# YukeWang96/GNNAdvisor_OSDI21

Measured on AMD Instinct MI355X. Metric: aggregated edges/sec, GCN sum-aggregation SpMM (SAG) hidden=64, higher is better.
Workload: dtype f32; 1 GPU; reddit-like power-law graph, random node order; num_nodes=232965, nnz=114623790, dim=64, partSize=128, num_parts=1008217, parallelism=single GPU, call=GNNA.SAG (pybind module, reference signature, fresh output), decider=auto/mi355x, column_phases=16, build_id=0.6.1+dd9458378fe52dcc

## Files before the change

gnnadvisor_osdi21_amd/_lib.py:

```python
from __future__ import annotations

import ctypes
import math
import os

import torch

_HERE = os.path.dirname(os.path.abspath(__file__))
LIB_PATH = os.environ.get("GNNA_LIB") or os.path.join(_HERE, "csrc", "libgnna.so")

GNNA_OK = 0


class GnnaError(RuntimeError):
    pass


class Tuning(ctypes.Structure):
    _fields_ = [("struct_size", ctypes.c_int), ("groups_per_chunk", ctypes.c_int), ("loads_in_flight", ctypes.c_int),
                ("blocks_per_cu", ctypes.c_int), ("xcd_remap", ctypes.c_int),
                ("trust_canonical", ctypes.c_int), ("column_phases", ctypes.c_int),
                ("avg_degree", ctypes.c_int), ("nonlocal_ids", ctypes.c_int), ("gcn_prescale", ctypes.c_int),
                ("pad_rows", ctypes.c_int), ("zero_fill", ctypes.c_int),
                ("sweep", ctypes.c_int), ("sweep_slack", ctypes.c_int), ("deterministic", ctypes.c_int),
# ... 238 lines not shown
    ci = torch.empty(max(1, s.numel()), dtype=torch.int32)
    nnz = load().gnna_csr_from_edges_i32(s.data_ptr(), d.data_ptr(), s.numel(), int(num_nodes),
                                         rp.data_ptr(), ci.data_ptr())
    if nnz < 0:
        _check(int(nnz))
    return rp, ci[:nnz].clone()


def row_counts(rows, num_nodes: int, counts: torch.Tensor | None = None) -> torch.Tensor:
    r = _host_i32(rows)
    if counts is None:
        counts = torch.zeros(int(num_nodes), dtype=torch.int64)
    assert counts.dtype == torch.int64 and counts.numel() == int(num_nodes) and counts.is_contiguous()
    _check(load().gnna_row_counts_i64(r.data_ptr(), r.numel(), int(num_nodes), counts.data_ptr()))
    return counts


def row_splits(counts: torch.Tensor, world: int, want_row_pointers: bool = False):
    assert counts.dtype == torch.int64 and counts.is_contiguous() and not counts.is_cuda
    n = counts.numel()
    bounds = torch.empty(int(world) + 1, dtype=torch.int64)
    rp = torch.empty(n + 1, dtype=torch.int64) if want_row_pointers else None
    _check(load().gnna_row_splits_i64(counts.data_ptr(), n, int(world), bounds.data_ptr(), _ptr(rp)))
    return (bounds.tolist(), rp) if want_row_pointers else bounds.tolist()


def csr_from_edges_range(src, dst, num_nodes: int, row_lo: int, row_hi: int, capacity: int | None = None):
    s, d = _host_i32(src), _host_i32(dst)
    assert s.numel() == d.numel()
    if capacity is None:
        capacity = int(((s >= row_lo) & (s < row_hi)).sum()) if s.numel() else 0
    rp = torch.empty(int(row_hi - row_lo) + 1, dtype=torch.int32)
    ci = torch.empty(max(1, int(capacity)), dtype=torch.int32)
    nnz = load().gnna_csr_from_edges_range_i32(s.data_ptr(), d.data_ptr(), s.numel(), int(num_nodes), int(row_lo),
                                               int(row_hi), rp.data_ptr(), ci.data_ptr(), int(capacity))
    if nnz < 0:
        _check(int(nnz))
    return rp, ci[:nnz].clone()


def degrees(row_pointers: torch.Tensor) -> torch.Tensor:
    rp = _host_i32(row_pointers)
    out = torch.empty(rp.numel() - 1, dtype=torch.float32)
    _check(load().gnna_degrees_f32(rp.data_ptr(), rp.numel() - 1, out.data_ptr()))
    return out


def edge_span(src, dst) -> float:
    s, d = _host_i32(src), _host_i32(dst)
    v = ctypes.c_double()
    _check(load().gnna_edge_span(s.data_ptr(), d.data_ptr(), s.numel(), ctypes.byref(v)))
    return v.value


def _reorder(entry: str, src, dst, num_nodes: int) -> torch.Tensor:
    s, d = _host_i32(src), _host_i32(dst)
    out = torch.empty(int(num_nodes), dtype=torch.int32)
    _check(getattr(load(), entry)(s.data_ptr(), d.data_ptr(), s.numel(), int(num_nodes), out.data_ptr()))
    return out


def reorder_rcm(src, dst, num_nodes: int) -> torch.Tensor:
    return _reorder("gnna_reorder_rcm_i32", src, dst, num_nodes)


def reorder_community(src, dst, num_nodes: int) -> torch.Tensor:
    return _reorder("gnna_reorder_community_i32", src, dst, num_nodes)


def reorder_community_csr(row_pointers, column_index, num_nodes: int) -> torch.Tensor:
    rp, ci = _host_i32(row_pointers), _host_i32(column_index)
    assert rp.numel() == int(num_nodes) + 1
    out = torch.empty(int(num_nodes), dtype=torch.int32)
    _check(load().gnna_reorder_community_csr_i32(rp.data_ptr(), ci.data_ptr(), int(num_nodes), out.data_ptr()))
    return out


def relabel_edges_(src: torch.Tensor, dst: torch.Tensor, new_id: torch.Tensor, num_nodes: int) -> float:
    for t in (src, dst, new_id):
        assert t.dtype == torch.int32 and t.is_contiguous() and not t.is_cuda
    v = ctypes.c_double()
    _check(load().gnna_relabel_edges_i32(src.data_ptr(), dst.data_ptr(), src.numel(), new_id.data_ptr(), int(num_nodes), ctypes.byref(v)))
    return v.value


def relabel_csr(row_pointers, column_index, new_id, num_nodes: int):
    rp, ci, nid = _host_i32(row_pointers), _host_i32(column_index), _host_i32(new_id)
    out_rp = torch.empty(int(num_nodes) + 1, dtype=torch.int32)
    out_ci = torch.empty(max(1, ci.numel()), dtype=torch.int32)
    _check(load().gnna_relabel_csr_i32(rp.data_ptr(), ci.data_ptr(), int(num_nodes), nid.data_ptr(), out_rp.data_ptr(), out_ci.data_ptr()))
    return out_rp, out_ci[:ci.numel()]


def last_num_phases() -> int:
    return int(load().gnna_last_num_phases())


def last_num_launches() -> int:
    return int(load().gnna_last_num_launches())


def profile_begin(max_calls: int) -> None:
    _check(load().gnna_profile_begin(int(max_calls)))


def profile_end() -> dict:
    a, b, n = ctypes.c_double(), ctypes.c_double(), ctypes.c_int()
    _check(load().gnna_profile_end(ctypes.byref(a), ctypes.byref(b), ctypes.byref(n)))
    return dict(main_ms=a.value, prologue_ms=b.value, calls=n.value)


def count_parts(partSize: int, indptr: torch.Tensor) -> int:
    assert indptr.dtype == torch.int32 and not indptr.is_cuda and indptr.is_contiguous()
    n = load().gnna_count_parts(int(partSize), indptr.data_ptr(), indptr.numel() - 1)
    if n < 0:
        _check(int(n))
    return int(n)


def build_part(partSize: int, indptr: torch.Tensor):
    indptr = indptr.contiguous()
    P = count_parts(partSize, indptr)
    pp = torch.empty(P + 1, dtype=torch.int32)
    p2n = torch.empty(P, dtype=torch.int32)
    _check(load().gnna_build_part_i32(int(partSize), indptr.data_ptr(), indptr.numel() - 1,
                                      pp.data_ptr(), p2n.data_ptr(), P))
    return pp, p2n


def _fresh_output(shape, device, dtype=torch.float32) -> torch.Tensor:
    if os.environ.get("GNNA_DEBUG_POISON", "0") not in ("", "0"):
        return torch.full(tuple(shape), float("nan") if dtype.is_floating_point else -(2 ** 31), dtype=dtype, device=device)
    return torch.empty(tuple(shape), dtype=dtype, device=device)


def _agg(fn_name, X, row_pointers, column_index, extra, part_pointers, part2Node, partSize, dimWorker,
         warpPerBlock, out):
    _need_device(X, "aggregation")
    assert X.dtype == torch.float32 and X.is_contiguous() and X.dim() == 2
    for t in (column_index, part_pointers, part2Node):
        assert t.dtype == torch.int32 and t.is_contiguous() and t.device == X.device
    if out is None:
        out = _fresh_output(X.shape, X.device)
    _call(X.device, fn_name, X.data_ptr(), _ptr(row_pointers), column_index.data_ptr(), extra,
          part_pointers.data_ptr(), part2Node.data_ptr(), out.data_ptr(), X.shape[0], X.shape[1], part2Node.numel(),
          int(partSize), int(dimWorker), int(warpPerBlock))
    return out


def sag(X, row_pointers, column_index, degrees, part_pointers, part2Node, partSize=32, dimWorker=32,
        warpPerBlock=4, out=None):
    return _agg("gnna_sag_f32", X, row_pointers, column_index, _ptr(degrees), part_pointers,
                part2Node, partSize, dimWorker, warpPerBlock, out)


def agg_gcn(X, row_pointers, column_index, degrees, part_pointers, part2Node, partSize=32,
            dimWorker=32, warpPerBlock=4, out=None):
    assert degrees.dtype == torch.float32 and degrees.device == X.device
    return _agg("gnna_agg_gcn_f32", X, row_pointers, column_index, degrees.data_ptr(),
                part_pointers, part2Node, partSize, dimWorker, warpPerBlock, out)


def agg_gin(X, row_pointers, column_index, epsilon, part_pointers, part2Node, partSize=32,
            dimWorker=32, warpPerBlock=4, out=None):
    return _agg("gnna_agg_gin_f32", X, row_pointers, column_index, ctypes.c_float(epsilon),
                part_pointers, part2Node, partSize, dimWorker, warpPerBlock, out)


MODE_SAG, MODE_GCN, MODE_GIN = 0, 1, 2


def agg_rect(mode, X, column_index, part_pointers, part2Node, num_out_rows, partSize=32,
             degrees_out=None, degrees_in=None, epsilon=1.0, out=None, accumulate=False, windows=None):
    _need_device(X, "aggregation")
    assert X.dtype == torch.float32 and X.is_contiguous() and X.dim() == 2
    if out is None:
        assert not accumulate, "accumulate needs an existing `out`"
        out = _fresh_output((num_out_rows, X.shape[1]), X.device)
    args = (int(mode), X.data_ptr(), X.shape[0], column_index.data_ptr(), _ptr(degrees_out), _ptr(degrees_in), float(epsilon),
            part_pointers.data_ptr(), part2Node.data_ptr(), out.data_ptr(), int(num_out_rows), X.shape[1], part2Node.numel(),
            int(partSize), 1 if accumulate else 0)
    if windows is not None:
        K, wb, we = (int(v) for v in windows)
        assert wb == 0 or out is not None
        _call(X.device, "gnna_agg_rect_windows_f32", *args, K, wb, we)
    else:
        _call(X.device, "gnna_agg_rect_f32", *args)
    return out


ACCUMULATE, EPILOGUE_RELU = 1, 2


def _flags(accumulate=False, relu=False) -> int:
    return (ACCUMULATE if accumulate else 0) | (EPILOGUE_RELU if relu else 0)


def _rows_view(t: torch.Tensor, what: str, dtype=torch.float32, unit="floats"):
    assert (dtype is None or t.dtype == dtype) and t.dim() == 2, \
        f"{what} must be a 2-D {'' if dtype is None else str(dtype).replace('torch.', '') + ' '}tensor"
    if t.shape[1] > 1 and t.stride(1) != 1:
        raise GnnaError(f"{what}: the {unit} of a row must be contiguous (stride(1) == 1)")
    ld = t.stride(0) if t.shape[0] > 1 else max(t.shape[1], t.stride(0))
    if ld < t.shape[1]:
        raise GnnaError(f"{what}: rows overlap (stride(0) = {t.stride(0)} < {t.shape[1]})")
    return t.data_ptr(), t.shape[0], t.shape[1], ld


def _rows_view_any(t: torch.Tensor, what: str):
    return _rows_view(t, what, dtype=None, unit="elements")


def _out_rows(out, rows, width, device, accumulate=False):
    if out is None:
        assert not accumulate, "accumulate needs an existing `out`"
        out = _fresh_output((rows, width), device)
    ptr, n, w, ld = _rows_view(out, "out")
    assert n == int(rows) and w == width and out.device == device
    return out, ptr, ld


def agg_ld(mode, X, column_index, part_pointers, part2Node, num_out_rows, partSize=32, degrees_out=None,
           degrees_in=None, epsilon=1.0, out=None, accumulate=False, relu=False):
    _need_device(X, "aggregation")
    xp, n_in, dim, ld_in = _rows_view(X, "X")
    out, yp, ld_out = _out_rows(out, num_out_rows, dim, X.device, accumulate)
    _call(X.device, "gnna_agg_ld_f32", int(mode), xp, ld_in, n_in, column_index.data_ptr(), _ptr(degrees_out), _ptr(degrees_in),
          float(epsilon), part_pointers.data_ptr(), part2Node.data_ptr(), yp, ld_out, int(num_out_rows), dim, part2Node.numel(),
          int(partSize), _flags(accumulate, relu))
    return out


F32, BF16, F16 = 0, 1, 2
_X16_TYPES = {torch.bfloat16: BF16, torch.float16: F16}


def agg_ld_x16(mode, X, column_index, part_pointers, part2Node, num_out_rows, partSize=32, degrees_out=None,
               degrees_in=None, epsilon=1.0, out=None, out_dtype=None, accumulate=False, relu=False):
    _need_device(X, "aggregation")
    if X.dtype not in _X16_TYPES:
        raise GnnaError(f"agg_ld_x16 takes bfloat16 or float16 features (got {X.dtype}); float32 goes through agg_ld")
    xp, n_in, dim, ld_in = _rows_view_any(X, "X")
    if out is None:
        assert not accumulate, "accumulate needs an existing `out`"
        out = _fresh_output((int(num_out_rows), dim), X.device, X.dtype if out_dtype is None else out_dtype)
    elif out_dtype is not None and out.dtype != out_dtype:
        raise GnnaError(f"out is {out.dtype}, out_dtype says {out_dtype}")
    if out.dtype != torch.float32 and out.dtype != X.dtype:
        raise GnnaError(f"the output is float32 or has the input's dtype {X.dtype} (got {out.dtype})")
    out_type = F32 if out.dtype == torch.float32 else _X16_TYPES[out.dtype]
    yp, n_out, dim_o, ld_out = _rows_view_any(out, "out")
    assert n_out == int(num_out_rows) and dim_o == dim and out.device == X.device
    for t in (degrees_out, degrees_in):
        assert t is None or t.dtype == torch.float32, "degrees stay float32"
    _call(X.device, "gnna_agg_ld_x16", int(mode), _X16_TYPES[X.dtype], xp, ld_in, n_in, column_index.data_ptr(), _ptr(degrees_out),
          _ptr(degrees_in), float(epsilon), part_pointers.data_ptr(), part2Node.data_ptr(), yp, out_type, ld_out, int(num_out_rows),
          dim, part2Node.numel(), int(partSize), _flags(accumulate, relu))
    return out


def prepare_x16(num_in_rows: int, num_out_rows: int, dims, device=None) -> None:
    dims = [int(d) for d in dims]
    arr = (ctypes.c_int * max(1, len(dims)))(*dims)
    device = torch.device("cuda", torch.cuda.current_device()) if device is None else torch.device(device)
    _call(device, "gnna_prepare_x16", int(num_in_rows), int(num_out_rows), arr, len(dims))


def preferred_ld(dim: int, num_in_rows: int, num_edges: int) -> int:
    return int(load().gnna_preferred_ld(int(dim), int(num_in_rows), int(num_edges)))


def empty_rows(num_rows: int, dim: int, ld: int, device) -> torch.Tensor:
    if ld == dim:
        return torch.empty(num_rows, dim, dtype=torch.float32, device=device)
    buf = torch.empty(num_rows * ld + ld, dtype=torch.float32, device=device)
    off = (-buf.data_ptr() // 4) % ld
    return buf[off: off + num_rows * ld].view(num_rows, ld)[:, :dim]


def prepare_graph(column_index, part_pointers, part2Node, num_in_rows: int, num_out_rows: int, partSize: int,
                  dims=()) -> dict:
    dims = [int(d) for d in dims]
    arr = (ctypes.c_int * max(1, len(dims)))(*dims)
    out = (ctypes.c_int * max(1, len(dims)))()
    _call(column_index.device, "gnna_prepare_graph", column_index.data_ptr(), part_pointers.data_ptr(), part2Node.data_ptr(),
          part2Node.numel(), int(num_in_rows), int(num_out_rows), int(partSize), arr, len(dims), out)
    _forget_when_freed(column_index)
    return {d: int(out[i]) for i, d in enumerate(dims)}


def release_graph(column_index) -> None:
    ptr = None if column_index is None else column_index.data_ptr()
    _check(load().gnna_release_graph(ptr))
    if column_index is None:
        _registered.clear()
    else:
        _registered.pop(ptr, None)


def runtime_counters() -> dict:
    out = (ctypes.c_int64 * 16)()
    n = load().gnna_runtime_counters_ex(out, 16)
    names = ("plan_builds", "launch_syncs", "launch_frees", "launch_mallocs", "backoff_skips", "sweep_launches",
             "pack_builds", "packed_launches", "full_hashes", "capture_scratch")
    return {name: int(out[i]) for i, name in enumerate(names) if i < n}


def debug_untrusted_copies(column_index) -> int:
    n = load().gnna_debug_untrusted_copies(column_index.data_ptr())
    _check(min(n, 0))
    return n


def set_graph_phases(column_index, dim: int, column_phases: int) -> None:
    _check(load().gnna_set_graph_phases(column_index.data_ptr(), int(dim), int(column_phases)))
    if column_phases > 0:
        _forget_when_freed(column_index)


def xtg(X, G, out=None):
    _need_device(X, "xtg")
    assert X.dtype == torch.float32 and G.dtype == torch.float32 and X.dim() == 2 and G.dim() == 2
    assert X.shape[0] == G.shape[0]
    X, G = X.contiguous(), G.contiguous()
    if out is None:
        out = torch.empty(X.shape[1], G.shape[1], dtype=torch.float32, device=X.device)
    _call(X.device, "gnna_xtg_f32", X.data_ptr(), G.data_ptr(), out.data_ptr(), X.shape[0], X.shape[1], G.shape[1])
    return out


def sddmm(dst_feat, src_feat, column_index, part_pointers, part2Node, partSize=32, out=None):
    _need_device(dst_feat, "sddmm")
    ap, n_out, dim, ld_dst = _rows_view(dst_feat, "dst_feat")
    bp, n_in, dim_b, ld_src = _rows_view(src_feat, "src_feat")
    assert dim == dim_b and dst_feat.device == src_feat.device
    if out is None:
        out = torch.zeros(column_index.numel(), dtype=torch.float32, device=dst_feat.device)
    tail = (column_index.data_ptr(), part_pointers.data_ptr(), part2Node.data_ptr(), out.data_ptr(), n_out, n_in, dim,
            part2Node.numel(), int(partSize))
    if ld_dst == dim and ld_src == dim:
        _call(dst_feat.device, "gnna_sddmm_f32", ap, bp, *tail)
    else:
        _call(dst_feat.device, "gnna_sddmm_ld_f32", ap, ld_dst, bp, ld_src, *tail)
    return out


def agg_edge(X, column_index, edge_weight, part_pointers, part2Node, num_out_rows, partSize=32, out=None,
             accumulate=False, relu=False):
    _need_device(X, "aggregation")
    assert edge_weight.dtype == torch.float32 and edge_weight.is_contiguous() and edge_weight.numel() == column_index.numel(), \
        "edge_weight must be a contiguous float32 tensor indexed like column_index"
    xp, n_in, dim, ld_in = _rows_view(X, "X")
    out, yp, ld_out = _out_rows(out, num_out_rows, dim, X.device, accumulate)
    _call(X.device, "gnna_agg_edge_ld_f32", xp, ld_in, n_in, column_index.data_ptr(), edge_weight.data_ptr(), part_pointers.data_ptr(),
          part2Node.data_ptr(), yp, ld_out, int(num_out_rows), dim, part2Node.numel(), int(partSize), _flags(accumulate, relu))
    return out


def edge_softmax(scores, row_pointers, out=None):
    assert scores.is_cuda and scores.dtype == torch.float32 and scores.is_contiguous() and scores.dim() in (1, 2)
    heads, nnz = (1, scores.numel()) if scores.dim() == 1 else scores.shape
    out = torch.empty_like(scores) if out is None else out
    _call(scores.device, "gnna_edge_softmax_f32", scores.data_ptr(), row_pointers.data_ptr(), row_pointers.numel() - 1, nnz, heads,
          out.data_ptr())
    return out


def edge_softmax_backward(probs, grad_probs, row_pointers, out=None):
    assert probs.is_cuda and probs.dtype == torch.float32 and probs.is_contiguous() and probs.dim() in (1, 2)
    assert grad_probs.shape == probs.shape and grad_probs.dtype == torch.float32 and grad_probs.is_contiguous()
    heads, nnz = (1, probs.numel()) if probs.dim() == 1 else probs.shape
    out = torch.empty_like(probs) if out is None else out
    _call(probs.device, "gnna_edge_softmax_backward_f32", probs.data_ptr(), grad_probs.data_ptr(), row_pointers.data_ptr(),
          row_pointers.numel() - 1, nnz, heads, out.data_ptr())
    return out


def reverse_edges(row_pointers, column_index) -> torch.Tensor:
    rp, ci = _host_i32(row_pointers), _host_i32(column_index)
    rev = torch.empty(ci.numel(), dtype=torch.int32)
    _check(load().gnna_reverse_edges_i32(rp.data_ptr(), ci.data_ptr(), rp.numel() - 1, rev.data_ptr()))
    return rev


REDUCE_MAX, REDUCE_MIN = 0, 1


def _arg_view(t: torch.Tensor, rows: int, dim: int, what: str):
    assert t.dtype == torch.int32 and t.dim() == 2 and tuple(t.shape) == (rows, dim), f"{what} must be int32 [{rows}, {dim}]"
    ptr, _, _, ld = _rows_view(t, what, dtype=torch.int32, unit="elements")
    return ptr, ld


def agg_reduce_ld(op, X, column_index, part_pointers, part2Node, partSize=32, *, num_out_rows=None, out=None, want_arg=True,
                  relu=False, arg=None):
    _need_device(X, "aggregation")
    xp, n_in, dim, ld_in = _rows_view(X, "X")
    n_out = n_in if num_out_rows is None else int(num_out_rows)
    out, yp, ld_out = _out_rows(out, n_out, dim, X.device)
    ap, ld_arg = None, dim
    if arg is not None or want_arg:
        if arg is None:
            arg = _fresh_output((n_out, dim), X.device, torch.int32)
        assert arg.device == X.device
        ap, ld_arg = _arg_view(arg, n_out, dim, "arg")
    _call(X.device, "gnna_agg_reduce_ld_f32", int(op), xp, ld_in, n_in, column_index.data_ptr(), part_pointers.data_ptr(),
          part2Node.data_ptr(), yp, ld_out, ap, ld_arg, n_out, dim, part2Node.numel(), int(partSize), _flags(relu=relu))
    return out, arg


def scatter_arg_ld(grad_out, arg, column_index, num_in_rows, out=None, accumulate=False):
    _need_device(grad_out, "scatter_arg")
    gp, n_out, dim, ld_go = _rows_view(grad_out, "grad_out")
    ap, ld_arg = _arg_view(arg, n_out, dim, "arg")
    out, op_, ld_gi = _out_rows(out, int(num_in_rows), dim, grad_out.device, accumulate)
    assert arg.device == grad_out.device
    _call(grad_out.device, "gnna_scatter_arg_ld_f32", gp, ld_go, ap, ld_arg, column_index.data_ptr(), n_out, op_, ld_gi,
          int(num_in_rows), dim, _flags(accumulate))
    return out


STATS = ("sum", "sumsq", "max", "min")


def agg_stats_ld(X, column_index, part_pointers, part2Node, num_out_rows=None, partSize=32, want=STATS, out=None):
    _need_device(X, "aggregation")
    want = tuple(want)
    unknown = [w for w in want if w not in STATS]
    if unknown or not want:
        raise ValueError(f"want must name some of {STATS} (got {want!r})")
    xp, n_in, dim, ld_in = _rows_view(X, "X")
    n_out = n_in if num_out_rows is None else int(num_out_rows)
    out = dict(out or {})
    res, args = {}, []
    for name in STATS:
        wanted = name in want
        val = None
        if wanted:
            val, vp, ld = _out_rows(out.get(name), n_out, dim, X.device)
            res[name] = val
        args += [vp if wanted else None, ld if wanted else dim]
        if name in ("max", "min"):
            arg = None
            if wanted and ("arg" + name in out or name not in out):
                arg = out.get("arg" + name)
                if arg is None:
                    arg = _fresh_output((n_out, dim), X.device, torch.int32)
                assert arg.device == X.device
                ap, ld_arg = _arg_view(arg, n_out, dim, "arg" + name)
                res["arg" + name] = arg
            args += [ap if arg is not None else None, ld_arg if arg is not None else dim]
    _call(X.device, "gnna_agg_stats_ld_f32", xp, ld_in, n_in, column_index.data_ptr(), part_pointers.data_ptr(), part2Node.data_ptr(),
          *args, n_out, dim, part2Node.numel(), int(partSize), 0)
    return res


def _temp_arg(temp, dim, device):
    assert temp.dtype == torch.float32 and temp.device == device and temp.is_contiguous() and temp.numel() in (1, dim), \
        f"temp must be a contiguous float32 tensor of 1 or {dim} elements on {device}"
    return temp.data_ptr(), temp.numel()


def _ids_ptr(column_index, row_pointers):
    return column_index.data_ptr() or row_pointers.data_ptr()


def agg_softmax(X, temp, row_pointers, column_index, num_out_rows=None, want_sq=False, out=None, lse=None, sq=None):
    _need_device(X, "aggregation")
    xp, n_in, dim, ld_in = _rows_view(X, "X")
    n_out = row_pointers.numel() - 1 if num_out_rows is None else int(num_out_rows)
    assert row_pointers.numel() == n_out + 1, f"row_pointers must be [num_out_rows + 1 = {n_out + 1}] (got {row_pointers.numel()} entries)"
    tp, tl = _temp_arg(temp, dim, X.device)
    out, op_, ld_out = _out_rows(out, n_out, dim, X.device)
    lse, lp, ld_lse = _out_rows(lse, n_out, dim, X.device)
    qp, ld_sq = None, dim
    if want_sq or sq is not None:
        sq, qp, ld_sq = _out_rows(sq, n_out, dim, X.device)
    _call(X.device, "gnna_agg_softmax_ld_f32", xp, ld_in, n_in, tp, tl, row_pointers.data_ptr(), _ids_ptr(column_index, row_pointers),
          op_, ld_out, lp, ld_lse, qp, ld_sq, n_out, dim, 0)
    return out, lse, sq


def agg_softmax_backward(X, temp, lse, Y, dY, t_row_pointers, t_column_index, out=None):
    _need_device(X, "aggregation")
    xp, n_in, dim, ld_in = _rows_view(X, "X")
    assert t_row_pointers.numel() == n_in + 1, f"t_row_pointers must be [num_in_rows + 1 = {n_in + 1}] (got {t_row_pointers.numel()} entries)"
    tp, tl = _temp_arg(temp, dim, X.device)
    lp, n_out, w, ld_lse = _rows_view(lse, "lse")
    yp, ny, wy, ld_y = _rows_view(Y, "Y")
    gp, ng, wg, ld_dy = _rows_view(dY, "dY")
    assert (ny, ng) == (n_out, n_out) and (w, wy, wg) == (dim, dim, dim), "lse, Y and dY must be [num_out_rows, dim]"
    out, op_, ld_din = _out_rows(out, n_in, dim, X.device)
    _call(X.device, "gnna_agg_softmax_backward_ld_f32", xp, ld_in, n_in, tp, tl, lp, ld_lse, yp, ld_y, gp, ld_dy,
          t_row_pointers.data_ptr(), _ids_ptr(t_column_index, t_row_pointers), op_, ld_din, n_out, dim, 0)
    return out


POOL_TILE_ROWS = 256
POOL_LONG_STEPS = 16
POOL_MEAN = 1
POOL_STATS = ("sum", "max", "min")


def _graph_pointers_arg(graph_pointers, device):
    assert graph_pointers.dtype == torch.int32 and graph_pointers.dim() == 1 and graph_pointers.numel() >= 1 and \
        graph_pointers.is_contiguous() and graph_pointers.device == device, \
        f"graph_pointers must be a contiguous int32 tensor [num_graphs + 1] on {device}"
    return graph_pointers.data_ptr(), graph_pointers.numel() - 1


def segment_pool(X, graph_pointers, want=("sum",), mean=False, out=None):
    want = tuple(want)
    if not want or [w for w in want if w not in POOL_STATS]:
        raise ValueError(f"want must name some of {POOL_STATS} (got {want!r})")
    _need_device(X, "segment_pool")
    xp, n, dim, ld_in = _rows_view(X, "X")
    gp, G = _graph_pointers_arg(graph_pointers, X.device)
    out = dict(out or {})
    res, args = {}, []
    for name in POOL_STATS:
        wanted = name in want
        if wanted:
            val, vp, ld = _out_rows(out.get(name), G, dim, X.device)
            res[name] = val
        args += [vp if wanted else None, ld if wanted else dim]
        if name != "sum":
            arg = None
            if wanted and ("arg" + name in out or name not in out):
                arg = out.get("arg" + name)
                if arg is None:
                    arg = _fresh_output((G, dim), X.device, torch.int32)
                assert arg.device == X.device
                ap, ld_arg = _arg_view(arg, G, dim, "arg" + name)
                res["arg" + name] = arg
            args += [ap if arg is not None else None, ld_arg if arg is not None else dim]
    if G > 0:
        _call(X.device, "gnna_segment_pool_ld_f32", xp if n > 0 else None, ld_in, n, gp, G, *args, dim, POOL_MEAN if mean else 0)
    return res


def segment_pool_backward(graph_pointers, num_rows, d_sum=None, d_max=None, argmax=None, d_min=None, argmin=None, mean=False, out=None):
    given = [t for t in (d_sum, d_max, d_min) if t is not None]
    if not given:
        raise ValueError("segment_pool_backward needs d_sum, d_max or d_min")
    if (d_max is None) != (argmax is None) or (d_min is None) != (argmin is None):
        raise ValueError("d_max comes with argmax, d_min with argmin")
    _need_device(given[0], "segment_pool_backward")
    device = given[0].device
    gp, G = _graph_pointers_arg(graph_pointers, device)
    dim = given[0].shape[1]
    args = []
    for grad, arg, name in ((d_sum, None, "d_sum"), (d_max, argmax, "d_max"), (d_min, argmin, "d_min")):
        if grad is None:
            args += [None, dim] * (1 if name == "d_sum" else 2)
            continue
        vp, rows, w, ld = _rows_view(grad, name)
        assert (rows, w) == (G, dim) and grad.device == device, f"{name} must be [num_graphs = {G}, dim = {dim}] on {device}"
        args += [vp, ld]
        if name != "d_sum":
            assert arg.device == device
            args += list(_arg_view(arg, G, dim, "arg" + name[2:]))
    out, op_, ld_din = _out_rows(out, int(num_rows), dim, device)
    if G == 0:
        stand_in = torch.zeros(1, dim, dtype=torch.float32, device=device)
        args = [stand_in.data_ptr(), dim] + [None, dim] * 4
    _call(device, "gnna_segment_pool_backward_ld_f32", *args, gp, G, op_ if int(num_rows) > 0 else None, ld_din, int(num_rows), dim,
          POOL_MEAN if mean else 0)
    return out


def _gate_view(gate, n, dim, device):
    g2 = gate.unsqueeze(1) if gate.dim() == 1 else gate
    gp_, rows, gate_dim, ld_gate = _rows_view(g2, "gate")
    assert rows == n and gate_dim in (1, dim) and gate.device == device, \
        f"gate must be [{n}], [{n}, 1] or [{n}, {dim}] on {device} (got {tuple(gate.shape)})"
    return gp_, gate_dim, ld_gate


def segment_attn_pool(X, gate, graph_pointers, out=None):
    _need_device(X, "segment_attn_pool")
    xp, n, dim, ld_in = _rows_view(X, "X")
    gtp, gate_dim, ld_gate = _gate_view(gate, n, dim, X.device)
    gp, G = _graph_pointers_arg(graph_pointers, X.device)
    given = dict(out or {})
    res = {}
    res["out"], op_, ld_out = _out_rows(given.get("out"), G, dim, X.device)
    lp, ld_lse = None, gate_dim
    if "lse" in given or "out" not in given:
        res["lse"], lp, ld_lse = _out_rows(given.get("lse"), G, gate_dim, X.device)
    if G > 0:
        _call(X.device, "gnna_segment_attn_pool_ld_f32", xp if n > 0 else None, ld_in, n, gtp if n > 0 else None, ld_gate, gate_dim,
              gp, G, op_, ld_out, lp, ld_lse, dim, 0)
    return res


def segment_attn_pool_backward(X, gate, lse, Y, dY, graph_pointers, need_input=True, need_gate=True, out=None):
    if not need_input and not need_gate:
        raise ValueError("segment_attn_pool_backward needs need_input or need_gate")
    _need_device(X, "segment_attn_pool_backward")
    xp, n, dim, ld_in = _rows_view(X, "X")
    gtp, gate_dim, ld_gate = _gate_view(gate, n, dim, X.device)
    gp, G = _graph_pointers_arg(graph_pointers, X.device)
    lp, gl, wl, ld_lse = _rows_view(lse, "lse")
    yp, gy, wy, ld_y = _rows_view(Y, "Y")
    dp, gd, wd, ld_dy = _rows_view(dY, "dY")
    assert (gl, gy, gd) == (G, G, G) and (wl, wy, wd) == (gate_dim, dim, dim) and lse.device == Y.device == dY.device == X.device, \
        f"lse must be [{G}, {gate_dim}], Y and dY [{G}, {dim}] on {X.device}"
# ... 483 lines not shown
```

gnnadvisor_osdi21_amd/build.py:

```python
from __future__ import annotations

import os
import subprocess
import sys
import sysconfig

PKG = os.path.dirname(os.path.abspath(__file__))
ROOT = os.path.dirname(PKG)
CSRC = os.path.join(PKG, "csrc")
INCLUDE = os.path.join(ROOT, "include")
LIB = os.path.join(CSRC, "libgnna.so")
EXT = os.path.join(PKG, "GNNAdvisor.so")
ARCH = "gfx950"
HIPCC = os.environ.get("HIPCC", "/opt/rocm/bin/hipcc")

LIB_SOURCES = [os.path.join(CSRC, f) for f in ("gnna_agg.hip", "gnna_stream.hip", "gnna_sweep.hip", "gnna_x16.hip", "gnna_reduce.hip", "gnna_stats.hip", "gnna_softagg.hip", "gnna_pool.hip", "gnna_attnpool.hip", "gnna_sddmm.hip", "gnna_edge.hip", "gnna_gat.hip", "gnna_gatv2.hip", "gnna_dotattn.hip", "gnna_typed.hip", "gnna_transpose.hip", "gnna_sample.hip",
                                                "gnna_gemm.hip", "gnna_runtime.hip", "gnna_host.cpp", "gnna_reorder.cpp")]
LIB_DEPS = LIB_SOURCES + [os.path.join(CSRC, "gnna_internal.h"), os.path.join(CSRC, "gnna_device.h"), os.path.join(CSRC, "gnna_launch.h"),
                           os.path.join(CSRC, "gnna_gat_common.h"), os.path.join(CSRC, "gnna_keys.h"), os.path.join(CSRC, "gnna_segments.h"), os.path.join(INCLUDE, "gnna.h"), os.path.join(INCLUDE, "gnna_ext.h"),
                           os.path.join(INCLUDE, "gnna_gatv2.h"), os.path.join(INCLUDE, "gnna_dotattn.h"),
                           os.path.join(INCLUDE, "gnna_gat_edge.h"), os.path.join(INCLUDE, "gnna_stats.h"),
                           os.path.join(INCLUDE, "gnna_softagg.h"), os.path.join(INCLUDE, "gnna_pool.h"),
                           os.path.join(INCLUDE, "gnna_attnpool.h")]
EXT_SOURCES = [os.path.join(CSRC, "gnna_torch.cpp")]
EXT_DEPS = EXT_SOURCES + [os.path.join(INCLUDE, "gnna.h"), os.path.join(INCLUDE, "gnna_ext.h"), os.path.join(INCLUDE, "gnna_gatv2.h"),
                          os.path.join(INCLUDE, "gnna_dotattn.h"), os.path.join(INCLUDE, "gnna_gat_edge.h"),
                          os.path.join(INCLUDE, "gnna_stats.h"), os.path.join(INCLUDE, "gnna_softagg.h"), os.path.join(INCLUDE, "gnna_pool.h"),
                          os.path.join(INCLUDE, "gnna_attnpool.h")]


def source_hash() -> str:
    import hashlib
    h = hashlib.sha256()
    for path in sorted(set(LIB_DEPS + EXT_DEPS)):
        h.update(os.path.relpath(path, ROOT).encode() + b"\0")
        with open(path, "rb") as f:
            h.update(f.read())
        h.update(b"\0")
    return h.hexdigest()[:16]


def _stale(target: str, deps: list[str]) -> bool:
    if not os.path.exists(target):
        return True
    t = os.path.getmtime(target)
    return any(os.path.getmtime(d) > t for d in deps)


def build_lib(force: bool = False, verbose: bool = False) -> str:
    from concurrent.futures import ThreadPoolExecutor
    objdir = os.path.join(CSRC, "build")
    os.makedirs(objdir, exist_ok=True)
    headers = [d for d in LIB_DEPS if d not in LIB_SOURCES]
    flags = [f"--offload-arch={ARCH}", "-O3", "-std=c++17", "-fPIC", "-munsafe-fp-atomics", "-ffp-contract=off",
             "-fvisibility=hidden", "-I" + INCLUDE, "-I" + CSRC]
    jobs, objs = [], []
    digest = source_hash()
    stamp = os.path.join(objdir, "source_hash.txt")
    stamped = open(stamp).read().strip() if os.path.exists(stamp) else ""
    if not force and stamped == digest and os.path.exists(LIB) and not _stale(LIB, LIB_DEPS):
        return LIB
    for src in LIB_SOURCES:
        obj = os.path.join(objdir, os.path.basename(src) + ".o")
        objs.append(obj)
        carries_id = os.path.basename(src) == "gnna_host.cpp"
        if force or _stale(obj, [src] + headers) or (carries_id and stamped != digest):
            jobs.append([HIPCC, *flags, *([f'-DGNNA_SOURCE_HASH="{digest}"'] if carries_id else []), "-c", src, "-o", obj])

    def run(cmd):
        if verbose:
            print(" ".join(cmd), flush=True)
        subprocess.check_call(cmd)
    if jobs:
        with ThreadPoolExecutor(max_workers=min(len(jobs), os.cpu_count() or 4)) as pool:
            list(pool.map(run, jobs))
    if jobs or force or _stale(LIB, objs):
        run([HIPCC, f"--offload-arch={ARCH}", "-shared", "-fPIC", "-fvisibility=hidden", *objs, "-o", LIB])
    with open(stamp, "w") as f:
        f.write(digest + "\n")
    if verbose:
        print(f"libgnna.so: source hash {digest} ({'compiled ' + str(len(jobs)) + ' object(s)' if jobs else 'objects up to date'})", flush=True)
    return LIB


def build_ext(force: bool = False, verbose: bool = False) -> str:
    build_lib(force, verbose)
    digest = source_hash()
    stamp = os.path.join(CSRC, "build", "ext_source_hash.txt")
    stamped = open(stamp).read().strip() if os.path.exists(stamp) else ""
    if force or _stale(EXT, EXT_DEPS + [LIB]) or stamped != digest:
        import pybind11
        import torch
        tdir = os.path.dirname(torch.__file__)
        cmd = [HIPCC, "-O2", "-std=c++17", "-fPIC", "-shared", "-w",
               "-DTORCH_EXTENSION_NAME=GNNAdvisor", "-DTORCH_API_INCLUDE_EXTENSION_H", f'-DGNNA_SOURCE_HASH="{digest}"',
               "-DUSE_ROCM", "-D__HIP_PLATFORM_AMD__",
               f"-D_GLIBCXX_USE_CXX11_ABI={int(torch._C._GLIBCXX_USE_CXX11_ABI)}",
               "-I" + INCLUDE,
               "-I" + os.path.join(tdir, "include"),
               "-I" + os.path.join(tdir, "include", "torch", "csrc", "api", "include"),
               "-I" + sysconfig.get_paths()["include"], "-I" + pybind11.get_include(),
               "-I/opt/rocm/include",
               "-x", "c++", *EXT_SOURCES, "-o", EXT,
               "-L" + CSRC, "-lgnna", "-Wl,-rpath,$ORIGIN/csrc",
               "-L" + os.path.join(tdir, "lib"), "-lc10", "-lc10_hip", "-ltorch", "-ltorch_cpu",
               "-ltorch_hip", "-ltorch_python", "-Wl,-rpath," + os.path.join(tdir, "lib")]
        if verbose:
            print(" ".join(cmd))
        subprocess.check_call(cmd)
        with open(stamp, "w") as f:
            f.write(digest + "\n")
    return EXT


def build_all(force: bool = False, verbose: bool = False) -> None:
    build_ext(force, verbose)


if __name__ == "__main__":
    build_all(force="--force" in sys.argv, verbose=True)
    print("built", LIB, "and", EXT)
```

gnnadvisor_osdi21_amd/csrc/gnna_agg.hip:

```cpp
#include <hip/hip_runtime.h>

#include <algorithm>
#include <cmath>
#include <cstdint>
#include <cstdio>

#include "gnna.h"
#include "gnna_device.h"
#include "gnna_internal.h"

namespace gnna {
namespace {


__global__ void __launch_bounds__(kBlock)
prologue_kernel(float *__restrict__ Y, size_t n_floats, int D, int ldy, const int32_t *__restrict__ p2n,
                const int32_t *__restrict__ pp, int64_t P, int32_t *flag, int32_t seq, int validate, int zero_fill,
                const int32_t *__restrict__ chk_ids, int64_t chk_n, const unsigned long long *__restrict__ chk_sum,
                int32_t *stale_flag, uint32_t *__restrict__ clear_words, int n_clear)
{
    if (blockIdx.x == 0 && (int)threadIdx.x < n_clear) clear_words[threadIdx.x] = 0u;
    const unsigned fill_blocks = chk_ids ? gridDim.x - 1 : gridDim.x;
    if (blockIdx.x >= fill_blocks) {
        if (threadIdx.x < kWave) {
            const unsigned long long then = chk_sum[0], distrusted = chk_sum[4];
            const unsigned long long now = graph_checksum(chk_ids, chk_n, pp, P, (int)threadIdx.x);
            if (threadIdx.x == 0 && (now != then || distrusted != 0ull)) *stale_flag = seq;
        }
        return;
    }
    const size_t tid = (size_t)blockIdx.x * blockDim.x + threadIdx.x;
    const size_t nthreads = (size_t)fill_blocks * blockDim.x;
    typedef float f32x4 __attribute__((ext_vector_type(4)));
    if (!zero_fill) {
    } else if (ldy != D) {
        if ((D & 3) == 0 && (ldy & 3) == 0 && (reinterpret_cast<uintptr_t>(Y) & 15) == 0) {
            const size_t n4 = n_floats >> 2;
            const unsigned d4 = (unsigned)D >> 2, ld4 = (unsigned)ldy >> 2;
            const f32x4 z = (f32x4)(0.f);
            for (size_t i = tid; i < n4; i += nthreads) {
                const size_t r = i / d4;
                reinterpret_cast<f32x4 *>(Y)[r * ld4 + (i - r * d4)] = z;
            }
        } else {
            for (size_t i = tid; i < n_floats; i += nthreads) {
                const size_t r = i / (unsigned)D;
                Y[r * (size_t)ldy + (i - r * (unsigned)D)] = 0.f;
            }
        }
    } else if ((reinterpret_cast<uintptr_t>(Y) & 15) == 0) {
        const size_t n4 = n_floats >> 2;
        f32x4 *Y4 = reinterpret_cast<f32x4 *>(Y);
        const f32x4 z = (f32x4)(0.f);
        for (size_t i = tid; i < n4; i += nthreads) Y4[i] = z;
        for (size_t i = (n4 << 2) + tid; i < n_floats; i += nthreads) Y[i] = 0.f;
    } else {
        for (size_t i = tid; i < n_floats; i += nthreads) Y[i] = 0.f;
    }
    if (validate) {
        bool bad = false;
        for (int64_t g = (int64_t)tid; g < P; g += (int64_t)nthreads) {
            if (pp[g + 1] < pp[g]) bad = true;
            if (g + 1 < P && p2n[g + 1] < p2n[g]) bad = true;
        }
        if (bad) *flag = seq;
    }
}

__global__ void __launch_bounds__(kBlock)
sparse_prologue_kernel(float *__restrict__ Y, int64_t N, int D, int ldy, const int32_t *__restrict__ p2n,
                       const int32_t *__restrict__ pp, int64_t P, int G, int32_t *flag, int32_t seq, int validate,
                       unsigned long long *gaps, int64_t big_rows)
{
    const int lane = threadIdx.x & (kWave - 1);
    const int64_t wave = ((int64_t)blockIdx.x * blockDim.x + threadIdx.x) >> 6;
    const int64_t nwaves = ((int64_t)gridDim.x * blockDim.x) >> 6;
    typedef float f32x4 __attribute__((ext_vector_type(4)));
    const bool vec_ok = (D & 3) == 0 && (reinterpret_cast<uintptr_t>(Y) & 15) == 0;
    auto clear_rows = [&](int64_t lo, int64_t cnt) {
        if (gaps && cnt >= big_rows) {
            unsigned long long idx = 0;
            if (lane == 0) idx = atomicAdd(&gaps[0], 1ull);
            idx = ((unsigned long long)__builtin_amdgcn_readfirstlane((int)(idx >> 32)) << 32) |
                  (uint32_t)__builtin_amdgcn_readfirstlane((int)idx);
            if (idx < (unsigned long long)kGapEntries) {
                if (lane == 0) { gaps[2 + 2 * idx] = (unsigned long long)lo; gaps[3 + 2 * idx] = (unsigned long long)cnt; }
                return;
            }
        }
        if (ldy != D) {
            for (int64_t r = lo; r < lo + cnt; r++) {
                float *row = Y + (size_t)r * (size_t)ldy;
                for (int i = lane; i < D; i += kWave) row[i] = 0.f;
            }
            return;
        }
        float *base = Y + (size_t)lo * (size_t)D;
        const size_t n = (size_t)cnt * (size_t)D;
        if (vec_ok) {
            f32x4 *b4 = reinterpret_cast<f32x4 *>(base);
            const f32x4 z = (f32x4)(0.f);
            for (size_t i = lane; i < (n >> 2); i += kWave) b4[i] = z;
        } else {
            for (size_t i = lane; i < n; i += kWave) base[i] = 0.f;
        }
    };
    if (wave == 0) {
        int64_t first = p2n[0];
        first = first < 0 ? 0 : (first > N ? N : first);
        if (first > 0) clear_rows(0, first);
    }
    bool bad = false;
    for (int64_t g0 = wave * kWave; g0 < P; g0 += nwaves * kWave) {
        const int64_t g = g0 + lane;
        const bool valid = g < P;
        int64_t lo = 0, cnt = 0;
        if (valid) {
            const int64_t r = p2n[g];
            const int64_t nxt = g + 1 < P ? (int64_t)p2n[g + 1] : N;
            const int a = pp[g], b = pp[g + 1];
            if (b < a || (g + 1 < P && nxt < r)) bad = true;
            const bool continues = g > 0 && (g % G) == 0 && p2n[g - 1] == r;
            const bool self = b <= a || continues;
            lo = self ? r : r + 1;
            int64_t hi = (self && nxt < r + 1) ? r + 1 : nxt;
            lo = lo < 0 ? 0 : lo;
            hi = hi > N ? N : hi;
            cnt = hi > lo ? hi - lo : 0;
        }
        unsigned long long m = __ballot(cnt > 0);
        while (m) {
            const int l = __builtin_ctzll(m);
            m &= m - 1;
            const int64_t lo_s = ((int64_t)__builtin_amdgcn_readlane((int)(lo >> 32), l) << 32) |
                                 (uint32_t)__builtin_amdgcn_readlane((int)lo, l);
            const int64_t cnt_s = ((int64_t)__builtin_amdgcn_readlane((int)(cnt >> 32), l) << 32) |
                                  (uint32_t)__builtin_amdgcn_readlane((int)cnt, l);
            clear_rows(lo_s, cnt_s);
        }
    }
    if (validate && bad) *flag = seq;
}

__global__ void __launch_bounds__(kBlock)
post_prologue_kernel(float *__restrict__ Y, size_t n_floats, int D, int ldy, const int32_t *flag, int32_t seq,
                     const unsigned long long *gaps)
{
    const size_t tid = (size_t)blockIdx.x * blockDim.x + threadIdx.x;
    const size_t nthreads = (size_t)gridDim.x * blockDim.x;
    auto at = [&](float *base, size_t i) -> float * {
        if (ldy == D) return base + i;
        const size_t r = i / (unsigned)D;
        return base + r * (size_t)ldy + (i - r * (unsigned)D);
    };
    if (*flag == seq) {
        for (size_t i = tid; i < n_floats; i += nthreads) *at(Y, i) = 0.f;
        return;
    }
    if (!gaps) return;
    const unsigned long long n = gaps[0] < (unsigned long long)kGapEntries ? gaps[0] : (unsigned long long)kGapEntries;
    for (unsigned long long k = 0; k < n; k++) {
        float *base = Y + (size_t)gaps[2 + 2 * k] * (size_t)ldy;
        const size_t cnt = (size_t)gaps[3 + 2 * k] * (size_t)D;
        for (size_t i = tid; i < cnt; i += nthreads) *at(base, i) = 0.f;
    }
}

__global__ void __launch_bounds__(kBlock)
scale_rows_kernel(const float *__restrict__ X, int64_t ld_in, const float *__restrict__ deg, float *__restrict__ Xs,
                  int64_t rows, int D, int ld_out)
{
    const size_t tid = (size_t)blockIdx.x * blockDim.x + threadIdx.x;
    const size_t nthreads = (size_t)gridDim.x * blockDim.x;
    typedef float f32x4 __attribute__((ext_vector_type(4)));
    const bool aligned = ((reinterpret_cast<uintptr_t>(X) | reinterpret_cast<uintptr_t>(Xs)) & 15) == 0;
    if (ld_out == D && ld_in == D && (D & 3) == 0 && aligned) {
        const size_t n4 = ((size_t)rows * (size_t)D) >> 2;
        const int d4 = D >> 2;
        for (size_t i = tid; i < n4; i += nthreads) {
            const f32x4 v = __builtin_nontemporal_load(reinterpret_cast<const f32x4 *>(X) + i);
            reinterpret_cast<f32x4 *>(Xs)[i] = deg ? v * deg[i / d4] : v;
        }
    } else if ((D & 3) == 0 && (ld_out & 3) == 0 && (ld_in & 3) == 0 && aligned) {
        const size_t n4 = ((size_t)rows * (size_t)D) >> 2;
        const unsigned d4 = (unsigned)D >> 2;
        const size_t ldo4 = (size_t)ld_out >> 2, ldi4 = (size_t)ld_in >> 2;
        for (size_t i = tid; i < n4; i += nthreads) {
            const size_t r = i / d4, c4 = i - r * d4;
            const f32x4 v = __builtin_nontemporal_load(reinterpret_cast<const f32x4 *>(X) + r * ldi4 + c4);
            reinterpret_cast<f32x4 *>(Xs)[r * ldo4 + c4] = deg ? v * deg[r] : v;
        }
    } else {
        const size_t total = (size_t)rows * (size_t)D;
        for (size_t i = tid; i < total; i += nthreads) {
            const size_t r = i / (unsigned)D, cc = i - r * (unsigned)D;
            const float v = __builtin_nontemporal_load(X + r * (size_t)ld_in + cc);
            Xs[r * (size_t)ld_out + cc] = deg ? v * deg[r] : v;
        }
    }
}


static size_t gather_footprint_bytes(int64_t num_in_rows, int ldx, int dim)
{
    return (size_t)num_in_rows * (size_t)std::min(ldx, (std::max(dim, 4) * 4 + 127) / 128 * 32) * sizeof(float);
}

thread_local int t_last_phases = 1;
thread_local int t_last_launches = 1;

double avg_lines_per_row(int64_t row_bytes, int64_t stride_bytes)
{
    int64_t lines = 0;
    for (int k = 0; k < 32; k++) {
        const int64_t o = (k * stride_bytes) % 128;
        lines += (o + row_bytes + 127) / 128;
    }
    return (double)lines / 32.0;
}

int choose_row_stride(int dim)
{
    if (dim < 2 || dim > 256) return dim;
    auto cost = [&](int stride) {
        return avg_lines_per_row((int64_t)dim * 4, (int64_t)stride * 4) * ((stride & 3) ? 1.07 : 1.0);
    };
    const double plain = cost(dim);
    int best = dim;
    double best_cost = plain * 0.93;
    const int cand[3] = {(dim + 3) / 4 * 4, (dim + 15) / 16 * 16, (dim + 31) / 32 * 32};
    for (int c : cand) {
        if (c == dim || c > 2 * dim) continue;
        const double cc = cost(c) * (1.0 + 0.02 * (double)(c - dim) / (double)dim);
        if (cc < best_cost) { best = c; best_cost = cc; }
    }
    return best;
}

int pick_row_stride(const gnna_tuning &t, int dim, bool hot_rows, int64_t num_in_rows, bool whole_call)
{
    int ldx = dim;
    if (t.pad_rows == 1 || (t.pad_rows == 0 && hot_rows)) ldx = choose_row_stride(dim);
    if (t.pad_rows == 0 && hot_rows && dim > 16 && dim <= 64 && whole_call) {
        const int gapped = 2 * ((dim * 4 + 127) / 128) * 32;
        if ((size_t)num_in_rows * (size_t)gapped * sizeof(float) <= ((size_t)160 << 20)) ldx = gapped;
    }
    if (t.pad_rows > 2 && t.pad_rows >= dim) ldx = t.pad_rows;
    return ldx;
}

}

int stage_rows_for_gather(DeviceState *ds, hipStream_t stream, const gnna_tuning &tune, const float *input, int64_t ld_in,
                          int64_t num_in_rows, int dim, int64_t est_edges, const float **X, int *ldx_out)
{
    *X = input; *ldx_out = (int)ld_in;
    const bool hot_rows = est_edges >= 32 * num_in_rows && (size_t)num_in_rows * (size_t)dim * sizeof(float) <= ((size_t)1 << 30);
    if (dim < 4 || !hot_rows) return GNNA_OK;
    const int want = pick_row_stride(tune, dim, hot_rows, num_in_rows, true);
    if (want == dim || ld_in == want) return GNNA_OK;
    const bool aligned16 = (reinterpret_cast<uintptr_t>(input) & 15) == 0 && (ld_in & 3) == 0;
    const int gapped = 2 * ((dim * 4 + 127) / 128) * 32;
    bool direct;
    if (want == gapped && dim > 16 && dim <= 64)
        direct = (ld_in % gapped) == 0 && (reinterpret_cast<uintptr_t>(input) % ((size_t)gapped * 4)) == 0;
    else
        direct = aligned16 && avg_lines_per_row((int64_t)dim * 4, ld_in * 4) <= avg_lines_per_row((int64_t)dim * 4, (int64_t)want * 4) + 1e-9;
    if (direct) return GNNA_OK;
    const size_t x_bytes = (size_t)num_in_rows * (size_t)want * sizeof(float);
    void *xs = nullptr;
    int rc = get_workspace(ds, stream, 1, x_bytes, &xs);
    if (rc != GNNA_OK) return rc;
    const size_t s_bytes = (size_t)num_in_rows * (size_t)dim * sizeof(float);
    int64_t sblocks = (int64_t)((s_bytes / 16 + kBlock - 1) / kBlock);
    sblocks = std::max<int64_t>(1, std::min<int64_t>(sblocks, (int64_t)ds->num_cus * 8));
    hipLaunchKernelGGL(scale_rows_kernel, dim3((unsigned)sblocks), dim3(kBlock), 0, stream, input, ld_in, (const float *)nullptr,
                       static_cast<float *>(xs), num_in_rows, dim, want);
    hipError_t es = hipGetLastError();
    if (es != hipSuccess) return fail(GNNA_ERR_HIP, "staging launch: %s", hipGetErrorString(es));
    *X = static_cast<const float *>(xs); *ldx_out = want;
    return GNNA_OK;
}

static double near_share(const SlicePlanStats &st, double half_rows)
{
    if (st.edges <= 0 || half_rows < 256.0) return 0.0;
    const double pos = std::min(23.0, 2.0 * std::log2(half_rows / 256.0));
    const int k = (int)pos;
    const double lo = st.near[k], hi = st.near[std::min(23, k + 1)];
    return (lo + (hi - lo) * (pos - k)) / st.edges;
}

int sweep_auto_phases(const gnna_tuning &t, int mode, int dim, size_t x_bytes, int64_t num_out_rows, int64_t num_in_rows,
                      const SlicePlanStats &st, int B, int num_cus, bool deterministic, int part_size)
{
    const double edges = st.edges;
    if (t.sweep != 0 || deterministic || B < 2) return 0;
    if (dim <= 32 || dim > 64 || !sweep_supports(mode, dim, x_bytes)) return 0;
    if (num_in_rows != num_out_rows || x_bytes > ((size_t)160 << 20)) return 0;
    if (edges < 300.0 * (double)std::max<int64_t>(1, num_out_rows)) return 0;
    const double cap = (double)sweep_acc_rows(dim, 1) * 0.9 * (double)std::max(8, num_cus);
    if ((double)num_out_rows > 2.0 * cap) return 0;
    if (near_share(st, (double)num_in_rows / 16.0) > 0.30) return 0;
    if (t.column_phases >= 2) return B;
    return std::max(2, std::min(std::min(16, 2 * B), std::max(2, part_size / 4)));
}

int sweep_phases_of_width(const gnna_tuning &t, int dim, size_t foot_bytes, size_t x_bytes, int64_t num_out_rows,
                          int64_t num_in_rows, const SlicePlanStats &st, int B, int num_cus, int partSize, int S)
{
    int Bs = sweep_auto_phases(t, MODE_SAG, dim, foot_bytes, num_out_rows, num_in_rows, st, B, num_cus, t.deterministic == 1, partSize);
    if (t.sweep == 1 && t.deterministic != 1 && sweep_supports(MODE_SAG, dim, x_bytes))
        Bs = t.column_phases >= 2 ? B : std::max(2, std::min(std::min(16, 2 * B), std::max(2, partSize / 4)));
    return std::min(Bs, S);
}

int choose_slices(const SlicePlanStats &st, size_t x_bytes, int S, uint32_t slice_rows, int64_t num_out_rows,
                  bool square, bool hinted_scattered)
{
    if (st.groups <= 0 || st.edges <= 0) return 1;
    if (!hinted_scattered) {
        if (square) {
            const double row_bytes = (double)x_bytes / ((double)slice_rows * S);
            const double half_rows = 1.75 * 1048576.0 / row_bytes;
            const bool long_rows_cached = st.edges >= 200.0 * (double)std::max<int64_t>(1, num_out_rows) && x_bytes <= (size_t)250000000;
            const bool one_line_rows = row_bytes > 64.0 && row_bytes <= 128.0;
            if (near_share(st, half_rows) >= (long_rows_cached && !one_line_rows ? 0.75 : 0.6)) return 1;
        }
        if (st.cells[0] <= 1.15 * st.groups) return 1;
    }
    int b = 1;
    const double row_bytes_all = (double)x_bytes / ((double)slice_rows * S);
    const size_t slice_target = row_bytes_all <= 64.0 ? ((size_t)4 << 20) : ((size_t)8 << 20);
    while (b < S && x_bytes / b > slice_target) b <<= 1;
    int lvl = 0;
    for (int t = S; t > b; t >>= 1) lvl++;
    const double rows = std::min((double)num_out_rows, st.groups);
    auto piece = [&](int l) {
        return st.edges / std::max(rows, st.cells[l] - (st.groups - rows));
    };
    int levels = 0;
    for (int t = S; t > 1; t >>= 1) levels++;
    levels = std::min(levels, kSliceLevels);
    const double min_piece = row_bytes_all <= 128.0 ? 24.0 : 12.0;
    while (b > 1 && lvl < levels && piece(lvl) < min_piece) { b >>= 1; lvl++; }
    if (lvl >= levels) b = 1;
    const size_t mall = (size_t)250000000;
    if (x_bytes > mall) {
        int bm = 2, lm = levels - 1;
        while (bm < S && x_bytes / bm > mall) { bm <<= 1; lm--; }
        if (x_bytes / bm <= mall && lm >= 0 && piece(lm) >= 8.0) b = std::max(b, bm);
    }
    return std::max(b, 1);
}

int launch_zero_fill(DeviceState *ds, hipStream_t stream, float *out, int64_t rows, int dim, int64_t ld)
{
    const size_t n_floats = (size_t)rows * (size_t)dim;
    if (n_floats == 0) return GNNA_OK;
    int64_t blocks = (int64_t)((n_floats / 4 + kBlock - 1) / kBlock);
    blocks = std::max<int64_t>(1, std::min<int64_t>(blocks, (int64_t)ds->num_cus * 8));
    hipLaunchKernelGGL(prologue_kernel, dim3((unsigned)blocks), dim3(kBlock), 0, stream, out, n_floats, dim, (int)ld, nullptr, nullptr,
                       (int64_t)0, nullptr, 0, 0, 1, nullptr, (int64_t)0, nullptr, nullptr, nullptr, 0);
    return launch_ok("zero-fill launch");
}

namespace {
__global__ void __launch_bounds__(kBlock)
relu_rows_kernel(float *__restrict__ Y, size_t ld, size_t rows, int D)
{
    const size_t n = rows * (size_t)D;
    for (size_t i = (size_t)blockIdx.x * blockDim.x + threadIdx.x; i < n; i += (size_t)gridDim.x * blockDim.x) {
        const size_t r = i / (unsigned)D, c = i - r * (unsigned)D;
        if (Y[r * ld + c] < 0.f) Y[r * ld + c] = 0.f;
    }
}
}

void launch_relu_rows(DeviceState *ds, hipStream_t stream, float *out, int64_t rows, int dim, int64_t ld)
{
    hipLaunchKernelGGL(relu_rows_kernel, dim3(elementwise_grid(rows * dim, ds->num_cus, 8)), dim3(kBlock), 0, stream, out,
                       (size_t)ld, (size_t)rows, dim);
}

namespace {

int launch_agg(int mode, const float *input, int64_t ld_in, int64_t num_in_rows, const int32_t *column_index,
               const float *degrees, const float *degrees_in, float epsilon, const int32_t *part_pointers,
               const int32_t *part2Node, float *out, int64_t ld_out, int64_t num_nodes, int dim, int64_t num_parts,
               int partSize, int dimWorker, int warpPerBlock, void *stream_v, unsigned flags,
               int num_windows = 1, int win_begin = 0, int win_end = 1, bool profiled = true, int hint_dim = 0);

int column_blocks(const gnna_tuning &tune, int dim, int64_t num_in_rows, int64_t est_edges)
{
    if (tune.wide_blocks == 2 || dim < 72) return 1;
    if (tune.wide_blocks == 1) return (dim + 63) / 64;
    const bool hot = est_edges >= 32 * num_in_rows;
    if (!hot || (size_t)num_in_rows * (size_t)dim * sizeof(float) > ((size_t)250000000)) return 1;
    const bool long_rows = est_edges >= 200 * num_in_rows;
    if (dim < (long_rows ? 100 : 192)) return 1;
    return (dim + 63) / 64;
}

int launch_agg_blocked(int nb, int mode, const float *input, int64_t ld_in, int64_t num_in_rows, const int32_t *column_index,
                       const float *degrees, const float *degrees_in, float epsilon, const int32_t *part_pointers,
                       const int32_t *part2Node, float *out, int64_t ld_out, int64_t num_nodes, int dim, int64_t num_parts,
                       int partSize, int dimWorker, int warpPerBlock, void *stream_v, unsigned flags)
{
    hipStream_t stream = static_cast<hipStream_t>(stream_v);
    const int prof_call = profile_acquire_call(num_parts > 0);
    profile_record(prof_call, 0, stream);
    profile_record(prof_call, 1, stream);
    const int w = ((dim + nb - 1) / nb + 3) / 4 * 4;
    int launches = 0, phases = 1;
    for (int c0 = 0; c0 < dim; c0 += w) {
        const int wb = std::min(w, dim - c0);
        const int rc = launch_agg(mode, input + c0, ld_in, num_in_rows, column_index, degrees, degrees_in, epsilon, part_pointers,
                                  part2Node, out + c0, ld_out, num_nodes, wb, num_parts, partSize, dimWorker, warpPerBlock, stream_v,
                                  flags, 1, 0, 1, false, dim);
        if (rc != GNNA_OK) return rc;
        launches += t_last_launches;
        phases = std::max(phases, t_last_phases);
    }
    t_last_launches = launches;
    t_last_phases = phases;
    profile_record(prof_call, 2, stream);
    return GNNA_OK;
}

int launch_agg(int mode, const float *input, int64_t ld_in, int64_t num_in_rows, const int32_t *column_index,
               const float *degrees, const float *degrees_in, float epsilon, const int32_t *part_pointers,
               const int32_t *part2Node, float *out, int64_t ld_out, int64_t num_nodes, int dim, int64_t num_parts,
               int partSize, int dimWorker, int warpPerBlock, void *stream_v, unsigned flags,
               int num_windows, int win_begin, int win_end, bool profiled, int hint_dim)
{
    const bool accumulate_into_out = (flags & GNNA_ACCUMULATE) != 0;
    const bool relu = (flags & GNNA_EPILOGUE_RELU) != 0;
    if (flags & ~(unsigned)(GNNA_ACCUMULATE | GNNA_EPILOGUE_RELU))
        return fail(GNNA_ERR_INVALID_ARGUMENT, "unknown flag bits 0x%x", flags);
    if (num_nodes < 0 || dim < 0 || num_parts < 0 || num_in_rows < 0)
        return fail(GNNA_ERR_INVALID_ARGUMENT, "negative size (num_nodes=%lld dim=%d num_parts=%lld)",
                          (long long)num_nodes, dim, (long long)num_parts);
    if (partSize <= 0 || dimWorker <= 0 || warpPerBlock <= 0)
        return fail(GNNA_ERR_INVALID_ARGUMENT,
                          "partSize, dimWorker and warpPerBlock must be positive (got %d, %d, %d)",
                          partSize, dimWorker, warpPerBlock);
    if (num_windows < 1 || num_windows > 16 || win_begin < 0 || win_end > num_windows || win_begin >= win_end)
        return fail(GNNA_ERR_INVALID_ARGUMENT, "bad source window range [%d, %d) of %d (at most 16 windows)",
                    win_begin, win_end, num_windows);
    if (num_nodes >= ((int64_t)1 << 29))
        return fail(GNNA_ERR_UNSUPPORTED, "%lld destination rows in one call (at most 536870911): shard the rows",
                    (long long)num_nodes);
    if (num_nodes == 0 || dim == 0) return GNNA_OK;
    if (bad_ld(ld_in, dim) || bad_ld(ld_out, dim))
        return fail(GNNA_ERR_INVALID_ARGUMENT, "row strides must be >= dim and < 2^29 floats (ld_in=%lld ld_out=%lld dim=%d)",
                    (long long)ld_in, (long long)ld_out, dim);
    if (!out || !input) return fail(GNNA_ERR_INVALID_ARGUMENT, "null feature pointer");
    if (num_parts > 0 && (!column_index || !part_pointers || !part2Node))
        return fail(GNNA_ERR_INVALID_ARGUMENT, "null index pointer");
    if (mode == MODE_GCN && (!degrees || !degrees_in))
        return fail(GNNA_ERR_INVALID_ARGUMENT, "null degrees pointer");
    if (mode == MODE_EDGE && num_parts > 0 && !degrees_in)
        return fail(GNNA_ERR_INVALID_ARGUMENT, "null edge_weight pointer");
    if (out == input) return fail(GNNA_ERR_INVALID_ARGUMENT, "out must not alias input");

    hipStream_t stream = static_cast<hipStream_t>(stream_v);
    DeviceState *ds = nullptr;
    int rc = get_device_state(&ds);
    if (rc != GNNA_OK) return rc;
    LaunchGuard in_flight;

    gnna_tuning tune;
    gnna_get_tuning(&tune);
    apply_graph_hints(column_index, hint_dim > 0 ? hint_dim : dim, &tune);

    const bool windowed = num_windows > 1;
    if (profiled && !windowed && num_parts > 0) {
        const int64_t est = num_parts * (int64_t)(tune.avg_degree > 0 ? std::min(partSize, tune.avg_degree) : partSize / 2 + 1);
        const int nb = column_blocks(tune, dim, num_in_rows, est);
        if (nb > 1)
            return launch_agg_blocked(nb, mode, input, ld_in, num_in_rows, column_index, degrees, degrees_in, epsilon, part_pointers,
                                      part2Node, out, ld_out, num_nodes, dim, num_parts, partSize, dimWorker, warpPerBlock, stream_v, flags);
    }
    int32_t *flag = nullptr;
    const int32_t seq = next_call_seq(ds, stream, &flag);
    const int prof_call = profiled ? profile_acquire_call(num_parts > 0) : -1;
    profile_record(prof_call, 0, stream);
    const int ldy = (int)ld_out;

    const size_t n_floats = (size_t)num_nodes * (size_t)dim;
    const unsigned long long *chk_sum = nullptr;
    int64_t chk_n = 0;
    int32_t *stale_flag = flag + kFlagSlots;
    auto run_prologue = [&](int sparse_G, uint32_t *clear_words = nullptr, int n_clear = 0) -> int {
        const int validate = (num_parts > 0 && !tune.trust_canonical) ? 1 : 0;
        const int zero_fill = (accumulate_into_out || win_begin > 0) ? 0 : 1;
        if (sparse_G > 0 && zero_fill && num_parts > 0) {
            int64_t blocks = (num_parts + kBlock - 1) / kBlock;
            blocks = std::max<int64_t>(1, std::min<int64_t>(blocks, (int64_t)ds->num_cus * 8));
            unsigned long long *gaps = ds->gap_lists + (size_t)call_block_of(ds, stream, seq) * kGapWords;
            (void)hipMemsetAsync(gaps, 0, sizeof(unsigned long long), stream);
            const int64_t big_rows = std::max<int64_t>(64, ((int64_t)1 << 20) / std::max(1, dim * 4));
            hipLaunchKernelGGL(sparse_prologue_kernel, dim3((unsigned)blocks), dim3(kBlock), 0, stream, out, num_nodes, dim, ldy,
                               part2Node, part_pointers, num_parts, sparse_G, flag, seq, validate, gaps, big_rows);
            hipLaunchKernelGGL(post_prologue_kernel, dim3((unsigned)(ds->num_cus * 8)), dim3(kBlock), 0, stream, out,
                               n_floats, dim, ldy, flag, seq, gaps);
        } else {
            size_t work = std::max(n_floats / 4, (size_t)num_parts);
            int64_t blocks = (int64_t)((work + kBlock - 1) / kBlock);
            blocks = std::max<int64_t>(1, std::min<int64_t>(blocks, (int64_t)ds->num_cus * 8));
            hipLaunchKernelGGL(prologue_kernel, dim3((unsigned)blocks + (chk_sum ? 1u : 0u)), dim3(kBlock), 0, stream, out, n_floats,
                               dim, ldy, part2Node, part_pointers, num_parts, flag, seq, validate, zero_fill,
                               chk_sum ? column_index : nullptr, chk_n, chk_sum, stale_flag, clear_words, n_clear);
        }
        hipError_t e = hipGetLastError();
        if (e != hipSuccess) return fail(GNNA_ERR_HIP, "prologue launch: %s", hipGetErrorString(e));
        profile_record(prof_call, 1, stream);
        return GNNA_OK;
    };
    if (num_parts == 0) {
        rc = run_prologue(0);
        if (rc != GNNA_OK || !relu || !accumulate_into_out) return rc;
        StreamLaunch e0;
        e0.mode = mode; e0.Y = out; e0.p2n = part2Node; e0.P = 0; e0.D = dim; e0.ldy = ldy; e0.relu = true; e0.num_out_rows = num_nodes;
        e0.flag = flag; e0.seq = seq; e0.cnt = nullptr; e0.B = 1; e0.plain_ok = false; e0.G = 1;
        return launch_stream_epilogue_only(e0, stream);
    }

    const int64_t window_rows = (num_in_rows + num_windows - 1) / num_windows;

    const int64_t est_edges = num_parts * (int64_t)(tune.avg_degree > 0 ? std::min(partSize, tune.avg_degree) : partSize / 2 + 1);
    const bool hot_rows = est_edges >= 32 * num_in_rows && (size_t)num_in_rows * (size_t)dim * sizeof(float) <= ((size_t)1 << 30);
    const bool prescale = mode == MODE_GCN && (tune.gcn_prescale == 1 || (tune.gcn_prescale == 0 && hot_rows));
    const int want = dim < 4 ? 4 : pick_row_stride(tune, dim, hot_rows, num_in_rows, !windowed);
    bool direct = !prescale && dim >= 4;
    if (direct && want != dim && ld_in != want) {
        const bool aligned16 = (reinterpret_cast<uintptr_t>(input) & 15) == 0 && (ld_in & 3) == 0;
        const int gapped = 2 * ((dim * 4 + 127) / 128) * 32;
        if (want == gapped && dim > 16 && dim <= 64)
            direct = (ld_in % gapped) == 0 && (reinterpret_cast<uintptr_t>(input) % ((size_t)gapped * 4)) == 0;
        else
            direct = aligned16 && avg_lines_per_row((int64_t)dim * 4, ld_in * 4) <= avg_lines_per_row((int64_t)dim * 4, (int64_t)want * 4) + 1e-9;
    }
    const int ldx = direct ? (int)ld_in : want;
    const float *X = input;
    const float *row_scale = nullptr;
    float eps = epsilon;
    const size_t x_bytes = (size_t)num_in_rows * (size_t)ldx * sizeof(float);
    const size_t foot_bytes = gather_footprint_bytes(num_in_rows, ldx, dim);
    const bool wide = x_bytes > 0xffffffffull;
    if (!direct) {
        void *xs = nullptr;
        rc = get_workspace(ds, stream, 1, x_bytes, &xs);
        if (rc != GNNA_OK) return rc;
        const int64_t r0 = std::min<int64_t>((int64_t)win_begin * window_rows, num_in_rows);
        const int64_t r1 = std::min<int64_t>((int64_t)win_end * window_rows, num_in_rows);
        const size_t s_bytes = (size_t)(r1 - r0) * (size_t)dim * sizeof(float);
        int64_t sblocks = (int64_t)((s_bytes / 16 + kBlock - 1) / kBlock);
        sblocks = std::max<int64_t>(1, std::min<int64_t>(sblocks, (int64_t)ds->num_cus * 8));
        hipLaunchKernelGGL(scale_rows_kernel, dim3((unsigned)sblocks), dim3(kBlock), 0, stream,
                           input + (size_t)r0 * (size_t)ld_in, ld_in, prescale ? degrees_in + r0 : nullptr,
                           static_cast<float *>(xs) + (size_t)r0 * ldx, r1 - r0, dim, ldx);
        hipError_t es = hipGetLastError();
        if (es != hipSuccess) return fail(GNNA_ERR_HIP, "staging launch: %s", hipGetErrorString(es));
        X = static_cast<const float *>(xs);
        if (prescale) {
            row_scale = degrees;
            eps = 1.f;
            mode = MODE_GIN;
        }
    }

    int B = 1;
    const uint8_t *cnt = nullptr;
    int S = kMaxSlices;
    int win_lo = 0, win_hi = 0;
    SlicePlan plan;
    const bool can_slice = num_parts >= 1024 && num_in_rows >= 64 && foot_bytes >= ((size_t)2 << 20);
    if (windowed) {
        rc = get_slice_plan(ds, stream, column_index, part_pointers, part2Node, num_parts, num_in_rows, true, false, &plan,
                            (uint32_t)std::max<int64_t>(1, window_rows));
        if (rc != GNNA_OK) return rc;
        if (!plan.cnt || !plan.stats.valid)
            return fail(GNNA_ERR_UNSUPPORTED, "the windowed aggregation needs its window counts, which cannot be built inside a "
                                              "stream capture: run the sequence once before capturing it");
        if (plan.stats.unsorted > 0)
            return fail(GNNA_ERR_UNSUPPORTED, "windowed aggregation: the column ids of %.0f neighbor-groups are not in increasing "
                                              "order (sort the ids of every row, as the loader's CSR has them)", plan.stats.unsorted);
        cnt = plan.cnt; S = plan.S; B = 1;
        win_lo = win_begin; win_hi = win_end == num_windows ? S : win_end;
    } else {
        if (tune.column_phases >= 2 && num_in_rows >= kMaxSlices) {
            B = std::min(tune.column_phases, kMaxSlices);
            rc = get_slice_plan(ds, stream, column_index, part_pointers, part2Node, num_parts, num_in_rows, false, false, &plan);
            if (rc != GNNA_OK) return rc;
        } else if (tune.column_phases == 0 && can_slice && foot_bytes >= ((size_t)6 << 20)) {
            rc = get_slice_plan(ds, stream, column_index, part_pointers, part2Node, num_parts, num_in_rows, true, false, &plan);
            if (rc != GNNA_OK) return rc;
            if (plan.cnt && plan.stats.valid)
                B = choose_slices(plan.stats, foot_bytes, plan.S, plan.slice_rows, num_nodes, num_in_rows == num_nodes,
                                  tune.nonlocal_ids == 1);
        }
        cnt = plan.cnt;
        if (cnt) S = plan.S;
        if (!cnt || B < 2) { B = 1; cnt = nullptr; }
    }

    const int auto_Bs = (cnt && !windowed && plan.stats.valid)
                            ? sweep_auto_phases(tune, mode, dim, foot_bytes, num_nodes, num_in_rows, plan.stats, B, ds->num_cus,
                                                tune.deterministic == 1, partSize) : 0;
    if (mode != MODE_EDGE && cnt && !windowed && dim >= 4 && (tune.sweep == 1 || auto_Bs > 0) && tune.deterministic != 1 &&
        sweep_supports(mode, dim, x_bytes)) {
        int Bs = B;
        if (auto_Bs > 0) {
            Bs = std::min(auto_Bs, S);
        } else if (tune.column_phases < 2) {
            Bs = std::max(2, std::min(std::min(std::min(16, 2 * B), std::max(2, partSize / 4)), S));
        }
        const int32_t *sw_ids = nullptr; const uint32_t *sw_off = nullptr;
        if (plan.handle && (tune.pack_ids == 1 || (tune.pack_ids == 0 && plan.pinned)) && tune.xcd_remap != 0) {
            rc = get_packed_ids(ds, stream, plan.handle, Bs, kWave, true, false, &sw_ids, &sw_off, &chk_sum, &chk_n, stale_flag, seq,
                                tune.ids_check_every);
            if (rc != GNNA_OK) return rc;
            if (sw_ids) count_event(CTR_PACKED_LAUNCHES);
        }
        uint32_t *sync = ds->sweep_sync + (size_t)call_block_of(ds, stream, seq) * kSweepSlotWords;
        static_assert(kXcds * 16 + 2 <= kBlock, "the prologue clears the sweep counters with one block");
        rc = run_prologue(0, sync, kXcds * 16 + 2);
        if (rc != GNNA_OK) return rc;
        SweepLaunch w;
        w.mode = mode; w.X = X; w.col = column_index; w.pp = part_pointers; w.p2n = part2Node; w.Y = out;
        w.cnt = cnt; w.row_scale = row_scale; w.flag = flag; w.seq = seq; w.trust = tune.trust_canonical ? 1 : 0; w.sync = sync;
        w.P = num_parts; w.D = dim; w.ldx = ldx; w.ldy = ldy; w.S = S; w.B = Bs;
        w.relu = relu; w.num_out_rows = num_nodes;
        w.U = std::max(tune.loads_in_flight, 8);
        w.rows_with_edges = plan.stats.valid ? (int64_t)std::min((double)num_nodes, plan.stats.groups) : num_nodes;
        if (tune.groups_per_chunk > 64) w.rounds = tune.groups_per_chunk / 64;
        w.slack = tune.sweep_slack; w.wgs_per_cu = tune.blocks_per_cu;
        w.dynamic = tune.xcd_remap != 0;
        w.plain_ok = !accumulate_into_out; w.eps = eps;
        w.ids_packed = sw_ids; w.item_off = sw_off; w.packed_stale = stale_flag;
        t_last_phases = Bs;
        t_last_launches = 1;
        rc = launch_sweep(ds, w, stream);
        if (rc != GNNA_OK) return rc;
        profile_record(prof_call, 2, stream);
        return GNNA_OK;
    }

    int G = std::min(64, tune.groups_per_chunk * B);
    if (mode == MODE_EDGE && cnt && !windowed && plan.handle && plan.pinned && (plan.stats.valid || tune.sweep == 1) &&
        tune.xcd_remap != 0) {
        const int Bs = sweep_phases_of_width(tune, dim, foot_bytes, x_bytes, num_nodes, num_in_rows, plan.stats, B, ds->num_cus,
                                             partSize, S);
        if (Bs >= 2) { B = Bs; G = kWave; }
    }
    t_last_phases = B;
    StreamLaunch a;
    a.mode = mode; a.X = X; a.col = column_index; a.pp = part_pointers; a.p2n = part2Node; a.Y = out;
    a.cnt = cnt; a.row_scale = row_scale; a.flag = flag; a.seq = seq;
    if (mode == MODE_EDGE) { a.deg_row = nullptr; a.deg_col = nullptr; a.edge_w = degrees_in; }
    else { a.deg_row = degrees; a.deg_col = degrees_in; }
    a.trust = tune.trust_canonical ? 1 : 0; a.P = num_parts;
    a.D = dim; a.ldx = ldx; a.ldy = ldy; a.G = G; a.U = tune.loads_in_flight; a.S = S; a.B = B;
    a.win_lo = win_lo; a.win_hi = win_hi; a.relu = relu; a.num_out_rows = num_nodes;
    t_last_launches = 1;
    a.wide = wide; a.plain_ok = (B == 1 && !accumulate_into_out && !windowed); a.xcd_remap = tune.xcd_remap != 0;
    a.eps = eps;
    if (tune.deterministic == 1 && !windowed) {
        const int G_eff = std::max(1, std::min(a.G, kWave));
        const size_t chunks = (size_t)((num_parts + G_eff - 1) / G_eff);
        const size_t part_bytes = ((chunks * 2 * (size_t)dim * sizeof(float)) + 255) & ~(size_t)255;
        const size_t stamp_bytes = chunks * 2 * sizeof(int32_t);
        void *ws = nullptr;
        rc = get_workspace(ds, stream, 2, part_bytes + stamp_bytes, &ws);
        if (rc != GNNA_OK) return rc;
        a.det = true;
        a.det_part = static_cast<float *>(ws);
        a.det_stamp = reinterpret_cast<int32_t *>(static_cast<char *>(ws) + part_bytes);
        hipError_t em = hipMemsetAsync(a.det_stamp, 0, stamp_bytes, stream);
        if (em != hipSuccess) return fail(GNNA_ERR_HIP, "deterministic schedule scratch: %s", hipGetErrorString(em));
        t_last_launches = B;
    }
    if (cnt && !windowed && plan.handle && (tune.pack_ids == 1 || (tune.pack_ids == 0 && plan.pinned))) {
        rc = get_packed_ids(ds, stream, plan.handle, B, std::max(1, std::min(a.G, kWave)), true, false, &a.ids_packed, &a.item_off,
                            &chk_sum, &chk_n, stale_flag, seq, tune.ids_check_every);
        a.packed_stale = stale_flag;
        if (rc != GNNA_OK) return rc;
        if (a.ids_packed) count_event(CTR_PACKED_LAUNCHES);
    }
    const bool sparse = !a.det && a.plain_ok && tune.zero_fill != 2 &&
                        (tune.zero_fill == 1 || n_floats * sizeof(float) >= ((size_t)32 << 20));
    rc = run_prologue(sparse ? std::max(1, std::min(a.G, kWave)) : 0);
    if (rc != GNNA_OK) return rc;
    rc = launch_stream(a, stream);
    if (rc != GNNA_OK) return rc;
    profile_record(prof_call, 2, stream);
    return GNNA_OK;
}

}
}

using namespace gnna;

extern "C" {
#pragma GCC visibility push(default)

int gnna_sag_f32(const float *input, const int32_t *row_pointers, const int32_t *column_index,
                 const float *degrees, const int32_t *part_pointers, const int32_t *part2Node,
                 float *out, int64_t num_nodes, int dim, int64_t num_parts,
                 int partSize, int dimWorker, int warpPerBlock, void *stream)
{
    (void)row_pointers; (void)degrees;
    return launch_agg(MODE_SAG, input, dim, num_nodes, column_index, nullptr, nullptr, 1.f, part_pointers,
                      part2Node, out, dim, num_nodes, dim, num_parts, partSize, dimWorker, warpPerBlock, stream, 0u);
}

int gnna_agg_gcn_f32(const float *input, const int32_t *row_pointers, const int32_t *column_index,
                     const float *degrees, const int32_t *part_pointers, const int32_t *part2Node,
                     float *out, int64_t num_nodes, int dim, int64_t num_parts,
                     int partSize, int dimWorker, int warpPerBlock, void *stream)
{
    (void)row_pointers;
    return launch_agg(MODE_GCN, input, dim, num_nodes, column_index, degrees, degrees, 1.f, part_pointers,
                      part2Node, out, dim, num_nodes, dim, num_parts, partSize, dimWorker, warpPerBlock, stream, 0u);
}

int gnna_agg_gin_f32(const float *input, const int32_t *row_pointers, const int32_t *column_index,
                     float epsilon, const int32_t *part_pointers, const int32_t *part2Node,
                     float *out, int64_t num_nodes, int dim, int64_t num_parts,
                     int partSize, int dimWorker, int warpPerBlock, void *stream)
{
    (void)row_pointers;
    return launch_agg(MODE_GIN, input, dim, num_nodes, column_index, nullptr, nullptr, epsilon, part_pointers,
                      part2Node, out, dim, num_nodes, dim, num_parts, partSize, dimWorker, warpPerBlock, stream, 0u);
}

int gnna_agg_rect_f32(int mode, const float *input, int64_t num_in_rows, const int32_t *column_index,
                      const float *degrees_out, const float *degrees_in, float epsilon,
                      const int32_t *part_pointers, const int32_t *part2Node, float *out,
                      int64_t num_out_rows, int dim, int64_t num_parts, int partSize, int accumulate,
                      void *stream)
{
    if (mode != MODE_SAG && mode != MODE_GCN && mode != MODE_GIN)
        return fail(GNNA_ERR_INVALID_ARGUMENT, "unknown mode %d", mode);
    return launch_agg(mode, input, dim, num_in_rows, column_index, degrees_out, degrees_in, epsilon, part_pointers,
                      part2Node, out, dim, num_out_rows, dim, num_parts, partSize, 32, 4, stream,
                      accumulate != 0 ? GNNA_ACCUMULATE : 0u);
}

int gnna_agg_ld_f32(int mode, const float *input, int64_t ld_in, int64_t num_in_rows, const int32_t *column_index,
                    const float *degrees_out, const float *degrees_in, float epsilon,
                    const int32_t *part_pointers, const int32_t *part2Node, float *out, int64_t ld_out,
                    int64_t num_out_rows, int dim, int64_t num_parts, int partSize, unsigned flags, void *stream)
{
    if (mode != MODE_SAG && mode != MODE_GCN && mode != MODE_GIN)
        return fail(GNNA_ERR_INVALID_ARGUMENT, "unknown mode %d", mode);
    return launch_agg(mode, input, ld_in, num_in_rows, column_index, degrees_out, degrees_in, epsilon, part_pointers,
                      part2Node, out, ld_out, num_out_rows, dim, num_parts, partSize, 32, 4, stream, flags);
}

int gnna_agg_rect_windows_f32(int mode, const float *input, int64_t num_in_rows, const int32_t *column_index,
                              const float *degrees_out, const float *degrees_in, float epsilon,
                              const int32_t *part_pointers, const int32_t *part2Node, float *out,
                              int64_t num_out_rows, int dim, int64_t num_parts, int partSize, int accumulate,
                              int num_windows, int window_begin, int window_end, void *stream)
{
    if (mode != MODE_SAG && mode != MODE_GCN && mode != MODE_GIN)
        return fail(GNNA_ERR_INVALID_ARGUMENT, "unknown mode %d", mode);
    return launch_agg(mode, input, dim, num_in_rows, column_index, degrees_out, degrees_in, epsilon, part_pointers,
                      part2Node, out, dim, num_out_rows, dim, num_parts, partSize, 32, 4, stream,
                      accumulate != 0 ? GNNA_ACCUMULATE : 0u, num_windows, window_begin, window_end);
}

int gnna_agg_edge_ld_f32(const float *input, int64_t ld_in, int64_t num_in_rows, const int32_t *column_index,
                         const float *edge_weight, const int32_t *part_pointers, const int32_t *part2Node, float *out,
                         int64_t ld_out, int64_t num_out_rows, int dim, int64_t num_parts, int partSize, unsigned flags,
                         void *stream)
{
    return launch_agg(MODE_EDGE, input, ld_in, num_in_rows, column_index, nullptr, edge_weight, 1.f, part_pointers,
                      part2Node, out, ld_out, num_out_rows, dim, num_parts, partSize, 32, 4, stream, flags);
}

int gnna_agg_ld_x16(int mode, int in_type, const void *input, int64_t ld_in, int64_t num_in_rows,
                    const int32_t *column_index, const float *degrees_out, const float *degrees_in, float epsilon,
                    const int32_t *part_pointers, const int32_t *part2Node, void *out, int out_type, int64_t ld_out,
                    int64_t num_out_rows, int dim, int64_t num_parts, int partSize, unsigned flags, void *stream_v)
{
    if (mode != MODE_SAG && mode != MODE_GCN && mode != MODE_GIN)
        return fail(GNNA_ERR_INVALID_ARGUMENT, "unknown mode %d", mode);
    if (in_type != GNNA_BF16 && in_type != GNNA_F16)
        return fail(GNNA_ERR_INVALID_ARGUMENT, "in_type must be GNNA_BF16 or GNNA_F16 (got %d)", in_type);
    if (out_type != GNNA_F32 && out_type != in_type)
        return fail(GNNA_ERR_INVALID_ARGUMENT, "out_type must be GNNA_F32 or the input's type (in_type=%d out_type=%d)", in_type, out_type);
    if (flags & ~(unsigned)(GNNA_ACCUMULATE | GNNA_EPILOGUE_RELU))
        return fail(GNNA_ERR_INVALID_ARGUMENT, "unknown flag bits 0x%x", flags);
    if (num_out_rows < 0 || dim < 0 || num_parts < 0 || num_in_rows < 0)
        return fail(GNNA_ERR_INVALID_ARGUMENT, "negative size (num_out_rows=%lld dim=%d num_parts=%lld)",
                    (long long)num_out_rows, dim, (long long)num_parts);
    if (partSize <= 0) return fail(GNNA_ERR_INVALID_ARGUMENT, "partSize must be positive (got %d)", partSize);
    if ((flags & GNNA_ACCUMULATE) && out_type != GNNA_F32)
        return fail(GNNA_ERR_UNSUPPORTED, "GNNA_ACCUMULATE with a 16-bit output would round the sum twice: accumulate into an fp32 output");
    if (num_out_rows >= ((int64_t)1 << 29))
        return fail(GNNA_ERR_UNSUPPORTED, "%lld destination rows in one call (at most 536870911): shard the rows", (long long)num_out_rows);
    if (num_out_rows == 0 || dim == 0) return GNNA_OK;
    if (bad_ld(ld_in, dim) || bad_ld(ld_out, dim))
        return fail(GNNA_ERR_INVALID_ARGUMENT, "row strides must be >= dim and < 2^29 elements (ld_in=%lld ld_out=%lld dim=%d)",
                    (long long)ld_in, (long long)ld_out, dim);
    if (!out || !input) return fail(GNNA_ERR_INVALID_ARGUMENT, "null feature pointer");
    if ((reinterpret_cast<uintptr_t>(input) & 1) || (reinterpret_cast<uintptr_t>(out) & (out_type == GNNA_F32 ? 3 : 1)))
        return fail(GNNA_ERR_INVALID_ARGUMENT, "feature pointers must be aligned to their element size");
    if (num_parts > 0 && (!column_index || !part_pointers || !part2Node))
        return fail(GNNA_ERR_INVALID_ARGUMENT, "null index pointer");
    if (mode == MODE_GCN && (!degrees_out || !degrees_in)) return fail(GNNA_ERR_INVALID_ARGUMENT, "null degrees pointer");
    if (out == input) return fail(GNNA_ERR_INVALID_ARGUMENT, "out must not alias input");
    int rc = deterministic_refused("gnna_agg_ld_x16",
                                   "its rows meet in fp32 through float atomics; use gnna_agg_ld_f32 on fp32 features");
    if (rc != GNNA_OK) return rc;
    hipStream_t stream = static_cast<hipStream_t>(stream_v);
    DeviceState *ds = nullptr;
    rc = get_device_state(&ds);
    if (rc != GNNA_OK) return rc;
    X16Launch c;
    c.mode = mode; c.in_type = in_type; c.out_type = out_type; c.input = input; c.ld_in = ld_in; c.num_in_rows = num_in_rows;
    c.column_index = column_index; c.degrees_out = degrees_out; c.degrees_in = degrees_in; c.epsilon = epsilon;
    c.part_pointers = part_pointers; c.part2Node = part2Node; c.out = out; c.ld_out = ld_out; c.num_out_rows = num_out_rows;
    c.dim = dim; c.num_parts = num_parts; c.partSize = partSize;
    c.accumulate = (flags & GNNA_ACCUMULATE) != 0; c.relu = (flags & GNNA_EPILOGUE_RELU) != 0; c.xcd_remap = xcd_remap_on() != 0;
    c.prof_call = profile_acquire_call(num_parts > 0);
    profile_record(c.prof_call, 0, stream);
    t_last_phases = 1;
    t_last_launches = 1;
    rc = launch_x16(ds, stream, c);
    if (rc != GNNA_OK) return rc;
    profile_record(c.prof_call, 2, stream);
    return GNNA_OK;
}

int gnna_prepare_x16(int64_t num_in_rows, int64_t num_out_rows, const int *dims, int num_dims, void *stream_v)
{
    if (num_in_rows < 0 || num_out_rows < 0 || num_dims < 0 || (num_dims > 0 && !dims))
        return fail(GNNA_ERR_INVALID_ARGUMENT, "gnna_prepare_x16: bad argument");
    hipStream_t stream = static_cast<hipStream_t>(stream_v);
    hipStreamCaptureStatus cap = hipStreamCaptureStatusNone;
    (void)hipStreamIsCapturing(stream, &cap);
    if (cap != hipStreamCaptureStatusNone)
        return fail(GNNA_ERR_UNSUPPORTED, "gnna_prepare_x16 allocates: call it before the capture");
    DeviceState *ds = nullptr;
    int rc = get_device_state(&ds);
    if (rc != GNNA_OK) return rc;
    for (int i = 0; i < num_dims; i++) {
        if (dims[i] <= 0) return fail(GNNA_ERR_INVALID_ARGUMENT, "gnna_prepare_x16: dims[%d] = %d", i, dims[i]);
        rc = reserve_x16(ds, stream, num_in_rows, num_out_rows, dims[i]);
        if (rc != GNNA_OK) return rc;
    }
    return GNNA_OK;
}

int64_t gnna_preferred_ld(int dim, int64_t num_in_rows, int64_t num_edges)
{
    if (dim <= 0 || num_in_rows <= 0) return dim > 0 ? dim : 0;
    gnna_tuning tune;
    gnna_get_tuning(&tune);
    const bool hot = num_edges >= 32 * num_in_rows && (size_t)num_in_rows * (size_t)dim * sizeof(float) <= ((size_t)1 << 30);
    return dim < 4 ? dim : pick_row_stride(tune, dim, hot, num_in_rows, true);
}

int gnna_prepare_graph(const int32_t *column_index, const int32_t *part_pointers, const int32_t *part2Node,
                       int64_t num_parts, int64_t num_in_rows, int64_t num_out_rows, int partSize,
                       const int *dims, int num_dims, int *phases_out, void *stream_v)
{
    if (num_parts < 0 || num_in_rows < 0 || num_out_rows < 0 || partSize <= 0 || num_dims < 0 || (num_dims > 0 && !dims))
        return fail(GNNA_ERR_INVALID_ARGUMENT, "gnna_prepare_graph: bad argument");
    for (int i = 0; i < num_dims; i++)
        if (phases_out) phases_out[i] = 1;
    if (num_parts == 0) return GNNA_OK;
    if (!column_index || !part_pointers || !part2Node) return fail(GNNA_ERR_INVALID_ARGUMENT, "null index pointer");
    hipStream_t stream = static_cast<hipStream_t>(stream_v);
    hipStreamCaptureStatus cap = hipStreamCaptureStatusNone;
    (void)hipStreamIsCapturing(stream, &cap);
    if (cap != hipStreamCaptureStatusNone)
        return fail(GNNA_ERR_UNSUPPORTED, "gnna_prepare_graph synchronises and allocates: call it before the capture");
    DeviceState *ds = nullptr;
    int rc = get_device_state(&ds);
    if (rc != GNNA_OK) return rc;
    drain_dead_buffers();
    LaunchGuard in_flight;
    SlicePlan plan;
    rc = get_slice_plan(ds, stream, column_index, part_pointers, part2Node, num_parts, num_in_rows, true, true, &plan);
    if (rc != GNNA_OK) return rc;
    if (!plan.cnt || !plan.stats.valid) return fail(GNNA_ERR_HIP, "gnna_prepare_graph: the slice plan could not be built");
    gnna_tuning tune;
    gnna_get_tuning(&tune);
    const bool hot = plan.stats.edges >= 32.0 * (double)num_in_rows;
    size_t staged = 0, det_bytes = 0;
    std::vector<std::pair<int, int>> widths;
    for (int i = 0; i < num_dims; i++) {
        if (dims[i] <= 0) return fail(GNNA_ERR_INVALID_ARGUMENT, "gnna_prepare_graph: dims[%d] = %d", i, dims[i]);
        const int nb = column_blocks(tune, dims[i], num_in_rows, (int64_t)plan.stats.edges);
        if (nb <= 1) { widths.emplace_back(i, dims[i]); continue; }
        const int w = ((dims[i] + nb - 1) / nb + 3) / 4 * 4;
        widths.emplace_back(i, w);
        if (dims[i] % w) widths.emplace_back(i, dims[i] % w);
    }
    for (const auto &wd : widths) {
        const int i = wd.first;
        const int dim = wd.second;
        gnna_tuning t = tune;
        apply_graph_hints(column_index, dims[i], &t);
        const size_t raw = (size_t)num_in_rows * (size_t)dim * sizeof(float);
        const bool hot_rows = hot && raw <= ((size_t)1 << 30);
        const int ldx = pick_row_stride(t, dim, hot_rows, num_in_rows, true);
        const size_t x_bytes = (size_t)num_in_rows * (size_t)ldx * sizeof(float);
        const size_t foot_bytes = gather_footprint_bytes(num_in_rows, ldx, dim);
        if (hot_rows || t.gcn_prescale == 1 || ldx != dim) staged = std::max(staged, x_bytes);
        int B = 1;
        const bool can_slice = num_parts >= 1024 && num_in_rows >= 64 && foot_bytes >= ((size_t)2 << 20);
        {
            if (t.column_phases >= 2 && num_in_rows >= kMaxSlices) B = std::min(t.column_phases, kMaxSlices);
            else if (t.column_phases == 0 && can_slice && foot_bytes >= ((size_t)6 << 20))
                B = choose_slices(plan.stats, foot_bytes, plan.S, plan.slice_rows, num_out_rows, num_in_rows == num_out_rows,
                                  t.nonlocal_ids == 1);
        }
        const bool first_of_width = &wd == &widths.front() || (&wd - 1)->first != i;
        if (phases_out) phases_out[i] = first_of_width ? std::max(1, B) : std::max(phases_out[i], std::max(1, B));
        if (B >= 2 && t.pack_ids != 2 && plan.handle) {
            const int32_t *ids = nullptr; const uint32_t *off = nullptr;
            const int Bs = sweep_phases_of_width(t, dim, foot_bytes, x_bytes, num_out_rows, num_in_rows, plan.stats, B, ds->num_cus,
                                                 partSize, plan.S);
            const bool swept = Bs >= 2 && t.xcd_remap != 0;
            if (swept) rc = get_packed_ids(ds, stream, plan.handle, Bs, kWave, true, true, &ids, &off);
            if (rc == GNNA_OK && (!swept || t.gcn_prescale == 2))
                rc = get_packed_ids(ds, stream, plan.handle, B, std::max(1, std::min(kWave, t.groups_per_chunk * B)), true, true, &ids, &off);
            if (rc != GNNA_OK) return rc;
            if (phases_out && Bs >= 2) phases_out[i] = first_of_width ? Bs : std::max(phases_out[i], Bs);
        }
        if (t.deterministic == 1 && dim >= 4) {
            const int G_eff = std::max(1, std::min(kWave, t.groups_per_chunk * std::max(1, B)));
            const size_t chunks = (size_t)((num_parts + G_eff - 1) / G_eff);
            det_bytes = std::max(det_bytes, (((chunks * 2 * (size_t)dim * sizeof(float)) + 255) & ~(size_t)255) +
                                                chunks * 2 * sizeof(int32_t));
        }
    }
    if (det_bytes) {
        void *ws = nullptr;
        rc = get_workspace(ds, stream, 2, det_bytes, &ws);
        if (rc != GNNA_OK) return rc;
    }
    if (staged) {
        void *ws = nullptr;
        rc = get_workspace(ds, stream, 1, staged, &ws);
        if (rc != GNNA_OK) return rc;
    }
    return GNNA_OK;
}

int gnna_release_graph(const int32_t *column_index)
{
    (void)release_slice_plans(column_index, false);
    return gnna_set_graph_hints(column_index, 0, 0);
}

int gnna_forget_graph(const int32_t *column_index)
{
    if (!column_index) return fail(GNNA_ERR_INVALID_ARGUMENT, "gnna_forget_graph: null (gnna_release_graph(NULL) drops everything)");
    (void)release_slice_plans(column_index, true);
    return gnna_set_graph_hints(column_index, 0, 0);
}

int gnna_forget_plans(const int32_t *column_index)
{
    if (!column_index) return fail(GNNA_ERR_INVALID_ARGUMENT, "gnna_forget_plans: null column_index");
    (void)release_slice_plans(column_index, true);
    return GNNA_OK;
}

int gnna_last_num_phases(void) { return t_last_phases; }
int gnna_last_num_launches(void) { return t_last_launches; }

#pragma GCC visibility pop
}
```

gnnadvisor_osdi21_amd/csrc/gnna_internal.h:

```cpp
#ifndef GNNA_INTERNAL_H_
#define GNNA_INTERNAL_H_

#include <hip/hip_runtime.h>

#include <atomic>
#include <cstddef>
#include <cstdint>
#include <map>
#include <utility>
#include <vector>

#include "gnna.h"
#include "gnna_launch.h"

namespace gnna {

int fail(int code, const char *fmt, ...) __attribute__((format(printf, 2, 3)));

int host_thread_budget(int cap);

void apply_graph_hints(const void *column_index, int dim, gnna_tuning *tune);

int launch_ok(const char *prefix_fmt, ...) __attribute__((format(printf, 1, 2)));
inline int xcd_remap_on()
{
    gnna_tuning tune;
    gnna_get_tuning(&tune);
    return tune.xcd_remap != 0 ? 1 : 0;
}
inline int deterministic_refused(const char *what, const char *reason)
{
    gnna_tuning tune;
    gnna_get_tuning(&tune);
    if (tune.deterministic != 1) return GNNA_OK;
    return fail(GNNA_ERR_UNSUPPORTED, "%s has no deterministic schedule (gnna_tuning.deterministic = 1): %s", what, reason);
}

struct Workspace {
    void *ptr = nullptr;
    size_t bytes = 0;
};
struct CaptureKey {
    unsigned long long capture_id;
    hipStream_t stream;
    int slot;
    bool operator<(const CaptureKey &o) const
    {
        if (capture_id != o.capture_id) return capture_id < o.capture_id;
        if (stream != o.stream) return stream < o.stream;
        return slot < o.slot;
    }
};
struct DeviceState {
    std::atomic<bool> init{false};
    int num_cus = 256;
    int32_t *flags = nullptr;
    unsigned long long *gap_lists = nullptr;
    uint32_t *sweep_sync = nullptr;
    std::map<hipStream_t, int> stream_block;
    int captured_blocks = 0;
    std::map<std::pair<hipStream_t, int>, Workspace> ws;
    std::map<CaptureKey, Workspace> capture_ws;
    std::vector<void *> capture_outgrown;
};
constexpr int kFlagSlots = 1024;
constexpr int kGapEntries = 63, kGapWords = 2 + 2 * kGapEntries;
constexpr int kStreamBlocks = 64, kCapturedBlocks = 160, kCallBlocks = 256;
static_assert(kCallBlocks <= kFlagSlots && kStreamBlocks + kCapturedBlocks < kCallBlocks, "call blocks");

int get_device_state(DeviceState **out);
int get_workspace(DeviceState *ds, hipStream_t stream, int slot, size_t bytes, void **out);
int32_t next_call_seq(DeviceState *ds, hipStream_t stream, int32_t **flag_slot);
int call_block_of(DeviceState *ds, hipStream_t stream, int32_t seq);

constexpr int kMaxSlices = 32;
constexpr int kSliceLevels = 5;
struct SlicePlanStats {
    bool valid = false;
    double cells[kSliceLevels] = {0, 0, 0, 0, 0};
    double edges = 0, groups = 0;
    double span = 0;
    double unsorted = 0;
    double near[24] = {0};
};
struct SlicePlan {
    const uint8_t *cnt = nullptr;
    int S = 0;
    uint32_t slice_rows = 0;
    SlicePlanStats stats;
    void *handle = nullptr;
    bool pinned = false;
};
inline uint32_t slice_rows_for(int64_t num_in_rows)
{
    const int64_t r = (num_in_rows + kMaxSlices - 1) / kMaxSlices;
    return (uint32_t)(r < 1 ? 1 : r);
}
int get_slice_plan(DeviceState *ds, hipStream_t stream, const int32_t *column_index, const int32_t *part_pointers,
                   const int32_t *part2Node, int64_t num_parts, int64_t num_in_rows, bool want_stats, bool pin,
                   SlicePlan *out, uint32_t window_rows = 0);
void drop_slice_plans();
int get_packed_ids(DeviceState *ds, hipStream_t stream, void *plan_handle, int B, int G, bool may_build, bool force,
                   const int32_t **ids, const uint32_t **item_off, const unsigned long long **checksum = nullptr,
                   int64_t *num_ids = nullptr, int32_t *stale_flag = nullptr, int32_t seq = 0, int check_every = 0);
int launch_ids_sample_check(hipStream_t stream, const int32_t *col, int64_t n, const int32_t *pp, int64_t P,
                            const unsigned long long *state, int32_t *stale_flag, int32_t seq);
int release_slice_plans(const void *column_index, bool deferred);
void drain_dead_buffers();
void begin_launch();
void end_launch();
struct LaunchGuard {
    LaunchGuard() { begin_launch(); }
    ~LaunchGuard() { end_launch(); }
    LaunchGuard(const LaunchGuard &) = delete;
    LaunchGuard &operator=(const LaunchGuard &) = delete;
};
int stage_rows_for_gather(DeviceState *ds, hipStream_t stream, const gnna_tuning &tune, const float *input, int64_t ld_in,
                          int64_t num_in_rows, int dim, int64_t est_edges, const float **X, int *ldx_out);
int choose_slices(const SlicePlanStats &st, size_t x_bytes, int S, uint32_t slice_rows, int64_t num_out_rows,
                  bool square, bool hinted_scattered);
enum { CTR_PLAN_BUILDS = 0, CTR_LAUNCH_SYNCS = 1, CTR_LAUNCH_FREES = 2, CTR_LAUNCH_MALLOCS = 3, CTR_BACKOFF_SKIPS = 4,
       CTR_SWEEP_LAUNCHES = 5, CTR_PACK_BUILDS = 6, CTR_PACKED_LAUNCHES = 7, CTR_FULL_HASHES = 8, CTR_CAPTURE_SCRATCH = 9,
       CTR_COUNT = 10 };
void count_event(int which);

struct StreamLaunch {
    int mode;
    const float *X; const int32_t *col; const int32_t *pp; const int32_t *p2n; float *Y;
    const uint8_t *cnt;
    const float *row_scale;
    const float *deg_row; const float *deg_col;
    const float *A = nullptr;
    const float *edge_w = nullptr;
    const int32_t *flag; int32_t seq; int32_t trust;
    int64_t P;
    int D, ldx, G, U, S, B;
    int lda = 0;
    int ldy = 0;
    int win_lo = 0, win_hi = 0;
    bool relu = false;
    int64_t num_out_rows = 0;
    bool wide, plain_ok, xcd_remap;
    float eps;
    bool det = false;
    float *det_part = nullptr; int32_t *det_stamp = nullptr;
    const int32_t *ids_packed = nullptr; const uint32_t *item_off = nullptr;
    const int32_t *packed_stale = nullptr;
};
int launch_stream(const StreamLaunch &a, hipStream_t stream);
int launch_stream_epilogue_only(const StreamLaunch &a, hipStream_t stream);

struct SweepLaunch {
    int mode;
    const float *X; const int32_t *col; const int32_t *pp; const int32_t *p2n; float *Y;
    const uint8_t *cnt;
    const float *row_scale;
    const int32_t *flag; int32_t seq; int32_t trust;
    uint32_t *sync;
    int64_t P;
    int D, ldx, U, S, B;
    int ldy = 0;
    bool relu = false;
    int64_t num_out_rows = 0;
    int rounds = 0;
    int64_t rows_with_edges = 0;
    int slack = 0;
    int wgs_per_cu = 0;
    bool dynamic = true;
    bool plain_ok;
    float eps;
    const int32_t *ids_packed = nullptr; const uint32_t *item_off = nullptr;
    const int32_t *packed_stale = nullptr;
};
bool sweep_supports(int mode, int dim, size_t x_bytes);
int sweep_acc_rows(int dim, int wgs_per_cu);
int launch_sweep(DeviceState *ds, const SweepLaunch &a, hipStream_t stream);
int sweep_auto_phases(const gnna_tuning &t, int mode, int dim, size_t x_bytes, int64_t num_out_rows, int64_t num_in_rows,
                      const SlicePlanStats &st, int B, int num_cus, bool deterministic, int part_size);
constexpr int kSweepListCap = 1023;
constexpr int kSweepSlotWords = 8 * 16 + 2 + 2 * kSweepListCap;

struct X16Launch {
    int mode;
    int in_type, out_type;
    const void *input; int64_t ld_in, num_in_rows;
    const int32_t *column_index; const float *degrees_out; const float *degrees_in; float epsilon;
    const int32_t *part_pointers; const int32_t *part2Node;
    void *out; int64_t ld_out, num_out_rows;
    int dim; int64_t num_parts; int partSize;
    bool accumulate, relu, xcd_remap;
    int prof_call = -1;
};
int launch_x16(DeviceState *ds, hipStream_t stream, const X16Launch &c);
int reserve_x16(DeviceState *ds, hipStream_t stream, int64_t num_in_rows, int64_t num_out_rows, int dim);
int launch_zero_fill(DeviceState *ds, hipStream_t stream, float *out, int64_t rows, int dim, int64_t ld);
void launch_relu_rows(DeviceState *ds, hipStream_t stream, float *out, int64_t rows, int dim, int64_t ld);

int64_t scan_tiles(int64_t n);
int launch_exclusive_scan(hipStream_t stream, int32_t *data, int64_t n, int32_t *partial);
int refuse_capture(const char *what, hipStream_t stream);

int profile_acquire_call(bool has_work);
void profile_record(int call, int which, hipStream_t stream);

}

#endif
```

gnnadvisor_osdi21_amd/csrc/gnna_stream.hip:

```cpp
#include <hip/hip_runtime.h>

#include <algorithm>
#include <cstdint>
#include <cstdio>
#include <cstdlib>
#include <atomic>
#include <mutex>
#include <vector>

#include "gnna.h"
#include "gnna_device.h"
#include "gnna_internal.h"

namespace gnna {
namespace {

constexpr int kIdSlots = 512;
#ifndef GNNA_NARROW_SLOTS
#define GNNA_NARROW_SLOTS 1024
#endif
template <int LPR, int MODE>
constexpr int id_slots() { return (LPR == 4 && MODE != MODE_GCN && MODE != MODE_EDGE && MODE != MODE_SDDMM) ? GNNA_NARROW_SLOTS : kIdSlots; }

struct StreamParams {
// ... 447 lines not shown
                        if (fresh(jn + u)) a[u] = a_load(jn + u);
                        v[u] = *row_ptr(nn[u]);
                    }
                }
#pragma unroll
                for (int u = 0; u < U; u++) {
                    const int j = (nb - 1) * U + u;
                    if (j < nr) dot_of(u, j);
                }
#pragma unroll
                for (int q = 0; q < (RL * RPI + kWave - 1) / kWave; q++) {
                    const int f = q * kWave + lane;
                    const int j = f / RPI, sl = f % RPI;
                    const int ej = __shfl(o_j, j), vj = __shfl(v_j, j);
                    if (f < RL * RPI && j < nr && sl < vj) {
                        float dot = pend[f];
                        float *dst = p.Y + ej + sl;
                        if (d0 > 0) dot += *dst;
                        *dst = dot;
                    }
                }
                continue;
            }
#pragma unroll
            for (int u = 0; u < U; u++) v[u] = *row_ptr(offs[u * RPI + slot]);
            auto consume = [&](int u, int j) {
                if ((TM >> j) & 1ull) {
                    const int vj = __builtin_amdgcn_readlane(v_j, j);
                    if (slot >= vj) v[u] = vzero<4>();
                }
                if constexpr (PER_EDGE) {
                    const VT tmp = v[u] * cfs[j * RPI + slot];
                    acc += tmp;
                } else {
                    acc += v[u];
                }
                if ((FL >> j) & 1ull) {
                    const int meta = __builtin_amdgcn_readlane(k_meta, j);
                    float scale = p.eps;
                    if constexpr (MODE == MODE_GIN) {
                        if (p.row_scale) scale *= p.row_scale[meta >> 2];
                    }
                    const VT r = fold_row<LPR, MODE>(acc, scale);
                    if (npend == PEND) { drain(); }
                    park_row<LPR>(r, pend + npend * PEND_FLOATS, dcol - d0, cvalid, lane, slot);
                    pend_meta = lane == npend ? meta : pend_meta;
                    npend++;
                    acc = vzero<4>();
                }
            };
#pragma unroll 1
            for (int b = 0; b + 1 < nb; b++) {
                const int jn = (b + 1) * U;
                uint32_t nn[U];
#pragma unroll
                for (int u = 0; u < U; u++) nn[u] = offs[(jn + u) * RPI + slot];
#pragma unroll
                for (int u = 0; u < U; u++) {
                    consume(u, b * U + u);
                    v[u] = *row_ptr(nn[u]);
                }
            }
#pragma unroll
            for (int u = 0; u < U; u++) {
                const int j = (nb - 1) * U + u;
                if (j < nr) consume(u, j);
            }
            if (npend > PEND / 2 || r0 + RL >= L) drain();
        }
    }
}

__global__ void __launch_bounds__(kBlock)
det_fixup_kernel(const int32_t *__restrict__ p2n, int64_t P, int G, int64_t num_chunks, float *__restrict__ Y, int D, int ldy,
                 const float *__restrict__ part, int32_t *__restrict__ stamps, int32_t stamp)
{
    const int lane = threadIdx.x & (kWave - 1);
    const int64_t wave = ((int64_t)blockIdx.x * blockDim.x + threadIdx.x) >> 6;
    const int64_t nwaves = ((int64_t)gridDim.x * blockDim.x) >> 6;
    for (int64_t c = wave; c < num_chunks; c += nwaves) {
        const int64_t g0 = c * G;
        const int64_t g1 = g0 + G < P ? g0 + G : P;
        const int rf = p2n[g0], rl = p2n[g1 - 1];
        const int prev = g0 > 0 ? p2n[g0 - 1] : -1, next = g1 < P ? p2n[g1] : -1;
        const bool head = next == rl && !(rl == rf && prev == rf);
        if (!head) continue;
        for (int d0 = 0; d0 < D; d0 += kWave) {
            const int i = d0 + lane;
            float acc = 0.f;
            if (stamps[c * 2 + 1] == stamp && i < D) acc = part[((size_t)c * 2 + 1) * (size_t)D + i];
            for (int64_t j = c + 1; j < num_chunks; j++) {
                const int64_t h0 = j * G;
                const int64_t h1 = h0 + G < P ? h0 + G : P;
                if (p2n[h0] != rl) break;
                if (stamps[j * 2] == stamp && i < D) acc += part[((size_t)j * 2) * (size_t)D + i];
                if (!(p2n[h1 - 1] == rl && h1 < P && p2n[h1] == rl)) break;
            }
            if (i < D) Y[(size_t)rl * (size_t)ldy + i] += acc;
        }
        if (lane == 0) {
            if (stamps[c * 2 + 1] == stamp) stamps[c * 2 + 1] = 0;
            for (int64_t j = c + 1; j < num_chunks; j++) {
                const int64_t h0 = j * G;
                const int64_t h1 = h0 + G < P ? h0 + G : P;
                if (p2n[h0] != rl) break;
                if (stamps[j * 2] == stamp) stamps[j * 2] = 0;
                if (!(p2n[h1 - 1] == rl && h1 < P && p2n[h1] == rl)) break;
            }
        }
    }
}

__global__ void __launch_bounds__(kBlock)
relu_fixup_kernel(float *__restrict__ Y, int64_t N, int D, int ldy, const int32_t *__restrict__ p2n, int64_t P, int G,
                  const int32_t *flag, int32_t seq, int whole)
{
    const int lane = threadIdx.x & (kWave - 1);
    const int64_t wave = ((int64_t)blockIdx.x * blockDim.x + threadIdx.x) >> 6;
    const int64_t nwaves = ((int64_t)gridDim.x * blockDim.x) >> 6;
    if (whole || *flag == seq) {
        for (int64_t r = wave; r < N; r += nwaves) {
            float *row = Y + (size_t)r * (size_t)ldy;
            for (int i = lane; i < D; i += kWave) row[i] = fmaxf(row[i], 0.f);
        }
        return;
    }
    const int64_t num_chunks = (P + G - 1) / G;
    for (int64_t c = 1 + wave; c < num_chunks; c += nwaves) {
        const int64_t g0 = c * G;
        const int r = p2n[g0];
        if (p2n[g0 - 1] != r || r < 0 || r >= N) continue;
        float *row = Y + (size_t)r * (size_t)ldy;
        for (int i = lane; i < D; i += kWave) row[i] = fmaxf(row[i], 0.f);
    }
}

__device__ __forceinline__ int group_part(const int32_t *__restrict__ pp, const uint8_t *__restrict__ cnt, int64_t P, int S, int B,
                                          int phase, int64_t g, int *first)
{
    const int pa = pp[g], pb = pp[g + 1];
    const int f_lo = phase * S / B, f_hi = (phase + 1) * S / B;
    int cum_lo = 0, cum_hi = 0x7fffffff;
    if (f_lo > 0) cum_lo = cnt[(size_t)(f_lo - 1) * (size_t)P + (size_t)g];
    if (f_hi < S) cum_hi = cnt[(size_t)(f_hi - 1) * (size_t)P + (size_t)g];
    const int len = pb > pa ? pb - pa : 0;
    const int beg = cum_lo < len ? cum_lo : len;
    int end = cum_hi < len ? cum_hi : len;
    end = end > beg ? end : beg;
    *first = pa + beg;
    return end - beg;
}

__global__ void __launch_bounds__(kBlock)
item_count_kernel(const int32_t *__restrict__ pp, const uint8_t *__restrict__ cnt, int64_t P, int64_t num_chunks, int G, int S, int B,
                  uint32_t *__restrict__ counts)
{
    const int lane = threadIdx.x & (kWave - 1);
    const int64_t wave = ((int64_t)blockIdx.x * blockDim.x + threadIdx.x) >> 6;
    const int64_t nwaves = ((int64_t)gridDim.x * blockDim.x) >> 6;
    const int64_t items = num_chunks * B;
    for (int64_t q = wave; q < items; q += nwaves) {
        const int phase = (int)(q / num_chunks);
        const int64_t g = (q % num_chunks) * G + lane;
        int first = 0;
        const int n = (lane < G && g < P) ? group_part(pp, cnt, P, S, B, phase, g, &first) : 0;
        const int tot = __builtin_amdgcn_readlane(wave_inclusive_scan(n), kWave - 1);
        if (lane == 0) counts[q] = (uint32_t)tot;
    }
}

__global__ void __launch_bounds__(1024)
item_scan_kernel(uint32_t *__restrict__ v, int64_t n)
{
    __shared__ uint32_t part[1024];
    const int64_t per = (n + 1023) / 1024;
    const int64_t lo = (int64_t)threadIdx.x * per, hi = lo + per < n ? lo + per : n;
    uint32_t sum = 0;
    for (int64_t i = lo; i < hi; i++) sum += v[i];
    part[threadIdx.x] = sum;
    __syncthreads();
    for (int off = 1; off < 1024; off <<= 1) {
        const uint32_t add = threadIdx.x >= (unsigned)off ? part[threadIdx.x - off] : 0u;
        __syncthreads();
        part[threadIdx.x] += add;
        __syncthreads();
    }
    uint32_t run = part[threadIdx.x] - sum;
    for (int64_t i = lo; i < hi; i++) { const uint32_t c = v[i]; v[i] = run; run += c; }
    if (threadIdx.x == 1023) v[n] = part[1023];
}

__global__ void __launch_bounds__(kBlock)
item_pack_kernel(const int32_t *__restrict__ col, const int32_t *__restrict__ pp, const uint8_t *__restrict__ cnt, int64_t P,
                 int64_t num_chunks, int G, int S, int B, const uint32_t *__restrict__ item_off, int32_t *__restrict__ out)
{
    const int lane = threadIdx.x & (kWave - 1);
    const int64_t wave = ((int64_t)blockIdx.x * blockDim.x + threadIdx.x) >> 6;
    const int64_t nwaves = ((int64_t)gridDim.x * blockDim.x) >> 6;
    const int64_t items = num_chunks * B;
    for (int64_t q = wave; q < items; q += nwaves) {
        const int phase = (int)(q / num_chunks);
        const int64_t g = (q % num_chunks) * G + lane;
        int first = 0;
        const int n = (lane < G && g < P) ? group_part(pp, cnt, P, S, B, phase, g, &first) : 0;
        const int incl = wave_inclusive_scan(n);
        int32_t *dst = out + item_off[q] + (uint32_t)(incl - n);
        for (int j = 0; j < n; j++) dst[j] = col[first + j];
    }
}

__global__ void __launch_bounds__(kWave)
ids_checksum_kernel(const int32_t *__restrict__ col, int64_t n, const int32_t *__restrict__ pp, int64_t P,
                    unsigned long long *__restrict__ out)
{
    const unsigned long long v = graph_checksum(col, n, pp, P, (int)threadIdx.x);
    if (threadIdx.x == 0) *out = v;
}

__device__ __forceinline__ unsigned long long mix_id(unsigned long long pos, uint32_t id, unsigned long long salt)
{
    unsigned long long x = ((pos << 32) | (unsigned long long)id) ^ salt;
    x ^= x >> 30; x *= 0xbf58476d1ce4e5b9ull;
    x ^= x >> 27; x *= 0x94d049bb133111ebull;
    return x ^ (x >> 31);
}

__global__ void __launch_bounds__(kBlock)
ids_full_hash_kernel(const int32_t *__restrict__ col, int64_t n, const int32_t *__restrict__ pp, int64_t P,
                     unsigned long long *__restrict__ state, int store, int32_t *stale_flag, int32_t seq)
{
    const int64_t tid = (int64_t)blockIdx.x * blockDim.x + threadIdx.x, nthreads = (int64_t)gridDim.x * blockDim.x;
    unsigned long long sum = 0;
    const bool vec = (reinterpret_cast<uintptr_t>(col) & 15) == 0;
    const int64_t n4 = vec ? n >> 2 : 0;
    typedef int i32x4 __attribute__((ext_vector_type(4)));
    for (int64_t i = tid; i < n4; i += nthreads) {
        const i32x4 v = __builtin_nontemporal_load(reinterpret_cast<const i32x4 *>(col) + i);
        const unsigned long long b = (unsigned long long)i << 2;
        sum += mix_id(b, (uint32_t)v.x, 0) + mix_id(b + 1, (uint32_t)v.y, 0) + mix_id(b + 2, (uint32_t)v.z, 0) + mix_id(b + 3, (uint32_t)v.w, 0);
    }
    for (int64_t i = (n4 << 2) + tid; i < n; i += nthreads) sum += mix_id((unsigned long long)i, (uint32_t)col[i], 0);
    for (int64_t i = tid; i <= P; i += nthreads) sum += mix_id((unsigned long long)i, (uint32_t)pp[i], 0x9E3779B97F4A7C15ull);
    for (int d = 32; d > 0; d >>= 1) sum += __shfl_xor(sum, d);
    __shared__ unsigned long long part[kBlock / kWave];
    __shared__ bool last;
    if ((threadIdx.x & (kWave - 1)) == 0) part[threadIdx.x / kWave] = sum;
    __syncthreads();
    if (threadIdx.x == 0) {
        unsigned long long t = 0;
        for (int w = 0; w < kBlock / kWave; w++) t += part[w];
        atomicAdd(&state[2], t);
        __threadfence();
        last = atomicAdd(&state[3], 1ull) == (unsigned long long)gridDim.x - 1ull;
        if (last) {
            __threadfence();
            const unsigned long long total = atomicAdd(&state[2], 0ull);
            if (store) { state[1] = total; state[4] = 0ull; }
            else if (total != state[1]) { state[4] = 1ull; if (stale_flag) *stale_flag = seq; }
            state[2] = 0ull; state[3] = 0ull;
            __threadfence();
        }
    }
}

__global__ void __launch_bounds__(kWave)
ids_sample_check_kernel(const int32_t *__restrict__ col, int64_t n, const int32_t *__restrict__ pp, int64_t P,
                        const unsigned long long *__restrict__ state, int32_t *stale_flag, int32_t seq)
{
    const unsigned long long now = graph_checksum(col, n, pp, P, (int)threadIdx.x);
    if (threadIdx.x == 0 && (now != state[0] || state[4] != 0ull)) *stale_flag = seq;
}

struct Plan {
    const void *col = nullptr, *pp = nullptr, *p2n = nullptr;
    int64_t P = 0;
    uint32_t slice_rows = 0;
    int device = -1;
    uint8_t *cnt = nullptr;
    size_t bytes = 0;
    hipEvent_t ready = nullptr;
    hipStream_t made_on = nullptr;
    hipStream_t last_stream = nullptr;
    bool multi_stream = false;
    SliceStats stats{};
    bool have_stats = false;
    bool pinned = false;
    uint64_t stamp = 0;
    uint32_t uses = 0;
    struct Packed {
        int B = 0, G = 0;
        int32_t *ids = nullptr;
        uint32_t *item_off = nullptr;
        unsigned long long *checksum = nullptr;
        uint64_t hits = 0;
        int64_t num_ids = 0;
        hipEvent_t ready = nullptr;
        hipStream_t made_on = nullptr;
        hipEvent_t hashed = nullptr;
        uint64_t stamp = 0;
    };
    std::vector<Packed> packed;
    uint64_t pack_lookups = 0;
    uint64_t pack_no_memory_until = 0;
};
constexpr uint64_t kPackedNoMemoryBackoff = 1024;
constexpr int kMaxPacked = 4;
constexpr uint64_t kPackedKeep = 16;
constexpr int kMaxPlans = 32;
std::vector<Plan *> g_plans;
std::mutex g_plan_mutex;
uint64_t g_plan_clock = 0;
constexpr int kColdStreak = 8;
int g_cold_evictions = 0;
int g_skip_builds = 0;
std::atomic<long long> g_counters[CTR_COUNT];

std::vector<void *> g_dead;
std::atomic<int> g_in_flight{0};

void drain_dead_locked(int allowed_in_flight)
{
    if (g_dead.empty() || g_in_flight.load(std::memory_order_acquire) > allowed_in_flight) return;
    for (void *ptr : g_dead) (void)hipFree(ptr);
    g_dead.clear();
}

size_t stats_offset(int64_t P) { return (((size_t)P * (size_t)(kMaxSlices - 1)) + 255) & ~(size_t)255; }

typedef void (*StreamKernel)(const StreamParams);

template <int LPR, int MODE>
StreamKernel pick_stream_wide(bool wide, int u)
{
    constexpr int RPI = kWave / LPR;
    constexpr int RL = (id_slots<LPR, MODE>() / RPI < kWave) ? id_slots<LPR, MODE>() / RPI : kWave;
    if constexpr (RL % 8 == 0) {
        if (u >= 8) return wide ? stream_kernel<LPR, MODE, 8, true> : stream_kernel<LPR, MODE, 8, false>;
    }
    return wide ? stream_kernel<LPR, MODE, 4, true> : stream_kernel<LPR, MODE, 4, false>;
}

template <int MODE>
StreamKernel pick_stream_lpr(int lpr, bool wide, int u)
{
    switch (lpr) {
    case 4: return pick_stream_wide<4, MODE>(wide, u);
    case 8: return pick_stream_wide<8, MODE>(wide, u);
    case 16: return pick_stream_wide<16, MODE>(wide, u);
    case 32: return pick_stream_wide<32, MODE>(wide, u);
    default: return pick_stream_wide<64, MODE>(wide, u);
    }
}

}

void count_event(int which) { g_counters[which].fetch_add(1, std::memory_order_relaxed); }

int get_slice_plan(DeviceState *ds, hipStream_t stream, const int32_t *column_index, const int32_t *part_pointers,
                   const int32_t *part2Node, int64_t num_parts, int64_t num_in_rows, bool want_stats, bool pin,
                   SlicePlan *out, uint32_t window_rows)
{
    *out = SlicePlan();
    const int S = kMaxSlices;
    const uint32_t slice_rows = window_rows ? window_rows : slice_rows_for(num_in_rows);
    int dev = 0;
    (void)hipGetDevice(&dev);
    std::lock_guard<std::mutex> lock(g_plan_mutex);
    Plan *hit = nullptr, *victim = nullptr;
    int unpinned = 0;
    for (Plan *pl : g_plans) {
        if (pl->col == column_index && pl->pp == part_pointers && pl->p2n == part2Node && pl->P == num_parts &&
            pl->slice_rows == slice_rows && pl->device == dev) { hit = pl; break; }
        if (!pl->pinned) {
            unpinned++;
            if (pl->device == dev && (!victim || pl->stamp < victim->stamp)) victim = pl;
        }
    }
    bool rebuild = false;
    if (hit && want_stats && !hit->have_stats) rebuild = true;
    if (!hit || rebuild) {
        hipStreamCaptureStatus cap = hipStreamCaptureStatusNone;
        (void)hipStreamIsCapturing(stream, &cap);
        if (cap != hipStreamCaptureStatusNone) return GNNA_OK;
        if (!hit && !pin && want_stats && window_rows == 0 && g_skip_builds > 0) {
            g_skip_builds--;
            count_event(CTR_BACKOFF_SKIPS);
            return GNNA_OK;
        }
        Plan *pl = hit;
        const size_t bytes = stats_offset(num_parts) + sizeof(SliceStats);
        if (!pl) {
            if (unpinned >= kMaxPlans && victim) {
                pl = victim;
                if (pl->uses <= 1) {
                    if (++g_cold_evictions >= kColdStreak) { g_skip_builds = 64; g_cold_evictions = 0; }
                } else {
                    g_cold_evictions = 0;
                }
            } else {
                pl = new Plan();
                g_plans.push_back(pl);
            }
        }
        if (pl->cnt && (pl->multi_stream || (pl->last_stream != stream && pl->uses > 0))) {
            (void)hipDeviceSynchronize();
            count_event(CTR_LAUNCH_SYNCS);
        }
        if (pl->bytes < bytes) {
            drain_dead_locked(1);
            if (pl->cnt) { (void)hipFree(pl->cnt); count_event(CTR_LAUNCH_FREES); }
            pl->cnt = nullptr; pl->bytes = 0;
            hipError_t e = hipMalloc(reinterpret_cast<void **>(&pl->cnt), bytes);
            count_event(CTR_LAUNCH_MALLOCS);
            if (e != hipSuccess) {
                pl->col = nullptr;
                return fail(GNNA_ERR_HIP, "hipMalloc(slice counts %zu B): %s", bytes, hipGetErrorString(e));
            }
            pl->bytes = bytes;
        }
        if (!pl->ready) (void)hipEventCreateWithFlags(&pl->ready, hipEventDisableTiming);
        for (auto &pk : pl->packed) {
            if (pk.ids) { (void)hipFree(pk.ids); count_event(CTR_LAUNCH_FREES); }
            if (pk.ready) (void)hipEventDestroy(pk.ready);
            if (pk.hashed) (void)hipEventDestroy(pk.hashed);
        }
        pl->packed.clear();
        pl->col = column_index; pl->pp = part_pointers; pl->p2n = part2Node; pl->P = num_parts; pl->slice_rows = slice_rows;
        pl->device = dev; pl->have_stats = false; pl->made_on = stream; pl->last_stream = stream; pl->multi_stream = false;
        pl->uses = 0;
        SliceStats *stats_dev = reinterpret_cast<SliceStats *>(pl->cnt + stats_offset(num_parts));
        (void)hipMemsetAsync(stats_dev, 0, sizeof(SliceStats), stream);
        int64_t blocks = std::max<int64_t>(1, std::min<int64_t>((num_parts + kWavesPerBlock - 1) / kWavesPerBlock,
                                                                  (int64_t)ds->num_cus * 16));
        hipLaunchKernelGGL(slice_count_kernel, dim3((unsigned)blocks), dim3(kBlock), 0, stream, column_index,
                           part_pointers, part2Node, num_parts, slice_rows, S, pl->cnt, stats_dev);
        count_event(CTR_PLAN_BUILDS);
        hipError_t e = hipGetLastError();
        if (e != hipSuccess) { pl->col = nullptr; return fail(GNNA_ERR_HIP, "slice count launch: %s", hipGetErrorString(e)); }
        if (want_stats) {
            e = hipMemcpyAsync(&pl->stats, stats_dev, sizeof(SliceStats), hipMemcpyDeviceToHost, stream);
            if (e == hipSuccess) e = hipStreamSynchronize(stream);
            if (!pin) count_event(CTR_LAUNCH_SYNCS);
            if (e != hipSuccess) { pl->col = nullptr; return fail(GNNA_ERR_HIP, "slice statistics: %s", hipGetErrorString(e)); }
            pl->have_stats = true;
        }
        (void)hipEventRecord(pl->ready, stream);
        hit = pl;
    } else if (hit->made_on != stream) {
        hipStreamCaptureStatus cap = hipStreamCaptureStatusNone;
        (void)hipStreamIsCapturing(stream, &cap);
        if (cap == hipStreamCaptureStatusNone) (void)hipStreamWaitEvent(stream, hit->ready, 0);
    }
    if (hit->uses > 0 && hit->last_stream != stream) hit->multi_stream = true;
    hit->last_stream = stream;
    hit->uses++;
    if (hit->uses > 1) { g_cold_evictions = 0; g_skip_builds = 0; }
    if (pin) hit->pinned = true;
    hit->stamp = ++g_plan_clock;
    out->cnt = hit->cnt;
    out->handle = hit;
    out->pinned = hit->pinned;
    out->S = S;
    out->slice_rows = slice_rows;
    out->stats.valid = hit->have_stats;
    for (int i = 0; i < kSliceLevels; i++) out->stats.cells[i] = (double)hit->stats.cells[i];
    out->stats.edges = (double)hit->stats.edges;
    out->stats.groups = (double)hit->stats.groups;
    out->stats.span = (double)hit->stats.span;
    out->stats.unsorted = (double)hit->stats.unsorted;
    for (int i = 0; i < 24; i++) out->stats.near[i] = (double)hit->stats.near[i];
    return GNNA_OK;
}

int release_slice_plans(const void *column_index, bool deferred)
{
    std::lock_guard<std::mutex> lock(g_plan_mutex);
    int dropped = 0;
    if (!column_index) { g_cold_evictions = 0; g_skip_builds = 0; }
    for (size_t i = 0; i < g_plans.size();) {
        Plan *pl = g_plans[i];
        if (column_index && pl->col != column_index) { i++; continue; }
        if (pl->cnt) g_dead.push_back(pl->cnt);
        if (pl->ready) (void)hipEventDestroy(pl->ready);
        for (auto &pk : pl->packed) {
            if (pk.ids) g_dead.push_back(pk.ids);
            if (pk.ready) (void)hipEventDestroy(pk.ready);
            if (pk.hashed) (void)hipEventDestroy(pk.hashed);
        }
        delete pl;
        g_plans.erase(g_plans.begin() + (long)i);
        dropped++;
    }
    if (!deferred) drain_dead_locked(0);
    return dropped;
}

void begin_launch()
{
    std::lock_guard<std::mutex> lock(g_plan_mutex);
    g_in_flight.fetch_add(1, std::memory_order_acq_rel);
}

void end_launch() { g_in_flight.fetch_sub(1, std::memory_order_acq_rel); }

void drain_dead_buffers()
{
    std::lock_guard<std::mutex> lock(g_plan_mutex);
    drain_dead_locked(0);
}

void drop_slice_plans() { (void)release_slice_plans(nullptr, false); }

int launch_ids_sample_check(hipStream_t stream, const int32_t *col, int64_t n, const int32_t *pp, int64_t P,
                            const unsigned long long *state, int32_t *stale_flag, int32_t seq)
{
    hipLaunchKernelGGL(ids_sample_check_kernel, dim3(1), dim3(kWave), 0, stream, col, n, pp, P, state, stale_flag, seq);
    hipError_t e = hipGetLastError();
    return e == hipSuccess ? GNNA_OK : fail(GNNA_ERR_HIP, "packed ids check launch: %s", hipGetErrorString(e));
}

static void launch_full_hash(DeviceState *ds, hipStream_t stream, const Plan *pl, Plan::Packed &pk, int64_t nnz, int store,
                             int32_t *stale_flag, int32_t seq)
{
    if (!pk.hashed) (void)hipEventCreateWithFlags(&pk.hashed, hipEventDisableTiming);
    else (void)hipStreamWaitEvent(stream, pk.hashed, 0);
    const int64_t work = (nnz + 3) / 4 + pl->P + 1;
    const int64_t blocks = std::max<int64_t>(1, std::min<int64_t>((work + kBlock - 1) / kBlock, (int64_t)ds->num_cus * 8));
    hipLaunchKernelGGL(ids_full_hash_kernel, dim3((unsigned)blocks), dim3(kBlock), 0, stream, static_cast<const int32_t *>(pl->col), nnz,
                       static_cast<const int32_t *>(pl->pp), pl->P, pk.checksum, store, stale_flag, seq);
    (void)hipEventRecord(pk.hashed, stream);
}

int get_packed_ids(DeviceState *ds, hipStream_t stream, void *plan_handle, int B, int G, bool may_build, bool force,
                   const int32_t **ids, const uint32_t **item_off, const unsigned long long **checksum, int64_t *num_ids,
                   int32_t *stale_flag, int32_t seq, int check_every)
{
    *ids = nullptr; *item_off = nullptr;
    if (checksum) *checksum = nullptr;
    if (num_ids) *num_ids = 0;
    if (!plan_handle || B < 2 || G < 1) return GNNA_OK;
    std::lock_guard<std::mutex> lock(g_plan_mutex);
    Plan *pl = nullptr;
    for (Plan *q : g_plans) if (q == plan_handle) { pl = q; break; }
    if (!pl || !pl->cnt) return GNNA_OK;
    hipStreamCaptureStatus cap = hipStreamCaptureStatusNone;
    (void)hipStreamIsCapturing(stream, &cap);
    pl->pack_lookups++;
    for (auto &pk : pl->packed) {
        if (pk.B == B && pk.G == G && pk.ids) {
            if (pk.made_on != stream && cap == hipStreamCaptureStatusNone) (void)hipStreamWaitEvent(stream, pk.ready, 0);
            pk.stamp = pl->pack_lookups;
            if (stale_flag && check_every > 0 && check_every < (1 << 30) && cap == hipStreamCaptureStatusNone &&
                ++pk.hits % (uint64_t)check_every == 0) {
                launch_full_hash(ds, stream, pl, pk, pk.num_ids, 0, stale_flag, seq);
                count_event(CTR_FULL_HASHES);
            }
            *ids = pk.ids; *item_off = pk.item_off;
            if (checksum) *checksum = pk.checksum;
            if (num_ids) *num_ids = pk.num_ids;
            return GNNA_OK;
        }
    }
    if (!may_build || cap != hipStreamCaptureStatusNone) return GNNA_OK;
    if (!force && pl->pack_lookups < pl->pack_no_memory_until) return GNNA_OK;
    const int64_t num_chunks = (pl->P + G - 1) / G;
    const int64_t items = num_chunks * B;
    int64_t nnz = 0;
    hipError_t e = hipSuccess;
    if (pl->have_stats) {
        nnz = (int64_t)pl->stats.edges;
    } else {
        int32_t last = 0;
        e = hipMemcpyAsync(&last, static_cast<const int32_t *>(pl->pp) + pl->P, sizeof(int32_t), hipMemcpyDeviceToHost, stream);
        if (e == hipSuccess) e = hipStreamSynchronize(stream);
        count_event(CTR_LAUNCH_SYNCS);
        if (e != hipSuccess) return fail(GNNA_ERR_HIP, "packed ids (edge count): %s", hipGetErrorString(e));
        nnz = last;
    }
    if (nnz <= 0 || nnz > 0x7fffffffLL) return GNNA_OK;
    Plan::Packed *slot = nullptr;
    if ((int)pl->packed.size() < kMaxPacked) {
        pl->packed.emplace_back();
        slot = &pl->packed.back();
    } else {
        for (auto &pk : pl->packed) if (!slot || !pk.ids || (slot->ids && pk.stamp < slot->stamp)) slot = &pk;
        if (slot->ids) {
            if (!force && pl->pack_lookups - slot->stamp < kPackedKeep) return GNNA_OK;
            (void)hipDeviceSynchronize();
            count_event(CTR_LAUNCH_SYNCS);
            (void)hipFree(slot->ids); count_event(CTR_LAUNCH_FREES);
        }
        slot->ids = nullptr; slot->item_off = nullptr;
    }
    const size_t id_bytes = (((size_t)nnz * sizeof(int32_t)) + 255) & ~(size_t)255;
    const size_t off_bytes = ((((size_t)items + 1) * sizeof(uint32_t)) + 15) & ~(size_t)15;
    const size_t bytes = id_bytes + off_bytes + 64;
    e = hipMalloc(reinterpret_cast<void **>(&slot->ids), bytes);
    count_event(CTR_LAUNCH_MALLOCS);
    if (e != hipSuccess) {
        (void)hipGetLastError();
        slot->ids = nullptr; slot->item_off = nullptr; slot->B = 0; slot->G = 0;
        if (slot->ready) { (void)hipEventDestroy(slot->ready); slot->ready = nullptr; }
        if (slot->hashed) { (void)hipEventDestroy(slot->hashed); slot->hashed = nullptr; }
        if (slot == &pl->packed.back()) pl->packed.pop_back();
        else slot->stamp = pl->pack_lookups;
        pl->pack_no_memory_until = pl->pack_lookups + kPackedNoMemoryBackoff;
        return GNNA_OK;
    }
    slot->item_off = reinterpret_cast<uint32_t *>(reinterpret_cast<char *>(slot->ids) + id_bytes);
    slot->checksum = reinterpret_cast<unsigned long long *>(reinterpret_cast<char *>(slot->ids) + id_bytes + off_bytes);
    slot->num_ids = nnz;
    slot->B = B; slot->G = G; slot->made_on = stream; slot->stamp = pl->pack_lookups;
    if (!slot->ready) (void)hipEventCreateWithFlags(&slot->ready, hipEventDisableTiming);
    const int64_t blocks = std::max<int64_t>(1, std::min<int64_t>((items + kWavesPerBlock - 1) / kWavesPerBlock, (int64_t)ds->num_cus * 16));
    hipLaunchKernelGGL(item_count_kernel, dim3((unsigned)blocks), dim3(kBlock), 0, stream, static_cast<const int32_t *>(pl->pp),
                       pl->cnt, pl->P, num_chunks, G, kMaxSlices, B, slot->item_off);
    hipLaunchKernelGGL(item_scan_kernel, dim3(1), dim3(1024), 0, stream, slot->item_off, items);
    hipLaunchKernelGGL(item_pack_kernel, dim3((unsigned)blocks), dim3(kBlock), 0, stream, static_cast<const int32_t *>(pl->col),
                       static_cast<const int32_t *>(pl->pp), pl->cnt, pl->P, num_chunks, G, kMaxSlices, B, slot->item_off, slot->ids);
    hipLaunchKernelGGL(ids_checksum_kernel, dim3(1), dim3(kWave), 0, stream, static_cast<const int32_t *>(pl->col), nnz,
                       static_cast<const int32_t *>(pl->pp), pl->P, slot->checksum);
    (void)hipMemsetAsync(slot->checksum + 1, 0, 7 * sizeof(unsigned long long), stream);
    launch_full_hash(ds, stream, pl, *slot, nnz, 1, nullptr, 0);
    slot->hits = 0;
    e = hipGetLastError();
    if (e != hipSuccess) return fail(GNNA_ERR_HIP, "packed ids launch: %s", hipGetErrorString(e));
    (void)hipEventRecord(slot->ready, stream);
    count_event(CTR_PACK_BUILDS);
    *ids = slot->ids; *item_off = slot->item_off;
    if (checksum) *checksum = slot->checksum;
    if (num_ids) *num_ids = slot->num_ids;
    return GNNA_OK;
}

static int launch_relu_fixup(const StreamLaunch &a, int G, bool whole, hipStream_t stream)
{
    if (!a.relu || a.mode == MODE_SDDMM) return GNNA_OK;
    const int64_t units = std::max<int64_t>(a.num_out_rows, (a.P + G - 1) / G);
    const int64_t blocks = std::max<int64_t>(1, std::min<int64_t>((units + kWavesPerBlock - 1) / kWavesPerBlock, 256 * 8));
    hipLaunchKernelGGL(relu_fixup_kernel, dim3((unsigned)blocks), dim3(kBlock), 0, stream, a.Y, a.num_out_rows, a.D,
                       a.ldy > 0 ? a.ldy : a.D, a.p2n, a.P, G, a.flag, a.seq, whole ? 1 : 0);
    hipError_t e = hipGetLastError();
    if (e != hipSuccess) return fail(GNNA_ERR_HIP, "epilogue launch: %s", hipGetErrorString(e));
    return GNNA_OK;
}

int launch_stream_epilogue_only(const StreamLaunch &a, hipStream_t stream)
{
    return launch_relu_fixup(a, 1, true, stream);
}

int launch_stream(const StreamLaunch &a, hipStream_t stream)
{
    StreamParams p;
    p.X = a.X; p.col = a.col; p.pp = a.pp; p.p2n = a.p2n; p.Y = a.Y; p.cnt = a.cnt; p.row_scale = a.row_scale;
    p.deg_row = a.deg_row; p.deg_col = a.deg_col; p.edge_w = a.edge_w; p.A = a.A;
    p.flag = a.flag; p.P = a.P; p.seq = a.seq; p.trust = a.trust; p.D = a.D; p.ldx = a.ldx;
    p.DL = std::max(a.D, 4); p.ldy = a.ldy > 0 ? a.ldy : a.D; p.lda = a.lda > 0 ? a.lda : a.D;
    p.G = std::max(1, std::min(a.G, kWave));
    p.num_chunks = (a.P + p.G - 1) / p.G;
    int64_t items = (p.num_chunks + kSWaves - 1) / kSWaves;
    p.xcd_remap = a.xcd_remap ? 1 : 0;
    if (p.xcd_remap) items = (items + kXcds - 1) / kXcds * kXcds;
    p.blocks_per_phase = items;
    p.S = a.cnt ? a.S : 1; p.B = a.cnt ? a.B : 1; p.phase_lo = 0;
    p.win_lo = 0; p.win_hi = p.S;
    if (a.cnt && a.win_hi > a.win_lo) { p.win_lo = a.win_lo; p.win_hi = std::min(a.win_hi, p.S); }
    p.plain_ok = a.plain_ok ? 1 : 0;
    const bool relu_in_kernel = a.relu && a.mode != MODE_SDDMM && p.B == 1 && a.plain_ok && !a.det;
    p.relu = relu_in_kernel ? 1 : 0;
    p.eps = a.eps;
    const int64_t grid = items * (int64_t)p.B;
    if (grid > 0x7fffffffLL) return fail(GNNA_ERR_UNSUPPORTED, "aggregation grid too large (%lld blocks)", (long long)grid);
    int lpr = 4;
    const int pieces = (p.DL + 3) / 4;
    while (lpr < 64 && lpr < pieces) lpr <<= 1;
    StreamKernel k = a.mode == MODE_GIN ? pick_stream_lpr<MODE_GIN>(lpr, a.wide, a.U)
                     : (a.mode == MODE_GCN ? pick_stream_lpr<MODE_GCN>(lpr, a.wide, a.U)
                     : (a.mode == MODE_EDGE ? pick_stream_lpr<MODE_EDGE>(lpr, a.wide, a.U)
                     : (a.mode == MODE_SDDMM ? pick_stream_lpr<MODE_SDDMM>(lpr, a.wide, a.U) : pick_stream_lpr<MODE_SAG>(lpr, a.wide, a.U))));
    p.det = 0; p.det_part = nullptr; p.det_stamp = nullptr; p.stamp = 0;
    p.ids_packed = !a.packed_stale ? nullptr : a.ids_packed; p.item_off = a.item_off;
    p.packed_stale = a.packed_stale;
    if (a.det && a.mode != MODE_SDDMM) {
        p.det = 1; p.det_part = a.det_part; p.det_stamp = a.det_stamp;
        int64_t fblocks = std::max<int64_t>(1, std::min<int64_t>((p.num_chunks + kWavesPerBlock - 1) / kWavesPerBlock, 65535));
        for (int ph = 0; ph < p.B; ph++) {
            p.phase_lo = ph;
            p.stamp = (int32_t)((((uint32_t)a.seq & 0x1ffffffu) << 6) | (uint32_t)ph);
            hipLaunchKernelGGL(k, dim3((unsigned)items), dim3(kSBlock), 0, stream, p);
            hipLaunchKernelGGL(det_fixup_kernel, dim3((unsigned)fblocks), dim3(kBlock), 0, stream, a.p2n, a.P, p.G, p.num_chunks,
                               a.Y, a.D, p.ldy, a.det_part, a.det_stamp, p.stamp);
        }
        hipError_t e = hipGetLastError();
        if (e != hipSuccess) return fail(GNNA_ERR_HIP, "aggregation launch: %s", hipGetErrorString(e));
        return launch_relu_fixup(a, p.G, true, stream);
    }
    hipLaunchKernelGGL(k, dim3((unsigned)grid), dim3(kSBlock), 0, stream, p);
    hipError_t e = hipGetLastError();
    if (e != hipSuccess) return fail(GNNA_ERR_HIP, "aggregation launch: %s", hipGetErrorString(e));
    return launch_relu_fixup(a, p.G, !relu_in_kernel, stream);
}

}

extern "C" {
#pragma GCC visibility push(default)
void gnna_runtime_counters(int64_t out[8])
{
    for (int i = 0; i < 8; i++) out[i] = i < gnna::CTR_COUNT ? (int64_t)gnna::g_counters[i].load() : 0;
}
int gnna_runtime_counters_ex(int64_t *out, int capacity)
{
    for (int i = 0; i < capacity && i < gnna::CTR_COUNT; i++) out[i] = (int64_t)gnna::g_counters[i].load();
    return gnna::CTR_COUNT;
}
int gnna_debug_untrusted_copies(const int32_t *column_index)
{
    hipError_t e = hipDeviceSynchronize();
    if (e != hipSuccess) return gnna::fail(GNNA_ERR_HIP, "hipDeviceSynchronize: %s", hipGetErrorString(e));
    std::lock_guard<std::mutex> lock(gnna::g_plan_mutex);
    int untrusted = 0;
    for (gnna::Plan *pl : gnna::g_plans) {
        if (pl->col != column_index) continue;
        for (auto &pk : pl->packed) {
            if (!pk.ids || !pk.checksum) continue;
            unsigned long long mark = 0;
            e = hipMemcpy(&mark, pk.checksum + 4, sizeof(mark), hipMemcpyDeviceToHost);
            if (e != hipSuccess) return gnna::fail(GNNA_ERR_HIP, "reading a packed copy's state: %s", hipGetErrorString(e));
            if (mark != 0ull) untrusted++;
        }
    }
    return untrusted;
}
#pragma GCC visibility pop
}
```

gnnadvisor_osdi21_amd/csrc/gnna_sweep.hip:

```cpp
#include <hip/hip_runtime.h>

#include <algorithm>
#include <cmath>
#include <cstdint>

#include "gnna.h"
#include "gnna_device.h"
#include "gnna_internal.h"

namespace gnna {
namespace {

constexpr int kSweepIdSlots = 512;
constexpr int kSweepBlock = 1024;
constexpr int kSweepWaves = kSweepBlock / kWave;
constexpr int kSweepLockWords = 128;

template <int LPR, int WGS> constexpr int acc_floats()
{
    return WGS == 1 ? (LPR >= 16 ? 32768 : 28672) : (LPR >= 16 ? 15360 : 11264);
}

__device__ __forceinline__ void lds_add(float *p, float v)
{
    typedef __attribute__((address_space(3))) float lds_float;
    (void)__hip_atomic_fetch_add((lds_float *)p, v, __ATOMIC_RELAXED, __HIP_MEMORY_SCOPE_WORKGROUP);
}

struct SweepParams {
    const float *X;
    const int32_t *col;
    const int32_t *pp;
    const int32_t *p2n;
    float *Y;
    const uint8_t *cnt;
    const float *row_scale;
    const int32_t *flag;
    uint32_t *sync;
    int64_t P;
    int32_t seq;
    int32_t trust;
    int32_t D;
    int32_t ldx;
    int32_t ldy;
    int32_t relu;
    int32_t S;
    int32_t B;
    int32_t rounds;
    int32_t plain_ok;
    int32_t dynamic;
    int32_t slack;
    float eps;
    const int32_t *ids_packed;
    const uint32_t *item_off;
    const int32_t *packed_stale;
    int64_t num_chunks;
};

__device__ __forceinline__ int64_t lower_bound64(const int32_t *__restrict__ pp, int64_t P, int64_t target, int lane)
{
    int64_t lo = 0, hi = P;
    while (hi > lo) {
        const int64_t span = hi - lo;
        const int64_t idx = lo + (span * lane) / kWave;
        const bool below = (int64_t)pp[idx] < target;
        const int c = __popcll(__ballot(below));
        if (c == 0) { hi = lo; break; }
        const int64_t new_lo = lo + (span * (c - 1)) / kWave + 1;
        const int64_t new_hi = c < kWave ? lo + (span * c) / kWave : hi;
        lo = new_lo;
        hi = new_hi > new_lo ? new_hi : new_lo;
    }
    return lo;
}

__device__ __forceinline__ int64_t sweep_set_start(int64_t i, int64_t num_sets, int64_t nnz, const int32_t *__restrict__ pp,
                                                   int64_t P, bool canonical, bool align64, int lane)
{
    const int64_t target = i >= num_sets ? nnz : (nnz * i) / num_sets;
    int64_t g = i <= 0 ? 0 : (i >= num_sets ? P : (canonical ? lower_bound64(pp, P, target, lane) : (P * i) / num_sets));
    if (align64 && g < P) g &= ~(int64_t)(kWave - 1);
    return g;
}

__global__ void __launch_bounds__(kBlock)
sweep_relu_fixup_kernel(float *__restrict__ Y, int64_t N, int D, int ldy, const uint32_t *__restrict__ list,
                        const int32_t *flag, int32_t seq, int32_t trust, int whole)
{
    const int lane = threadIdx.x & (kWave - 1);
    const int64_t wave = ((int64_t)blockIdx.x * blockDim.x + threadIdx.x) >> 6;
    const int64_t nwaves = ((int64_t)gridDim.x * blockDim.x) >> 6;
    const bool canonical = trust || (*flag != seq);
    auto clamp_row = [&](int64_t r) {
        float *row = Y + (size_t)r * (size_t)ldy;
        for (int i = lane; i < D; i += kWave) row[i] = fmaxf(row[i], 0.f);
    };
    if (whole || !canonical || list[1] != 0u) {
        for (int64_t r = wave; r < N; r += nwaves) clamp_row(r);
        return;
    }
    const uint32_t n = list[0] < (uint32_t)kSweepListCap ? list[0] : (uint32_t)kSweepListCap;
    for (int64_t i = wave; i < (int64_t)n; i += nwaves) {
        const int64_t first = (int64_t)list[2 + 2 * i], cnt = (int64_t)list[3 + 2 * i];
        for (int64_t r = first; r < first + cnt && r < N; r++) clamp_row(r);
    }
}

template <int LPR, int MODE, int U, int WGS>
__global__ void __launch_bounds__(kSweepBlock) __attribute__((amdgpu_waves_per_eu(4 * WGS, 4 * WGS)))
sweep_kernel(const SweepParams p)
{
    typedef typename VecOf<4>::T VT;
    typedef typename VecOf<4>::M MT;
    constexpr int RPI = kWave / LPR;
    constexpr int RL = (kSweepIdSlots / RPI < kWave) ? kSweepIdSlots / RPI : kWave;
    static_assert(RL % U == 0, "a round is a whole number of batches");
    constexpr int ACC = acc_floats<LPR, WGS>();
    __shared__ float s_acc[ACC];
    __shared__ uint32_t s_off[kSweepWaves][RL * RPI];
    __shared__ int64_t s_g[2];
    __shared__ int s_ctl[8];
    __shared__ unsigned s_lock[kSweepLockWords];

    const int lane = threadIdx.x & (kWave - 1);
    const int wib = __builtin_amdgcn_readfirstlane((int)threadIdx.x >> 6);
    const int lslot = lane / LPR;
    const int c = lane % LPR;
    const int D = p.D;
    const bool canonical = p.trust || (*p.flag != p.seq);
    const bool stale_ids = p.ids_packed != nullptr && *p.packed_stale == p.seq;
    const char *xbase = reinterpret_cast<const char *>(p.X);
    const uint32_t row_bytes32 = (uint32_t)p.ldx * 4u;
    uint32_t *offs = s_off[wib];
    const int CAP = ACC / D;
    const unsigned long long upto = (2ull << lane) - 1ull;
    const unsigned long long above = ~upto;

    const int piece = c * 4;
    const bool cvalid = piece < D;
    int dcol = piece, shift = 0;
    if (piece + 4 > D && cvalid) { dcol = D - 4; shift = piece - dcol; }
    const uint32_t col_off = (uint32_t)(cvalid ? dcol : 0) * 4u;
    const int comp = lane >> 4;
    const bool add_lane = LPR <= 16 ? ((lane & 15) < LPR && cvalid && comp >= shift) : (lslot == 0 && cvalid);

    const int xcd = (int)(blockIdx.x & (kXcds - 1));
    const int nbx = (int)(gridDim.x >> 3);
    const int bx = (int)(blockIdx.x >> 3);
    uint32_t *ctr = p.sync + xcd * 16;
    const bool syncing = p.slack < 1000 && nbx > 1;
    const int B = p.B, R = p.rounds;
    const int64_t nnz = (int64_t)p.pp[p.P];
    const int64_t num_sets = (int64_t)gridDim.x * R;

    if (threadIdx.x == 0) { s_ctl[2] = 0; s_ctl[3] = 0; }

    for (int r = 0; r < R; r++) {
        const int64_t set = ((int64_t)xcd * nbx + bx) * R + r;
        if (wib < 2) {
            const int64_t g = sweep_set_start(set + wib, num_sets, nnz, p.pp, p.P, canonical, p.ids_packed != nullptr, lane);
            if (lane == 0) s_g[wib] = g;
        }
        if (threadIdx.x == 0) { s_ctl[0] = 0; s_ctl[1] = 0; }
        __syncthreads();
        const int64_t g_lo = s_g[0], g_hi = s_g[1];
        int row_first = 0, row_last = -1, set_prev_row = -1, set_next_row = -1;
        if (g_hi > g_lo) {
            row_first = p.p2n[g_lo];
            row_last = p.p2n[g_hi - 1];
            if (g_lo > 0) set_prev_row = p.p2n[g_lo - 1];
            if (g_hi < p.P) set_next_row = p.p2n[g_hi];
        }
        int nrows = 0;
        if (canonical && row_last >= row_first) nrows = row_last - row_first + 1 < CAP ? row_last - row_first + 1 : CAP;
        if (p.relu && canonical && threadIdx.x == 0 && g_hi > g_lo) {
            uint32_t *list = p.sync + kXcds * 16;
            auto push = [&](int first, int cnt) {
                const uint32_t idx = atomicAdd(&list[0], 1u);
                if (idx < (uint32_t)kSweepListCap) { list[2 + 2 * idx] = (uint32_t)first; list[3 + 2 * idx] = (uint32_t)cnt; }
                else list[1] = 1u;
            };
            if (set_prev_row == row_first) push(row_first, 1);
            const int over_rows = row_last - row_first + 1 - CAP;
            if (over_rows > 2048) list[1] = 1u;
            else
                for (int r0 = 0; r0 < over_rows; r0 += 16) push(row_first + CAP + r0, over_rows - r0 < 16 ? over_rows - r0 : 16);
        }
        for (int i = threadIdx.x; i < nrows * D; i += kSweepBlock) s_acc[i] = 0.f;
        __syncthreads();

        const int64_t ng_set = g_hi - g_lo;
        const int nchunks = (int)((ng_set + kWave - 1) / kWave);
        const bool dyn = p.dynamic != 0 && nchunks <= kSweepLockWords * 32;
        const int64_t gw_lo = dyn ? g_lo : g_lo + (ng_set * wib) / kSweepWaves;
        const int64_t gw_hi = dyn ? g_hi : g_lo + (ng_set * (wib + 1)) / kSweepWaves;
        const int nch_w = (int)((gw_hi - gw_lo + kWave - 1) / kWave);
        const int per_step = nch_w > 0 ? nch_w : 1;
        if (dyn)
            for (int i = threadIdx.x; i < kSweepLockWords; i += kSweepBlock) s_lock[i] = 0u;
        __syncthreads();
        const int total_items = dyn ? nchunks * B : per_step * B;
        int it = 0, last_T = -1;
        while (true) {
            int item = it++;
            if (dyn) {
                if (lane == 0) item = __hip_atomic_fetch_add(&s_ctl[0], 1, __ATOMIC_RELAXED, __HIP_MEMORY_SCOPE_WORKGROUP);
                item = __builtin_amdgcn_readfirstlane(item);
            }
            if (item >= total_items) break;
            const int t = item / per_step;
            const int chunk = item - t * per_step;
            const int T = r * B + t;
            const int64_t g0 = gw_lo + (int64_t)chunk * kWave;
            const int ng = nch_w > 0 ? (int)(gw_hi - g0 < (int64_t)kWave ? gw_hi - g0 : (int64_t)kWave) : 0;

            if (syncing && T >= p.slack && T != last_T) {
                const uint32_t need = (uint32_t)nbx * (uint32_t)(T - p.slack + 1);
                const int seen = __hip_atomic_load(&s_ctl[2], __ATOMIC_RELAXED, __HIP_MEMORY_SCOPE_WORKGROUP);
                const int gave_up = __hip_atomic_load(&s_ctl[3], __ATOMIC_RELAXED, __HIP_MEMORY_SCOPE_WORKGROUP);
                if ((int32_t)((uint32_t)__builtin_amdgcn_readfirstlane(seen) - need) < 0 && !__builtin_amdgcn_readfirstlane(gave_up)) {
                    const unsigned long long t0 = wall_clock64();
                    while (true) {
                        const uint32_t now = __builtin_amdgcn_readfirstlane(
                            __hip_atomic_load(ctr, __ATOMIC_RELAXED, __HIP_MEMORY_SCOPE_AGENT));
                        if ((int32_t)(now - need) >= 0) {
                            if (lane == 0) __hip_atomic_store(&s_ctl[2], (int)now, __ATOMIC_RELAXED, __HIP_MEMORY_SCOPE_WORKGROUP);
                            break;
                        }
                        if (wall_clock64() - t0 > 20000ull) {
                            if (lane == 0) __hip_atomic_store(&s_ctl[3], 1, __ATOMIC_RELAXED, __HIP_MEMORY_SCOPE_WORKGROUP);
                            break;
                        }
                        __builtin_amdgcn_s_sleep(4);
                    }
                }
            }
            last_T = T;
            int wave_prev_row = -1, wave_next_row = -1;
            if (ng > 0) {
                const int64_t lo = dyn ? g0 : gw_lo, hi = dyn ? g0 + ng : gw_hi;
                if (lo > g_lo) wave_prev_row = p.p2n[lo - 1];
                if (hi < g_hi) wave_next_row = p.p2n[hi];
            }
            if (dyn && lane == 0) {
                const unsigned bit = 1u << (chunk & 31);
                while (__hip_atomic_fetch_or(&s_lock[chunk >> 5], bit, __ATOMIC_ACQUIRE, __HIP_MEMORY_SCOPE_WORKGROUP) & bit)
                    __builtin_amdgcn_s_sleep(2);
            }

            if (ng > 0)
            {
                const int f_lo = t * p.S / B, f_hi = (t + 1) * p.S / B;

                const bool gl = lane < ng;
                const int my_row = gl ? p.p2n[g0 + lane] : -1;
                const int pa = gl ? p.pp[g0 + lane] : 0;
                const int pb = gl ? p.pp[g0 + lane + 1] : 0;
                int cum_lo = 0, cum_hi = 0x7fffffff;
                if (gl) {
                    if (f_lo > 0) cum_lo = p.cnt[(size_t)(f_lo - 1) * (size_t)p.P + (size_t)(g0 + lane)];
                    if (f_hi < p.S) cum_hi = p.cnt[(size_t)(f_hi - 1) * (size_t)p.P + (size_t)(g0 + lane)];
                }
                const bool packed = dyn && p.ids_packed != nullptr && !stale_ids;
                const uint32_t item_base = packed ? p.item_off[(size_t)t * (size_t)p.num_chunks + (size_t)(g0 >> 6)] : 0u;
                const int32_t *__restrict__ ids = packed ? p.ids_packed : p.col;
                const int len = pb > pa ? pb - pa : 0;
                const int beg = cum_lo < len ? cum_lo : len;
                int end = cum_hi < len ? cum_hi : len;
                end = end > beg ? end : beg;
                const int n_own = gl ? end - beg : 0;
                if (__ballot(n_own > 0) != 0) {
                    const int up_row = __shfl_up(my_row, 1);
                    const bool seg_start = gl && (lane == 0 || my_row != up_row || !canonical);
                    const unsigned long long SS = __ballot(seg_start);
                    const int up_end = __shfl_up(pa + end, 1), up_n = __shfl_up(n_own, 1);
                    const bool cont = n_own > 0 && !seg_start && up_n > 0 && (packed || up_end == pa + beg);
                    const unsigned long long NE = __ballot(n_own > 0 && !cont);
                    const int n_cum = wave_inclusive_scan(n_own);
                    const unsigned long long heads_above = NE & above;
                    const int next_head = heads_above ? __builtin_ctzll(heads_above) : 64;
                    const int chain_cum = __shfl(n_cum, next_head - 1);
                    const int n = (n_own > 0 && !cont) ? chain_cum - n_cum + n_own : 0;
                    const unsigned long long between = SS & above & (next_head < 63 ? ((2ull << next_head) - 1ull) : ~0ull);
                    const bool last_in_seg = n > 0 && (next_head == 64 || between != 0);
                    const int aslot = my_row - row_first;
                    const int over = (aslot < 0 || aslot >= nrows) ? 1 : 0;
                    const int edge = (my_row == wave_prev_row || my_row == wave_next_row) ? 4 : 0;

                    const int rank = __popcll(NE & (upto >> 1));
                    const int Rn = __popcll(NE);
                    const int dstl = (n > 0 ? rank : 63) << 2;
                    const int c_pbeg = __builtin_amdgcn_ds_permute(dstl, packed ? (int)item_base + (n_cum - n_own) : pa + beg);
                    const int t_n = __builtin_amdgcn_ds_permute(dstl, n);
                    const int c_n = lane < Rn ? t_n : 0;
                    const int c_meta = __builtin_amdgcn_ds_permute(dstl, ((over ? my_row : aslot) << 3) | edge | (last_in_seg ? 2 : 0) | over);
                    const int c_nl = (c_n + RPI - 1) / RPI;
                    const int c_offI = wave_inclusive_scan(c_nl);
                    const int c_offX = c_offI - c_nl;
                    const int L = __builtin_amdgcn_readlane(c_offI, kWave - 1);

                    VT acc = vzero<4>();
                    struct Round {
                        uint32_t o[RPI];
                        int v_j, k_meta;
                        unsigned long long FL, TM;
                        int nr;
                    };
                    auto describe = [&](int r0) -> Round {
                        Round rd;
                        const unsigned long long below = __ballot(lane < Rn && c_offI <= r0);
                        unsigned long long inwin = __ballot(lane < Rn && c_offI > r0 && c_offI <= r0 + RL - 1);
                        unsigned long long E = 0;
                        while (inwin) {
                            const int kk = __builtin_ctzll(inwin);
                            inwin &= inwin - 1;
                            E |= 1ull << (__builtin_amdgcn_readlane(c_offI, kk) - r0);
                        }
                        const int kp = __popcll(below) + __popcll(E & upto);
                        const int k_offX = __shfl(c_offX, kp), k_pbeg = __shfl(c_pbeg, kp), k_n = __shfl(c_n, kp);
                        rd.k_meta = __shfl(c_meta, kp);
                        const int J = r0 + lane;
                        const bool active = J < L && lane < RL;
                        const int i = J - k_offX;
                        const int e_j = k_pbeg + i * RPI;
                        int v_j = active ? k_n - i * RPI : 0;
                        const bool fl_j = active && (rd.k_meta & 2) && v_j <= RPI;
                        v_j = v_j > RPI ? RPI : v_j;
                        rd.v_j = v_j;
                        rd.FL = __ballot(fl_j);
                        rd.TM = __ballot(active && v_j < RPI);
                        rd.nr = (L - r0) < RL ? (L - r0) : RL;
#pragma unroll
                        for (int q = 0; q < RPI; q++) rd.o[q] = 0u;
                        if (lane < RL) {
                            if (v_j == RPI) {
                                if constexpr (RPI >= 4) {
                                    typedef int i32x4 __attribute__((ext_vector_type(4)));
                                    typedef i32x4 i32x4u __attribute__((aligned(4)));
#pragma unroll
                                    for (int s4 = 0; s4 < RPI; s4 += 4) {
                                        const i32x4 tt = *reinterpret_cast<const i32x4u *>(ids + e_j + s4);
                                        rd.o[s4] = (uint32_t)tt[0]; rd.o[s4 + 1] = (uint32_t)tt[1]; rd.o[s4 + 2] = (uint32_t)tt[2]; rd.o[s4 + 3] = (uint32_t)tt[3];
                                    }
                                } else {
#pragma unroll
                                    for (int q = 0; q < RPI; q++) rd.o[q] = (uint32_t)ids[e_j + q];
                                }
                            } else {
                                const uint32_t first = v_j > 0 ? (uint32_t)ids[e_j] : 0u;
#pragma unroll
                                for (int q = 0; q < RPI; q++) {
                                    rd.o[q] = first;
                                    if (q > 0 && q < v_j) rd.o[q] = (uint32_t)ids[e_j + q];
                                }
                            }
                        }
                        return rd;
                    };
                    Round cur = describe(0);
                    for (int r0 = 0; r0 < L; r0 += RL) {
                        if (lane < RL) {
#pragma unroll
                            for (int q = 0; q < RPI; q++) offs[lane * RPI + q] = cur.o[q] * row_bytes32;
                        }
                        const bool more = r0 + RL < L;
                        Round nxt = cur;
                        if (more) nxt = describe(r0 + RL);
                        const int v_j = cur.v_j, k_meta = cur.k_meta, nr = cur.nr;
                        const unsigned long long FL = cur.FL, TM = cur.TM;

                        auto row_ptr = [&](uint32_t o) -> const MT * {
                            return reinterpret_cast<const MT *>(xbase + (o + col_off));
                        };
                        const int nb = (nr + U - 1) / U;
                        VT v[U];
#pragma unroll
                        for (int u = 0; u < U; u++) v[u] = *row_ptr(offs[u * RPI + lslot]);
                        auto consume = [&](int u, int j) {
                            if ((TM >> j) & 1ull) {
                                const int vj = __builtin_amdgcn_readlane(v_j, j);
                                if (lslot >= vj) v[u] = vzero<4>();
                            }
                            acc += v[u];
                            if ((FL >> j) & 1ull) {
                                const int meta = __builtin_amdgcn_readlane(k_meta, j);
                                const VT rr = fold_row<LPR, MODE_SAG>(acc, 1.f);
                                if (!(meta & 1)) {
                                    float *dst = s_acc + (meta >> 3) * D + dcol;
                                    if (meta & 4) {
                                        if constexpr (LPR <= 16) {
                                            if (add_lane) lds_add(dst + comp, rr[0]);
                                        } else {
                                            if (add_lane) {
#pragma unroll
                                                for (int q = 0; q < 4; q++)
                                                    if (q >= shift) lds_add(dst + q, rr[q]);
                                            }
                                        }
                                    } else {
                                        if constexpr (LPR <= 16) {
                                            if (add_lane) dst[comp] += rr[0];
                                        } else {
                                            if (add_lane) {
#pragma unroll
                                                for (int q = 0; q < 4; q++)
                                                    if (q >= shift) dst[q] += rr[q];
                                            }
                                        }
                                    }
                                } else {
                                    const int64_t row = meta >> 3;
                                    float scale = 1.f;
                                    if constexpr (MODE == MODE_GIN) {
                                        scale = p.eps;
                                        if (p.row_scale) scale *= p.row_scale[row];
                                    }
                                    float *dst = p.Y + (size_t)row * (size_t)p.ldy + dcol;
                                    if constexpr (LPR <= 16) {
                                        if (add_lane) unsafeAtomicAdd(dst + comp, rr[0] * scale);
                                    } else {
                                        if (add_lane) {
#pragma unroll
                                            for (int q = 0; q < 4; q++)
                                                if (q >= shift) unsafeAtomicAdd(dst + q, rr[q] * scale);
                                        }
                                    }
                                }
                                acc = vzero<4>();
                            }
                        };
#pragma unroll 1
                        for (int b = 0; b + 1 < nb; b++) {
                            const int jn = (b + 1) * U;
                            uint32_t nn[U];
#pragma unroll
                            for (int u = 0; u < U; u++) nn[u] = offs[(jn + u) * RPI + lslot];
#pragma unroll
                            for (int u = 0; u < U; u++) {
                                consume(u, b * U + u);
                                v[u] = *row_ptr(nn[u]);
                            }
                        }
#pragma unroll
                        for (int u = 0; u < U; u++) {
                            const int j = (nb - 1) * U + u;
                            if (j < nr) consume(u, j);
                        }
                        cur = nxt;
                    }
                }
            }
            if (dyn && lane == 0)
                (void)__hip_atomic_fetch_and(&s_lock[chunk >> 5], ~(1u << (chunk & 31)), __ATOMIC_RELEASE, __HIP_MEMORY_SCOPE_WORKGROUP);
            if (syncing && lane == 0 && (dyn || chunk == per_step - 1)) {
                const int done = __hip_atomic_fetch_add(&s_ctl[1], 1, __ATOMIC_RELAXED, __HIP_MEMORY_SCOPE_WORKGROUP) + 1;
                if (done % (dyn ? nchunks : kSweepWaves) == 0)
                    (void)__hip_atomic_fetch_add(ctr, 1u, __ATOMIC_RELAXED, __HIP_MEMORY_SCOPE_AGENT);
            }
        }
        if (dyn && nchunks == 0 && syncing && threadIdx.x == 0)
            (void)__hip_atomic_fetch_add(ctr, (uint32_t)B, __ATOMIC_RELAXED, __HIP_MEMORY_SCOPE_AGENT);
        __syncthreads();

        for (int q = wib; q < nrows; q += kSweepWaves) {
            const int row = row_first + q;
            const bool shared = row == set_prev_row || row == set_next_row;
            const bool use_atomic = shared || !p.plain_ok;
            float scale = 1.f;
            if constexpr (MODE == MODE_GIN) {
                scale = p.eps;
                if (p.row_scale) scale *= p.row_scale[row];
            }
            float *dst = p.Y + (size_t)row * (size_t)p.ldy;
            const float *src = s_acc + q * D;
            for (int i = lane; i < D; i += kWave) {
                const float val = src[i] * scale;
                if (!use_atomic) __builtin_nontemporal_store(p.relu ? fmaxf(val, 0.f) : val, dst + i);
                else unsafeAtomicAdd(dst + i, val);
            }
        }
        __syncthreads();
    }
}

typedef void (*SweepKernel)(const SweepParams);

template <int LPR, int MODE, int WGS>
SweepKernel pick_sweep_u(int u)
{
    constexpr int RPI = kWave / LPR;
    constexpr int RL = (kSweepIdSlots / RPI < kWave) ? kSweepIdSlots / RPI : kWave;
    if constexpr (RL % 16 == 0 && WGS == 1) {
        if (u >= 16) return sweep_kernel<LPR, MODE, 16, WGS>;
    }
    if constexpr (RL % 8 == 0 && WGS == 1) {
        if (u >= 8) return sweep_kernel<LPR, MODE, 8, WGS>;
    }
    return sweep_kernel<LPR, MODE, 4, WGS>;
}

template <int MODE, int WGS>
SweepKernel pick_sweep(int lpr, int u)
{
    switch (lpr) {
    case 4: return pick_sweep_u<4, MODE, WGS>(u);
    case 8: return pick_sweep_u<8, MODE, WGS>(u);
    case 16: return pick_sweep_u<16, MODE, WGS>(u);
    default: return pick_sweep_u<32, MODE, WGS>(u);
    }
}

}

int sweep_acc_rows(int dim, int wgs)
{
    const int pieces = (dim + 3) / 4;
    const int acc = wgs == 1 ? (pieces <= 8 ? acc_floats<8, 1>() : acc_floats<16, 1>())
                             : (pieces <= 8 ? acc_floats<8, 2>() : acc_floats<16, 2>());
    return std::max(1, acc / std::max(1, dim));
}

bool sweep_supports(int mode, int dim, size_t x_bytes)
{
    return (mode == MODE_SAG || mode == MODE_GIN) && dim >= 4 && dim <= 128 && x_bytes <= 0xffffffffull;
}

int launch_sweep(DeviceState *ds, const SweepLaunch &a, hipStream_t stream)
{
    SweepParams p;
    p.X = a.X; p.col = a.col; p.pp = a.pp; p.p2n = a.p2n; p.Y = a.Y; p.cnt = a.cnt; p.row_scale = a.row_scale;
    p.flag = a.flag; p.seq = a.seq; p.trust = a.trust; p.sync = a.sync;
    p.P = a.P; p.D = a.D; p.ldx = a.ldx; p.S = a.S; p.B = a.B; p.plain_ok = a.plain_ok ? 1 : 0; p.eps = a.eps;
    p.ldy = a.ldy > 0 ? a.ldy : a.D;
    p.relu = (a.relu && a.plain_ok) ? 1 : 0;
    p.slack = a.slack > 0 ? a.slack : 2;
    p.ids_packed = a.packed_stale ? a.ids_packed : nullptr; p.item_off = a.item_off; p.packed_stale = a.packed_stale;
    p.num_chunks = (a.P + kWave - 1) / kWave;
    p.dynamic = a.dynamic ? 1 : 0;
    int lpr = 4;
    const int pieces = (a.D + 3) / 4;
    while (lpr < 32 && lpr < pieces) lpr <<= 1;
    const int wgs = a.wgs_per_cu == 2 ? 2 : 1;
    SweepKernel k = wgs == 1 ? (a.mode == MODE_GIN ? pick_sweep<MODE_GIN, 1>(lpr, a.U) : pick_sweep<MODE_SAG, 1>(lpr, a.U))
                             : (a.mode == MODE_GIN ? pick_sweep<MODE_GIN, 2>(lpr, a.U) : pick_sweep<MODE_SAG, 2>(lpr, a.U));
    const int cus_per_xcd = std::max(1, ds->num_cus / kXcds);
    const unsigned grid = (unsigned)(cus_per_xcd * kXcds * wgs);
    const int cap = sweep_acc_rows(a.D, wgs);
    int R = a.rounds;
    if (R <= 0) {
        const double rows = (double)std::max<int64_t>(1, a.rows_with_edges);
        R = (int)std::max(1.0, std::ceil(rows / ((double)grid * 0.9 * (double)cap)));
    }
    p.rounds = std::min(R, 4096);
    hipLaunchKernelGGL(k, dim3(grid), dim3(kSweepBlock), 0, stream, p);
    hipError_t e = hipGetLastError();
    if (e != hipSuccess) return fail(GNNA_ERR_HIP, "sweep launch: %s", hipGetErrorString(e));
    count_event(CTR_SWEEP_LAUNCHES);
    if (a.relu) {
        const bool whole = !a.plain_ok;
        const int64_t blocks = std::max<int64_t>(1, std::min<int64_t>((a.num_out_rows + kWavesPerBlock - 1) / kWavesPerBlock, 256 * 8));
        hipLaunchKernelGGL(sweep_relu_fixup_kernel, dim3((unsigned)blocks), dim3(kBlock), 0, stream, a.Y, a.num_out_rows, a.D, p.ldy,
                           a.sync + kXcds * 16, a.flag, a.seq, a.trust, whole ? 1 : 0);
        e = hipGetLastError();
        if (e != hipSuccess) return fail(GNNA_ERR_HIP, "epilogue launch: %s", hipGetErrorString(e));
    }
    return GNNA_OK;
}

}
```

Baseline: 82.21 billion edges/s.

## Split hub-to-hub edges into a dense MFMA block alongside the residual sweep

Adds a dense-block path for power-law graphs. It picks high-degree hub nodes, encodes the hub-to-hub adjacency as a bitmap and aggregates those edges with an MFMA-based dense kernel. The remaining edges are rewritten into a residual CSR that the sweep kernel reads instead of the full graph. This is meant to cut gather traffic for the dense hub subgraph, at the cost of one-time build kernels, extra memory, a second launch, and a cost model that decides whether the block pays off.

```diff
diff --git a/gnnadvisor_osdi21_amd/_lib.py b/gnnadvisor_osdi21_amd/_lib.py
--- a/gnnadvisor_osdi21_amd/_lib.py
+++ b/gnnadvisor_osdi21_amd/_lib.py
@@ -564,7 +564,7 @@
     out = (ctypes.c_int64 * 16)()
     n = load().gnna_runtime_counters_ex(out, 16)
     names = ("plan_builds", "launch_syncs", "launch_frees", "launch_mallocs", "backoff_skips", "sweep_launches",
-             "pack_builds", "packed_launches", "full_hashes", "capture_scratch")
+             "pack_builds", "packed_launches", "full_hashes", "capture_scratch", "dense_block_builds", "dense_block_launches")
     return {name: int(out[i]) for i, name in enumerate(names) if i < n}
 
 
diff --git a/gnnadvisor_osdi21_amd/build.py b/gnnadvisor_osdi21_amd/build.py
--- a/gnnadvisor_osdi21_amd/build.py
+++ b/gnnadvisor_osdi21_amd/build.py
@@ -14,7 +14,7 @@
 ARCH = "gfx950"
 HIPCC = os.environ.get("HIPCC", "/opt/rocm/bin/hipcc")
 
-LIB_SOURCES = [os.path.join(CSRC, f) for f in ("gnna_agg.hip", "gnna_stream.hip", "gnna_sweep.hip", "gnna_x16.hip", "gnna_reduce.hip", "gnna_stats.hip", "gnna_softagg.hip", "gnna_pool.hip", "gnna_attnpool.hip", "gnna_sddmm.hip", "gnna_edge.hip", "gnna_gat.hip", "gnna_gatv2.hip", "gnna_dotattn.hip", "gnna_typed.hip", "gnna_transpose.hip", "gnna_sample.hip",
+LIB_SOURCES = [os.path.join(CSRC, f) for f in ("gnna_agg.hip", "gnna_stream.hip", "gnna_sweep.hip", "gnna_dense.hip", "gnna_x16.hip", "gnna_reduce.hip", "gnna_stats.hip", "gnna_softagg.hip", "gnna_pool.hip", "gnna_attnpool.hip", "gnna_sddmm.hip", "gnna_edge.hip", "gnna_gat.hip", "gnna_gatv2.hip", "gnna_dotattn.hip", "gnna_typed.hip", "gnna_transpose.hip", "gnna_sample.hip",
                                                 "gnna_gemm.hip", "gnna_runtime.hip", "gnna_host.cpp", "gnna_reorder.cpp")]
 LIB_DEPS = LIB_SOURCES + [os.path.join(CSRC, "gnna_internal.h"), os.path.join(CSRC, "gnna_device.h"), os.path.join(CSRC, "gnna_launch.h"),
                            os.path.join(CSRC, "gnna_gat_common.h"), os.path.join(CSRC, "gnna_keys.h"), os.path.join(CSRC, "gnna_segments.h"), os.path.join(INCLUDE, "gnna.h"), os.path.join(INCLUDE, "gnna_ext.h"),
diff --git a/gnnadvisor_osdi21_amd/csrc/gnna_agg.hip b/gnnadvisor_osdi21_amd/csrc/gnna_agg.hip
--- a/gnnadvisor_osdi21_amd/csrc/gnna_agg.hip
+++ b/gnnadvisor_osdi21_amd/csrc/gnna_agg.hip
@@ -305,6 +305,30 @@
     if (t.column_phases >= 2) return B;
     return std::max(2, std::min(std::min(16, 2 * B), std::max(2, part_size / 4)));
 }
+
+constexpr double kDenseEdgeSeconds = 10.7e-12;
+constexpr double kDenseChunkSeconds = 2.06e-6;
+constexpr double kDenseLaunchSeconds = 7.0e-6;
+constexpr double kDenseMinSaving = 25.0e-6;
+constexpr double kDenseMinShare = 0.03;
+
+int trimmed_hubs(int H, int num_cus)
+{
+    const int round = kDenseTileRanks * std::max(1, num_cus);
+    return (H > round && H % round != 0 && H % round < round / 4) ? H / round * round : H;
+}
+
+double dense_block_saving(double hubs, double entries, int num_cus)
+{
+    if (hubs <= 0.0) return 0.0;
+    const double He = (double)trimmed_hubs((int)hubs, num_cus);
+    const double Hp = std::ceil(He / kDenseChunkRanks) * kDenseChunkRanks;
+    const double rounds = std::ceil(Hp / kDenseTileRanks / (double)std::max(1, num_cus));
+    const double kept = entries * (He / hubs) * (He / hubs);
+    return kept * kDenseEdgeSeconds - rounds * (Hp / kDenseChunkRanks) * kDenseChunkSeconds - kDenseLaunchSeconds;
+}
+
+bool dense_block_pays(double saving, double entries, double edges) { return saving > kDenseMinSaving && entries >= kDenseMinShare * edges; }
 
 int sweep_phases_of_width(const gnna_tuning &t, int dim, size_t foot_bytes, size_t x_bytes, int64_t num_out_rows,
                           int64_t num_in_rows, const SlicePlanStats &st, int B, int num_cus, int partSize, int S)
@@ -624,6 +648,15 @@
             if (rc != GNNA_OK) return rc;
             if (sw_ids) count_event(CTR_PACKED_LAUNCHES);
         }
+        DenseBlock db;
+        const int32_t *res_ids = nullptr; const uint32_t *res_off = nullptr;
+        bool dense = false;
+        if (sw_ids && plan.pinned && !relu && dim >= kDenseMinDim && dim <= kDenseMaxDim && num_in_rows == num_nodes && tune.column_phases < 2 &&
+            plan_dense_block(plan.handle, &db) && !db.off && db.res_plan && db.res_cnt && (auto_Bs > 0 || db.forced)) {
+            rc = get_packed_ids(ds, stream, db.res_plan, Bs, kWave, false, false, &res_ids, &res_off);
+            if (rc != GNNA_OK) return rc;
+            dense = true;
+        }
         uint32_t *sync = ds->sweep_sync + (size_t)call_block_of(ds, stream, seq) * kSweepSlotWords;
         static_assert(kXcds * 16 + 2 <= kBlock, "the prologue clears the sweep counters with one block");
         rc = run_prologue(0, sync, kXcds * 16 + 2);
@@ -640,10 +673,15 @@
         w.dynamic = tune.xcd_remap != 0;
         w.plain_ok = !accumulate_into_out; w.eps = eps;
         w.ids_packed = sw_ids; w.item_off = sw_off; w.packed_stale = stale_flag;
+        if (dense) { w.res_col = db.res_col; w.res_pp = db.res_pp; w.res_cnt = db.res_cnt; w.res_ids_packed = res_ids; w.res_item_off = res_off; }
         t_last_phases = Bs;
         t_last_launches = 1;
         rc = launch_sweep(ds, w, stream);
         if (rc != GNNA_OK) return rc;
+        if (dense) {
+            rc = launch_hub_block(ds, stream, db, X, ldx, out, ldy, dim, mode == MODE_GIN, eps, row_scale, stale_flag, seq);
+            if (rc != GNNA_OK) return rc;
+        }
         profile_record(prof_call, 2, stream);
         return GNNA_OK;
     }
@@ -935,6 +973,41 @@
                 rc = get_packed_ids(ds, stream, plan.handle, B, std::max(1, std::min(kWave, t.groups_per_chunk * B)), true, true, &ids, &off);
             if (rc != GNNA_OK) return rc;
             if (phases_out && Bs >= 2) phases_out[i] = first_of_width ? Bs : std::max(phases_out[i], Bs);
+            const int dense_mode = dense_block_mode();
+            const bool self_swept = t.sweep == 0 && t.column_phases < 2;
+            {
+                DenseBlock have;
+                if (plan_dense_block(plan.handle, &have) && have.off != (dense_mode == 0)) {
+                    have.off = dense_mode == 0;
+                    plan_set_dense_block(plan.handle, have);
+                }
+            }
+            if (swept && ids && dense_mode != 0 && dim >= kDenseMinDim && dim <= kDenseMaxDim && num_in_rows == num_out_rows &&
+                (dense_mode == 2 || self_swept)) {
+                DenseBlock db;
+                if (!plan_dense_block(plan.handle, &db) && db.declined_mode != dense_mode) {
+                    rc = build_dense_block(ds, stream, column_index, part_pointers, part2Node, num_parts, num_in_rows,
+                                           (int64_t)plan.stats.edges, dense_mode, &db);
+                    if (rc != GNNA_OK) return rc;
+                    if (db.buf) {
+                        QuietBuilds quiet;
+                        SlicePlan res;
+                        rc = get_slice_plan(ds, stream, db.res_col, db.res_pp, part2Node, num_parts, num_in_rows, true, true, &res);
+                        if (rc == GNNA_OK && res.cnt) { db.res_plan = res.handle; db.res_cnt = res.cnt; }
+                        plan_set_dense_block(plan.handle, db);
+                        if (rc != GNNA_OK) return rc;
+                    } else {
+                        db.declined_mode = dense_mode;
+                        plan_set_dense_block(plan.handle, db);
+                    }
+                }
+                if (db.buf && db.res_plan) {
+                    QuietBuilds quiet;
+                    const int32_t *rids = nullptr; const uint32_t *roff = nullptr;
+                    rc = get_packed_ids(ds, stream, db.res_plan, Bs, kWave, true, true, &rids, &roff);
+                    if (rc != GNNA_OK) return rc;
+                }
+            }
         }
         if (t.deterministic == 1 && dim >= 4) {
             const int G_eff = std::max(1, std::min(kWave, t.groups_per_chunk * std::max(1, B)));
diff --git a/gnnadvisor_osdi21_amd/csrc/gnna_dense.hip b/gnnadvisor_osdi21_amd/csrc/gnna_dense.hip
--- /dev/null
+++ b/gnnadvisor_osdi21_amd/csrc/gnna_dense.hip
@@ -0,0 +1,473 @@
+#include <hip/hip_runtime.h>
+
+#include <algorithm>
+#include <cmath>
+#include <cstdint>
+#include <cstdio>
+#include <cstdlib>
+#include <vector>
+
+#include "gnna.h"
+#include "gnna_device.h"
+#include "gnna_internal.h"
+
+namespace gnna {
+namespace {
+
+constexpr int kHubBuckets = 64;
+constexpr int kHubMax = 16384;
+constexpr int kHubThreads = 512;
+constexpr int kHubWaves = kHubThreads / kWave;
+constexpr int kHubTileM = kDenseTileRanks;
+constexpr int kHubKC = kDenseChunkRanks;
+static_assert(kHubTileM == 32, "two MFMA tiles per workgroup");
+constexpr int kHubStage = kHubKC / 32;
+constexpr int kHubRowStride = 80;
+static_assert(kHubKC % kHubTileM == 0 && kHubKC * 16 == kHubThreads * kHubStage && kHubKC / 4 * 2 == kWave, "staging; one bitmap word per lane");
+static_assert((kHubKC / 4) % kHubWaves == 0 && (kHubTileM * 64) % kHubThreads == 0, "steps per wavefront, elements per thread");
+
+__host__ __device__ inline int hub_bucket(int64_t d)
+{
+    if (d <= 1) return 0;
+    int k = 0;
+    while ((d >> (k + 1)) != 0) k++;
+    const int b = 2 * k + ((d * d >= ((int64_t)1 << (2 * k + 1))) ? 1 : 0);
+    return b < kHubBuckets ? b : kHubBuckets - 1;
+}
+
+__global__ void __launch_bounds__(kBlock)
+hub_degree_kernel(const int32_t *__restrict__ pp, const int32_t *__restrict__ p2n, int64_t P, int64_t N, int32_t *__restrict__ deg)
+{
+    for (int64_t g = (int64_t)blockIdx.x * blockDim.x + threadIdx.x; g < P; g += (int64_t)gridDim.x * blockDim.x) {
+        const int64_t r = p2n[g];
+        const int len = pp[g + 1] - pp[g];
+        if (r >= 0 && r < N && len > 0) atomicAdd(&deg[r], len);
+    }
+}
+
+__global__ void __launch_bounds__(kBlock)
+hub_hist_kernel(const int32_t *__restrict__ col, const int32_t *__restrict__ pp, const int32_t *__restrict__ p2n, int64_t P, int64_t N,
+                const int32_t *__restrict__ deg, unsigned long long *__restrict__ hist)
+{
+    __shared__ unsigned int s_h[2 * kHubBuckets];
+    for (int i = threadIdx.x; i < 2 * kHubBuckets; i += kBlock) s_h[i] = 0u;
+    __syncthreads();
+    const int64_t tid = (int64_t)blockIdx.x * blockDim.x + threadIdx.x, nthreads = (int64_t)gridDim.x * blockDim.x;
+    for (int64_t i = tid; i < N; i += nthreads) atomicAdd(&s_h[hub_bucket(deg[i])], 1u);
+    const int lane = threadIdx.x & (kWave - 1);
+    const int64_t wave = tid >> 6, nwaves = nthreads >> 6;
+    for (int64_t g = wave; g < P; g += nwaves) {
+        const int64_t r = p2n[g];
+        if (r < 0 || r >= N) continue;
+        const int dd = deg[r];
+        const int a = pp[g], b = pp[g + 1];
+        for (int e = a + lane; e < b; e += kWave) {
+            const int64_t s = col[e];
+            if (s < 0 || s >= N) continue;
+            const int ds = deg[s];
+            atomicAdd(&s_h[kHubBuckets + hub_bucket(dd < ds ? dd : ds)], 1u);
+        }
+    }
+    __syncthreads();
+    for (int i = threadIdx.x; i < 2 * kHubBuckets; i += kBlock)
+        if (s_h[i]) atomicAdd(&hist[i], (unsigned long long)s_h[i]);
+}
+
+__global__ void __launch_bounds__(kBlock)
+hub_list_kernel(const int32_t *__restrict__ deg, int64_t N, int theta, int32_t *__restrict__ count, int32_t *__restrict__ list, int cap)
+{
+    for (int64_t i = (int64_t)blockIdx.x * blockDim.x + threadIdx.x; i < N; i += (int64_t)gridDim.x * blockDim.x) {
+        if (deg[i] >= theta) {
+            const int idx = atomicAdd(count, 1);
+            if (idx < cap) { list[idx] = (int32_t)i; list[cap + idx] = deg[i]; }
+        }
+    }
+}
+
+__global__ void __launch_bounds__(kBlock)
+hub_rank_kernel(const int32_t *__restrict__ r2n, int H, int64_t N, int32_t *__restrict__ n2r)
+{
+    const int i = blockIdx.x * blockDim.x + threadIdx.x;
+    if (i < H && r2n[i] >= 0 && r2n[i] < N) n2r[r2n[i]] = i;
+}
+
+__global__ void __launch_bounds__(kBlock)
+hub_bitmap_kernel(const int32_t *__restrict__ col, const int32_t *__restrict__ pp, const int32_t *__restrict__ p2n, int64_t P, int64_t N,
+                  const int32_t *__restrict__ n2r, int words_per_tile_row, unsigned long long *__restrict__ bm,
+                  uint32_t *__restrict__ taken, unsigned long long *__restrict__ total)
+{
+    const int lane = threadIdx.x & (kWave - 1);
+    const int64_t wave = ((int64_t)blockIdx.x * blockDim.x + threadIdx.x) >> 6;
+    const int64_t nwaves = ((int64_t)gridDim.x * blockDim.x) >> 6;
+    unsigned int mine = 0;
+    for (int64_t g = wave; g < P; g += nwaves) {
+        const int64_t r = p2n[g];
+        if (r < 0 || r >= N) continue;
+        const int rd = n2r[r];
+        if (rd < 0) continue;
+        const int a = pp[g], b = pp[g + 1];
+        for (int e = a + lane; e < b; e += kWave) {
+            const int64_t s = col[e];
+            if (s < 0 || s >= N) continue;
+            const int rs = n2r[s];
+            if (rs < 0) continue;
+            const size_t word = (size_t)(rd >> 4) * (size_t)words_per_tile_row + (size_t)(rs >> 2);
+            const unsigned long long bit = 1ull << ((rd & 15) + 16 * (rs & 3));
+            const unsigned long long old = atomicOr(&bm[word], bit);
+            if (!(old & bit)) {
+                atomicOr(&taken[(uint32_t)e >> 5], 1u << (e & 31));
+                mine++;
+            }
+        }
+    }
+    unsigned long long sum = mine;
+    for (int d = 32; d > 0; d >>= 1) sum += __shfl_xor(sum, d);
+    if (lane == 0 && sum) atomicAdd(total, sum);
+}
+
+__device__ __forceinline__ bool hub_taken(const uint32_t *__restrict__ taken, int e)
+{
+    return (taken[(uint32_t)e >> 5] >> (e & 31)) & 1u;
+}
+
+__global__ void __launch_bounds__(kBlock)
+hub_res_count_kernel(const int32_t *__restrict__ pp, int64_t P, const uint32_t *__restrict__ taken, int32_t *__restrict__ res_pp)
+{
+    for (int64_t g = (int64_t)blockIdx.x * blockDim.x + threadIdx.x; g <= P; g += (int64_t)gridDim.x * blockDim.x) {
+        int n = 0;
+        if (g < P) {
+            const int a = pp[g], b = pp[g + 1];
+            for (int e = a; e < b; e++) n += hub_taken(taken, e) ? 0 : 1;
+        }
+        res_pp[g] = n;
+    }
+}
+
+__global__ void __launch_bounds__(kBlock)
+hub_res_fill_kernel(const int32_t *__restrict__ col, const int32_t *__restrict__ pp, int64_t P, const uint32_t *__restrict__ taken,
+                    const int32_t *__restrict__ res_pp, int32_t *__restrict__ res_col, int64_t res_nnz)
+{
+    const int lane = threadIdx.x & (kWave - 1);
+    const int64_t wave = ((int64_t)blockIdx.x * blockDim.x + threadIdx.x) >> 6;
+    const int64_t nwaves = ((int64_t)gridDim.x * blockDim.x) >> 6;
+    const unsigned long long below = (1ull << lane) - 1ull;
+    for (int64_t g = wave; g < P; g += nwaves) {
+        const int a = pp[g], b = pp[g + 1];
+        int64_t at = res_pp[g];
+        for (int e0 = a; e0 < b; e0 += kWave) {
+            const int e = e0 + lane;
+            const bool keep = e < b && !hub_taken(taken, e);
+            const unsigned long long K = __ballot(keep);
+            const int64_t dst = at + __popcll(K & below);
+            if (keep && dst < res_nnz) res_col[dst] = col[e];
+            at += __popcll(K);
+        }
+    }
+}
+
+struct HubParams {
+    const float *X;
+    float *Y;
+    const int32_t *r2n;
+    const unsigned long long *bm;
+    const float *row_scale;
+    const int32_t *stale;
+    int32_t seq;
+    int H_pad, D, ldx, ldy;
+    int scaled;
+    float eps;
+};
+
+__global__ void __launch_bounds__(kHubThreads)
+hub_block_kernel(const HubParams p)
+{
+    typedef typename VecOf<4>::T VT;
+    typedef typename VecOf<4>::M MT;
+    if (*p.stale == p.seq) return;
+    __shared__ __attribute__((aligned(16))) float s_x[kHubKC * kHubRowStride];
+    __shared__ float s_red[kHubTileM][64];
+    const int tid = (int)threadIdx.x;
+    const int lane = tid & (kWave - 1);
+    const int wib = __builtin_amdgcn_readfirstlane(tid >> 6);
+    const int chunks = p.H_pad / kHubKC;
+    const int words_per_tile_row = p.H_pad >> 2;
+    const int tile0 = (int)blockIdx.x * (kHubTileM / 16);
+    const int D = p.D;
+
+    const int srow = tid >> 4, spiece = (tid & 15) * 4;
+    auto load_piece = [&](int node) -> VT {
+        VT v = vzero<4>();
+        if (node >= 0 && spiece < D) {
+            const float *src = p.X + (size_t)node * (size_t)p.ldx + spiece;
+            if (spiece + 4 <= D) {
+                v = *reinterpret_cast<const MT *>(src);
+            } else {
+#pragma unroll
+                for (int q = 0; q < 4; q++)
+                    if (spiece + q < D) v[q] = src[q];
+            }
+        }
+        return v;
+    };
+    struct Stage {
+        VT r[kHubStage];
+        int node[kHubStage];
+        unsigned long long w;
+    };
+    auto fetch_ids = [&](int c, Stage &st) {
+#pragma unroll
+        for (int i = 0; i < kHubStage; i++) st.node[i] = c < chunks ? p.r2n[c * kHubKC + 32 * i + srow] : -1;
+    };
+    auto fetch = [&](int c, Stage &st) {
+        if (c >= chunks) return;
+#pragma unroll
+        for (int i = 0; i < kHubStage; i++) st.r[i] = load_piece(st.node[i]);
+        st.w = p.bm[(size_t)(tile0 + (lane >> 5)) * (size_t)words_per_tile_row + (size_t)(c * (kHubKC / 4) + (lane & 31))];
+        fetch_ids(c + 2, st);
+    };
+
+    VT acc[2][4];
+#pragma unroll
+    for (int t = 0; t < 2; t++)
+#pragma unroll
+        for (int q = 0; q < 4; q++) acc[t][q] = vzero<4>();
+
+    auto multiply = [&](unsigned long long w) {
+        const int w_lo = (int)(uint32_t)w, w_hi = (int)(uint32_t)(w >> 32);
+#pragma unroll
+        for (int j = 0; j < kHubKC / 4 / kHubWaves; j++) {
+            const int s = wib * (kHubKC / 4 / kHubWaves) + j;
+            const unsigned long long m0 = ((unsigned long long)(uint32_t)__builtin_amdgcn_readlane(w_hi, s) << 32) |
+                                          (uint32_t)__builtin_amdgcn_readlane(w_lo, s);
+            const unsigned long long m1 = ((unsigned long long)(uint32_t)__builtin_amdgcn_readlane(w_hi, 32 + s) << 32) |
+                                          (uint32_t)__builtin_amdgcn_readlane(w_lo, 32 + s);
+            if ((m0 | m1) == 0ull) continue;
+            const float *xs = &s_x[(s * 4 + (lane >> 4)) * kHubRowStride + (lane & 15)];
+            const float a0 = ((m0 >> lane) & 1ull) ? 1.f : 0.f;
+            const float a1 = ((m1 >> lane) & 1ull) ? 1.f : 0.f;
+#pragma unroll
+            for (int q = 0; q < 4; q++) {
+                if (q * 16 >= D) continue;
+                const float b = xs[q * 16];
+                acc[0][q] = __builtin_amdgcn_mfma_f32_16x16x4f32(a0, b, acc[0][q], 0, 0, 0);
+                acc[1][q] = __builtin_amdgcn_mfma_f32_16x16x4f32(a1, b, acc[1][q], 0, 0, 0);
+            }
+        }
+    };
+    auto turn = [&](int c, Stage &st) {
+        if (c >= chunks) return;
+        __syncthreads();
+#pragma unroll
+        for (int i = 0; i < kHubStage; i++) *reinterpret_cast<VT *>(&s_x[(srow + 32 * i) * kHubRowStride + spiece]) = st.r[i];
+        const unsigned long long w = st.w;
+        __syncthreads();
+        fetch(c + 2, st);
+        multiply(w);
+    };
+    Stage s0, s1;
+    fetch_ids(0, s0);
+    fetch_ids(1, s1);
+    fetch(0, s0);
+    fetch(1, s1);
+    for (int c = 0; c < chunks; c += 2) {
+        turn(c, s0);
+        turn(c + 1, s1);
+    }
+
+    for (int w = 0; w < kHubWaves; w++) {
+        if (wib == w) {
+#pragma unroll
+            for (int t = 0; t < 2; t++)
+#pragma unroll
+                for (int q = 0; q < 4; q++)
+#pragma unroll
+                    for (int r = 0; r < 4; r++) {
+                        float *d = &s_red[t * 16 + (lane >> 4) * 4 + r][q * 16 + (lane & 15)];
+                        *d = w == 0 ? acc[t][q][r] : *d + acc[t][q][r];
+                    }
+        }
+        __syncthreads();
+    }
+#pragma unroll
+    for (int i = 0; i < kHubTileM * 64 / kHubThreads; i++) {
+        const int idx = i * kHubThreads + tid;
+        const int row = idx >> 6, col = idx & 63;
+        const float sum = s_red[row][col];
+        const int node = p.r2n[tile0 * 16 + row];
+        if (node < 0 || col >= D || sum == 0.f) continue;
+        float scale = 1.f;
+        if (p.scaled) {
+            scale = p.eps;
+            if (p.row_scale) scale *= p.row_scale[node];
+        }
+        float *dst = p.Y + (size_t)node * (size_t)p.ldy + col;
+        *dst += sum * scale;
+    }
+}
+
+int smallest_degree_of_bucket(int b)
+{
+    if (b <= 0) return 0;
+    int64_t d = (int64_t)std::floor(std::pow(2.0, b / 2.0)) - 2;
+    if (d < 1) d = 1;
+    while (hub_bucket(d) < b) d++;
+    return (int)std::min<int64_t>(d, 0x7fffffff);
+}
+
+struct DenseTemp {
+    void *ptr = nullptr;
+    ~DenseTemp() { if (ptr) { (void)hipFree(ptr); count_event(CTR_LAUNCH_FREES); } }
+};
+
+size_t align256(size_t n) { return (n + 255) & ~(size_t)255; }
+
+}
+
+int dense_block_mode()
+{
+    const char *s = std::getenv("GNNA_DENSE_BLOCK");
+    if (!s || !*s) return 1;
+    const int v = std::atoi(s);
+    return v == 0 ? 0 : (v == 2 ? 2 : 1);
+}
+
+int build_dense_block(DeviceState *ds, hipStream_t stream, const int32_t *col, const int32_t *pp, const int32_t *p2n, int64_t P,
+                      int64_t N, int64_t nnz, int mode, DenseBlock *out)
+{
+    *out = DenseBlock();
+    if (mode == 0 || P <= 0 || N <= 0 || nnz <= 0 || nnz > 0x7fffffffLL || N > 0x7fffffffLL) return GNNA_OK;
+    const size_t deg_b = align256((size_t)N * 4), hist_b = align256(2 * kHubBuckets * 8), cnt_b = 256;
+    const size_t list_b = align256((size_t)kHubMax * 8), taken_b = align256((((size_t)nnz + 31) / 32 + 1) * 4);
+    const size_t part_b = align256((size_t)std::max<int64_t>(1, scan_tiles(P + 1)) * 4), n2r_b = align256((size_t)N * 4);
+    DenseTemp tmp;
+    hipError_t e = hipMalloc(&tmp.ptr, deg_b + hist_b + cnt_b + list_b + taken_b + part_b + n2r_b);
+    count_event(CTR_LAUNCH_MALLOCS);
+    if (e != hipSuccess) { tmp.ptr = nullptr; (void)hipGetLastError(); return GNNA_OK; }
+    char *base = static_cast<char *>(tmp.ptr);
+    int32_t *deg = reinterpret_cast<int32_t *>(base);
+    unsigned long long *hist = reinterpret_cast<unsigned long long *>(base + deg_b);
+    int32_t *hub_count = reinterpret_cast<int32_t *>(base + deg_b + hist_b);
+    unsigned long long *taken_total = reinterpret_cast<unsigned long long *>(base + deg_b + hist_b + 8);
+    int32_t *hub_list = reinterpret_cast<int32_t *>(base + deg_b + hist_b + cnt_b);
+    uint32_t *taken = reinterpret_cast<uint32_t *>(base + deg_b + hist_b + cnt_b + list_b);
+    int32_t *partial = reinterpret_cast<int32_t *>(base + deg_b + hist_b + cnt_b + list_b + taken_b);
+    int32_t *n2r = reinterpret_cast<int32_t *>(base + deg_b + hist_b + cnt_b + list_b + taken_b + part_b);
+    (void)hipMemsetAsync(tmp.ptr, 0, deg_b + hist_b + cnt_b + list_b + taken_b, stream);
+    const unsigned gblocks = elementwise_grid(P, ds->num_cus, 8);
+    const unsigned wblocks = (unsigned)std::max<int64_t>(1, std::min<int64_t>((P + kWavesPerBlock - 1) / kWavesPerBlock, (int64_t)ds->num_cus * 16));
+    hipLaunchKernelGGL(hub_degree_kernel, dim3(gblocks), dim3(kBlock), 0, stream, pp, p2n, P, N, deg);
+    hipLaunchKernelGGL(hub_hist_kernel, dim3(wblocks), dim3(kBlock), 0, stream, col, pp, p2n, P, N, deg, hist);
+    unsigned long long h[2 * kHubBuckets];
+    e = hipMemcpyAsync(h, hist, sizeof(h), hipMemcpyDeviceToHost, stream);
+    if (e == hipSuccess) e = hipStreamSynchronize(stream);
+    if (e != hipSuccess) return fail(GNNA_ERR_HIP, "dense block (histograms): %s", hipGetErrorString(e));
+
+    int best_b = -1;
+    double best_gain = 0.0;
+    double Hs = 0.0, Es = 0.0;
+    int fallback_b = -1;
+    for (int b = kHubBuckets - 1; b >= 1; b--) {
+        Hs += (double)h[b];
+        Es += (double)h[kHubBuckets + b];
+        if (Hs <= 0.0) continue;
+        if (Hs > (double)kHubMax) break;
+        if (Es > 0.0) fallback_b = b;
+        const double gain = dense_block_saving(Hs, Es, ds->num_cus);
+        const bool ok = mode == 2 ? Es > 0.0 : dense_block_pays(gain, Es, (double)nnz);
+        if (ok && (best_b < 0 || gain > best_gain)) { best_b = b; best_gain = gain; }
+    }
+    int theta = best_b >= 0 ? smallest_degree_of_bucket(best_b) : 0;
+    if (mode == 2) {
+        if (best_b < 0 && fallback_b >= 0) theta = smallest_degree_of_bucket(fallback_b);
+        const char *s = std::getenv("GNNA_DENSE_BLOCK_THETA");
+        if (s && *s && std::atoi(s) > 0) theta = std::atoi(s);
+    }
+    if (theta <= 0) return GNNA_OK;
+
+    hipLaunchKernelGGL(hub_list_kernel, dim3(elementwise_grid(N, ds->num_cus, 8)), dim3(kBlock), 0, stream, deg, N, theta, hub_count,
+                       hub_list, kHubMax);
+    std::vector<int32_t> fetched((cnt_b + list_b) / 4);
+    e = hipMemcpyAsync(fetched.data(), hub_count, cnt_b + list_b, hipMemcpyDeviceToHost, stream);
+    if (e == hipSuccess) e = hipStreamSynchronize(stream);
+    if (e != hipSuccess) return fail(GNNA_ERR_HIP, "dense block (hub ids): %s", hipGetErrorString(e));
+    int32_t H = fetched[0];
+    if (H <= 0 || H > kHubMax) return GNNA_OK;
+    const int32_t *got = fetched.data() + cnt_b / 4;
+    std::vector<int32_t> ids(got, got + H), degs(got + kHubMax, got + kHubMax + H);
+    if (trimmed_hubs(H, ds->num_cus) != H) {
+        std::vector<int32_t> order((size_t)H);
+        for (int i = 0; i < H; i++) order[(size_t)i] = i;
+        std::sort(order.begin(), order.end(), [&](int32_t a, int32_t b) {
+            return degs[(size_t)a] != degs[(size_t)b] ? degs[(size_t)a] > degs[(size_t)b] : ids[(size_t)a] < ids[(size_t)b];
+        });
+        H = trimmed_hubs(H, ds->num_cus);
+        std::vector<int32_t> kept((size_t)H);
+        for (int i = 0; i < H; i++) kept[(size_t)i] = ids[(size_t)order[(size_t)i]];
+        ids.swap(kept);
+    }
+    const int H_pad = (H + kHubKC - 1) / kHubKC * kHubKC;
+    std::vector<int32_t> ranks((size_t)H_pad, -1);
+    std::copy(ids.begin(), ids.end(), ranks.begin());
+    std::sort(ranks.begin(), ranks.begin() + H);
+
+    const size_t r2n_b = align256((size_t)H_pad * 4);
+    const size_t bm_b = align256((size_t)(H_pad / 16) * (size_t)(H_pad / 4) * 8), rpp_b = align256((size_t)(P + 1) * 4);
+    void *blk = nullptr;
+    e = hipMalloc(&blk, r2n_b + bm_b + rpp_b);
+    count_event(CTR_LAUNCH_MALLOCS);
+    if (e != hipSuccess) { (void)hipGetLastError(); return GNNA_OK; }
+    char *bb = static_cast<char *>(blk);
+    int32_t *r2n = reinterpret_cast<int32_t *>(bb);
+    unsigned long long *bm = reinterpret_cast<unsigned long long *>(bb + r2n_b);
+    int32_t *res_pp = reinterpret_cast<int32_t *>(bb + r2n_b + bm_b);
+    int32_t *res_col = nullptr;
+    auto give_up = [&](int rc) { (void)hipStreamSynchronize(stream); (void)hipFree(blk); if (res_col) (void)hipFree(res_col); return rc; };
+    e = hipMemcpy(r2n, ranks.data(), (size_t)H_pad * 4, hipMemcpyHostToDevice);
+    if (e != hipSuccess) return give_up(fail(GNNA_ERR_HIP, "dense block (ranks): %s", hipGetErrorString(e)));
+    (void)hipMemsetAsync(n2r, 0xff, n2r_b, stream);
+    (void)hipMemsetAsync(bm, 0, bm_b, stream);
+    hipLaunchKernelGGL(hub_rank_kernel, dim3((unsigned)((H + kBlock - 1) / kBlock)), dim3(kBlock), 0, stream, r2n, (int)H, N, n2r);
+    hipLaunchKernelGGL(hub_bitmap_kernel, dim3(wblocks), dim3(kBlock), 0, stream, col, pp, p2n, P, N, n2r, H_pad / 4, bm, taken, taken_total);
+    hipLaunchKernelGGL(hub_res_count_kernel, dim3(elementwise_grid(P + 1, ds->num_cus, 8)), dim3(kBlock), 0, stream, pp, P, taken, res_pp);
+    int rc = launch_exclusive_scan(stream, res_pp, P + 1, partial);
+    if (rc != GNNA_OK) return give_up(rc);
+    unsigned long long entries = 0;
+    e = hipMemcpyAsync(&entries, taken_total, sizeof(entries), hipMemcpyDeviceToHost, stream);
+    if (e == hipSuccess) e = hipStreamSynchronize(stream);
+    if (e != hipSuccess) return give_up(fail(GNNA_ERR_HIP, "dense block (bitmap): %s", hipGetErrorString(e)));
+    const int64_t res_nnz = nnz - (int64_t)entries;
+    if (entries == 0 || res_nnz <= 0) return give_up(GNNA_OK);
+    e = hipMalloc(reinterpret_cast<void **>(&res_col), ((size_t)res_nnz + 16) * 4);
+    count_event(CTR_LAUNCH_MALLOCS);
+    if (e != hipSuccess) { (void)hipGetLastError(); res_col = nullptr; return give_up(GNNA_OK); }
+    (void)hipMemsetAsync(res_col + res_nnz, 0, 16 * 4, stream);
+    hipLaunchKernelGGL(hub_res_fill_kernel, dim3(wblocks), dim3(kBlock), 0, stream, col, pp, P, taken, res_pp, res_col, res_nnz);
+    e = hipGetLastError();
+    if (e == hipSuccess) e = hipStreamSynchronize(stream);
+    if (e != hipSuccess) return give_up(fail(GNNA_ERR_HIP, "dense block (residual): %s", hipGetErrorString(e)));
+    out->buf = blk; out->r2n = r2n; out->bm = bm; out->res_pp = res_pp; out->res_col = res_col;
+    out->H = H; out->H_pad = H_pad; out->theta = theta; out->entries = (int64_t)entries; out->res_nnz = res_nnz;
+    out->forced = mode == 2;
+    const char *log = std::getenv("GNNA_DENSE_BLOCK_LOG");
+    if (log && *log && *log != '0')
+        std::fprintf(stderr, "gnna dense block: theta %d, H %d (padded %d), entries %lld of %lld edges, density %.3f\n", theta, (int)H,
+                     H_pad, (long long)entries, (long long)nnz, (double)entries / ((double)H * (double)H));
+    count_event(CTR_DENSE_BUILDS);
+    return GNNA_OK;
+}
+
+int launch_hub_block(DeviceState *ds, hipStream_t stream, const DenseBlock &db, const float *X, int ldx, float *Y, int ldy, int dim,
+                     bool scaled, float eps, const float *row_scale, const int32_t *stale_flag, int32_t seq)
+{
+    HubParams p;
+    p.X = X; p.Y = Y; p.r2n = db.r2n; p.bm = static_cast<const unsigned long long *>(db.bm); p.row_scale = row_scale;
+    p.stale = stale_flag; p.seq = seq; p.H_pad = db.H_pad; p.D = dim; p.ldx = ldx; p.ldy = ldy;
+    p.scaled = scaled ? 1 : 0; p.eps = eps;
+    (void)ds;
+    hipLaunchKernelGGL(hub_block_kernel, dim3((unsigned)(db.H_pad / kHubTileM)), dim3(kHubThreads), 0, stream, p);
+    const int rc = launch_ok("hub block launch");
+    if (rc == GNNA_OK) count_event(CTR_DENSE_LAUNCHES);
+    return rc;
+}
+
+}
diff --git a/gnnadvisor_osdi21_amd/csrc/gnna_internal.h b/gnnadvisor_osdi21_amd/csrc/gnna_internal.h
--- a/gnnadvisor_osdi21_amd/csrc/gnna_internal.h
+++ b/gnnadvisor_osdi21_amd/csrc/gnna_internal.h
@@ -121,8 +121,41 @@
                   bool square, bool hinted_scattered);
 enum { CTR_PLAN_BUILDS = 0, CTR_LAUNCH_SYNCS = 1, CTR_LAUNCH_FREES = 2, CTR_LAUNCH_MALLOCS = 3, CTR_BACKOFF_SKIPS = 4,
        CTR_SWEEP_LAUNCHES = 5, CTR_PACK_BUILDS = 6, CTR_PACKED_LAUNCHES = 7, CTR_FULL_HASHES = 8, CTR_CAPTURE_SCRATCH = 9,
-       CTR_COUNT = 10 };
+       CTR_DENSE_BUILDS = 10, CTR_DENSE_LAUNCHES = 11, CTR_COUNT = 12 };
 void count_event(int which);
+struct QuietBuilds {
+    QuietBuilds();
+    ~QuietBuilds();
+    QuietBuilds(const QuietBuilds &) = delete;
+    QuietBuilds &operator=(const QuietBuilds &) = delete;
+};
+
+struct DenseBlock {
+    void *buf = nullptr;
+    const int32_t *r2n = nullptr;
+    const void *bm = nullptr;
+    const int32_t *res_pp = nullptr;
+    int32_t *res_col = nullptr;
+    const uint8_t *res_cnt = nullptr;
+    void *res_plan = nullptr;
+    int H = 0, H_pad = 0, theta = 0;
+    int64_t entries = 0, res_nnz = 0;
+    bool forced = false;
+    bool off = false;
+    int declined_mode = -1;
+};
+constexpr int kDenseTileRanks = 32, kDenseChunkRanks = 128;
+constexpr int kDenseMinDim = 33, kDenseMaxDim = 64;
+int trimmed_hubs(int H, int num_cus);
+double dense_block_saving(double hubs, double entries, int num_cus);
+bool dense_block_pays(double saving, double entries, double edges);
+int dense_block_mode();
+int build_dense_block(DeviceState *ds, hipStream_t stream, const int32_t *col, const int32_t *pp, const int32_t *p2n, int64_t P,
+                      int64_t N, int64_t nnz, int mode, DenseBlock *out);
+int launch_hub_block(DeviceState *ds, hipStream_t stream, const DenseBlock &db, const float *X, int ldx, float *Y, int ldy, int dim,
+                     bool scaled, float eps, const float *row_scale, const int32_t *stale_flag, int32_t seq);
+bool plan_dense_block(void *plan_handle, DenseBlock *out);
+void plan_set_dense_block(void *plan_handle, const DenseBlock &db);
 
 struct StreamLaunch {
     int mode;
@@ -171,6 +204,8 @@
     float eps;
     const int32_t *ids_packed = nullptr; const uint32_t *item_off = nullptr;
     const int32_t *packed_stale = nullptr;
+    const int32_t *res_col = nullptr; const int32_t *res_pp = nullptr; const uint8_t *res_cnt = nullptr;
+    const int32_t *res_ids_packed = nullptr; const uint32_t *res_item_off = nullptr;
 };
 bool sweep_supports(int mode, int dim, size_t x_bytes);
 int sweep_acc_rows(int dim, int wgs_per_cu);
diff --git a/gnnadvisor_osdi21_amd/csrc/gnna_stream.hip b/gnnadvisor_osdi21_amd/csrc/gnna_stream.hip
--- a/gnnadvisor_osdi21_amd/csrc/gnna_stream.hip
+++ b/gnnadvisor_osdi21_amd/csrc/gnna_stream.hip
@@ -773,6 +773,7 @@
     std::vector<Packed> packed;
     uint64_t pack_lookups = 0;
     uint64_t pack_no_memory_until = 0;
+    DenseBlock dense;
 };
 constexpr uint64_t kPackedNoMemoryBackoff = 1024;
 constexpr int kMaxPacked = 4;
@@ -785,6 +786,7 @@
 int g_cold_evictions = 0;
 int g_skip_builds = 0;
 std::atomic<long long> g_counters[CTR_COUNT];
+thread_local int t_quiet_builds = 0;
 
 std::vector<void *> g_dead;
 std::atomic<int> g_in_flight{0};
@@ -825,7 +827,31 @@
 
 }
 
-void count_event(int which) { g_counters[which].fetch_add(1, std::memory_order_relaxed); }
+void count_event(int which)
+{
+    if (t_quiet_builds > 0 && (which == CTR_PLAN_BUILDS || which == CTR_PACK_BUILDS)) return;
+    g_counters[which].fetch_add(1, std::memory_order_relaxed);
+}
+QuietBuilds::QuietBuilds() { t_quiet_builds++; }
+QuietBuilds::~QuietBuilds() { t_quiet_builds--; }
+
+bool plan_dense_block(void *plan_handle, DenseBlock *out)
+{
+    std::lock_guard<std::mutex> lock(g_plan_mutex);
+    for (Plan *q : g_plans)
+        if (q == plan_handle) {
+            *out = q->dense;
+            return q->dense.buf != nullptr;
+        }
+    return false;
+}
+
+void plan_set_dense_block(void *plan_handle, const DenseBlock &db)
+{
+    std::lock_guard<std::mutex> lock(g_plan_mutex);
+    for (Plan *q : g_plans)
+        if (q == plan_handle) { q->dense = db; return; }
+}
 
 int get_slice_plan(DeviceState *ds, hipStream_t stream, const int32_t *column_index, const int32_t *part_pointers,
                    const int32_t *part2Node, int64_t num_parts, int64_t num_in_rows, bool want_stats, bool pin,
@@ -948,9 +974,21 @@
     std::lock_guard<std::mutex> lock(g_plan_mutex);
     int dropped = 0;
     if (!column_index) { g_cold_evictions = 0; g_skip_builds = 0; }
+    std::vector<const void *> also;
+    auto wanted = [&](const Plan *pl) {
+        if (!column_index || pl->col == column_index) return true;
+        return std::find(also.begin(), also.end(), pl->col) != also.end();
+    };
     for (size_t i = 0; i < g_plans.size();) {
         Plan *pl = g_plans[i];
-        if (column_index && pl->col != column_index) { i++; continue; }
+        if (!wanted(pl)) { i++; continue; }
+        if (pl->dense.buf) {
+            g_dead.push_back(pl->dense.buf);
+            if (pl->dense.res_col) { g_dead.push_back(pl->dense.res_col); also.push_back(pl->dense.res_col); }
+            i = 0;
+            pl->dense = DenseBlock();
+            continue;
+        }
         if (pl->cnt) g_dead.push_back(pl->cnt);
         if (pl->ready) (void)hipEventDestroy(pl->ready);
         for (auto &pk : pl->packed) {
diff --git a/gnnadvisor_osdi21_amd/csrc/gnna_sweep.hip b/gnnadvisor_osdi21_amd/csrc/gnna_sweep.hip
--- a/gnnadvisor_osdi21_amd/csrc/gnna_sweep.hip
+++ b/gnnadvisor_osdi21_amd/csrc/gnna_sweep.hip
@@ -55,6 +55,11 @@
     const uint32_t *item_off;
     const int32_t *packed_stale;
     int64_t num_chunks;
+    const int32_t *res_col;
+    const int32_t *res_pp;
+    const uint8_t *res_cnt;
+    const int32_t *res_ids_packed;
+    const uint32_t *res_item_off;
 };
 
 __device__ __forceinline__ int64_t lower_bound64(const int32_t *__restrict__ pp, int64_t P, int64_t target, int lane)
@@ -128,7 +133,13 @@
     const int c = lane % LPR;
     const int D = p.D;
     const bool canonical = p.trust || (*p.flag != p.seq);
-    const bool stale_ids = p.ids_packed != nullptr && *p.packed_stale == p.seq;
+    const bool use_res = p.res_pp != nullptr && *p.packed_stale != p.seq;
+    const int32_t *g_col = use_res ? p.res_col : p.col;
+    const int32_t *g_pp = use_res ? p.res_pp : p.pp;
+    const uint8_t *g_cnt = use_res ? p.res_cnt : p.cnt;
+    const int32_t *g_packed = use_res ? p.res_ids_packed : p.ids_packed;
+    const uint32_t *g_item_off = use_res ? p.res_item_off : p.item_off;
+    const bool stale_ids = !use_res && p.ids_packed != nullptr && *p.packed_stale == p.seq;
     const char *xbase = reinterpret_cast<const char *>(p.X);
     const uint32_t row_bytes32 = (uint32_t)p.ldx * 4u;
     uint32_t *offs = s_off[wib];
@@ -150,7 +161,7 @@
     uint32_t *ctr = p.sync + xcd * 16;
     const bool syncing = p.slack < 1000 && nbx > 1;
     const int B = p.B, R = p.rounds;
-    const int64_t nnz = (int64_t)p.pp[p.P];
+    const int64_t nnz = (int64_t)g_pp[p.P];
     const int64_t num_sets = (int64_t)gridDim.x * R;
 
     if (threadIdx.x == 0) { s_ctl[2] = 0; s_ctl[3] = 0; }
@@ -158,7 +169,7 @@
     for (int r = 0; r < R; r++) {
         const int64_t set = ((int64_t)xcd * nbx + bx) * R + r;
         if (wib < 2) {
-            const int64_t g = sweep_set_start(set + wib, num_sets, nnz, p.pp, p.P, canonical, p.ids_packed != nullptr, lane);
+            const int64_t g = sweep_set_start(set + wib, num_sets, nnz, g_pp, p.P, canonical, g_packed != nullptr, lane);
             if (lane == 0) s_g[wib] = g;
         }
         if (threadIdx.x == 0) { s_ctl[0] = 0; s_ctl[1] = 0; }
@@ -254,16 +265,16 @@
 
                 const bool gl = lane < ng;
                 const int my_row = gl ? p.p2n[g0 + lane] : -1;
-                const int pa = gl ? p.pp[g0 + lane] : 0;
-                const int pb = gl ? p.pp[g0 + lane + 1] : 0;
+                const int pa = gl ? g_pp[g0 + lane] : 0;
+                const int pb = gl ? g_pp[g0 + lane + 1] : 0;
                 int cum_lo = 0, cum_hi = 0x7fffffff;
                 if (gl) {
-                    if (f_lo > 0) cum_lo = p.cnt[(size_t)(f_lo - 1) * (size_t)p.P + (size_t)(g0 + lane)];
-                    if (f_hi < p.S) cum_hi = p.cnt[(size_t)(f_hi - 1) * (size_t)p.P + (size_t)(g0 + lane)];
+                    if (f_lo > 0) cum_lo = g_cnt[(size_t)(f_lo - 1) * (size_t)p.P + (size_t)(g0 + lane)];
+                    if (f_hi < p.S) cum_hi = g_cnt[(size_t)(f_hi - 1) * (size_t)p.P + (size_t)(g0 + lane)];
                 }
-                const bool packed = dyn && p.ids_packed != nullptr && !stale_ids;
-                const uint32_t item_base = packed ? p.item_off[(size_t)t * (size_t)p.num_chunks + (size_t)(g0 >> 6)] : 0u;
-                const int32_t *__restrict__ ids = packed ? p.ids_packed : p.col;
+                const bool packed = dyn && g_packed != nullptr && !stale_ids;
+                const uint32_t item_base = packed ? g_item_off[(size_t)t * (size_t)p.num_chunks + (size_t)(g0 >> 6)] : 0u;
+                const int32_t *__restrict__ ids = packed ? g_packed : g_col;
                 const int len = pb > pa ? pb - pa : 0;
                 const int beg = cum_lo < len ? cum_lo : len;
                 int end = cum_hi < len ? cum_hi : len;
@@ -536,6 +547,9 @@
     p.slack = a.slack > 0 ? a.slack : 2;
     p.ids_packed = a.packed_stale ? a.ids_packed : nullptr; p.item_off = a.item_off; p.packed_stale = a.packed_stale;
     p.num_chunks = (a.P + kWave - 1) / kWave;
+    const bool res = a.packed_stale && a.res_pp && a.res_col && a.res_cnt;
+    p.res_col = res ? a.res_col : nullptr; p.res_pp = res ? a.res_pp : nullptr; p.res_cnt = res ? a.res_cnt : nullptr;
+    p.res_ids_packed = res ? a.res_ids_packed : nullptr; p.res_item_off = res ? a.res_item_off : nullptr;
     p.dynamic = a.dynamic ? 1 : 0;
     int lpr = 4;
     const int pieces = (a.D + 3) / 4;
```

Result: faster. 84.18 billion edges/s (median of 6 runs) (+2.4%).
